# profess-dev/profess-ad

Hardware: AMD Instinct MI355X
Metric: energy+grad evals/sec (higher is better)
Workload: dtype f64; 1 GPU; 256^3 grid, f64, IonElectron+Hartree+WGC99(+TF+vW)+PBE closure chi->(E,dE/dchi); density=converged fcc-Al 32^3 fixture tiled 8^3 + 1e-3 low-|k| perturbation, parallelism=single GPU

## Files before the change

include/ofdft_hip.h:

```cpp
#ifndef OFDFT_HIP_H
#define OFDFT_HIP_H

#include <stdint.h>

#ifdef __cplusplus
extern "C" {
#endif

typedef struct ofdft_ctx ofdft_ctx;

#define OFDFT_OK            0
#define OFDFT_EINVAL       -1
#define OFDFT_EHIP         -2
#define OFDFT_ESTATE       -3
#define OFDFT_ENOMEM       -4

#define OFDFT_F64 0
#define OFDFT_F32 1

#define OFDFT_ION_ELECTRON  (1u << 0)
#define OFDFT_HARTREE       (1u << 1)
#define OFDFT_TF            (1u << 2)
#define OFDFT_VW            (1u << 3)
#define OFDFT_WT_NL         (1u << 4)
#define OFDFT_WGC99_NL      (1u << 5)
#define OFDFT_LDA_X         (1u << 6)
#define OFDFT_PZ_C          (1u << 7)
#define OFDFT_PW_C          (1u << 8)
#define OFDFT_CHACHIYO_C    (1u << 9)
#define OFDFT_PBE_X         (1u << 10)
#define OFDFT_PBE_C         (1u << 11)
#define OFDFT_GGA_K         (1u << 12)
#define OFDFT_VWGTF         (1u << 13)
#define OFDFT_NLK           (1u << 14)
#define OFDFT_NTERMS        15

#define OFDFT_P_WT_ALPHA    0
#define OFDFT_P_WT_BETA     1
#define OFDFT_P_WGC_ALPHA   2
#define OFDFT_P_WGC_BETA    3
#define OFDFT_P_WGC_GAMMA   4
#define OFDFT_P_WGC_KAPPA   5
#define OFDFT_P_GGAK_KIND   6
#define OFDFT_P_GGAK_MU     7
#define OFDFT_P_GGAK_BETA   8
#define OFDFT_P_GGAK_LAMBDA 9
#define OFDFT_P_GGAK_SIGMA  10
#define OFDFT_P_VWGTF_KIND  11
#define OFDFT_P_WTS_KIND    12
#define OFDFT_P_NLK_KIND    13
#define OFDFT_P_NLK_P0      14
#define OFDFT_P_NLK_P1      15
#define OFDFT_P_NLK_P2      16
#define OFDFT_NPARAMS       17

#define OFDFT_Q_FFT_COUNT        0
#define OFDFT_Q_WORKSPACE_BYTES  1
#define OFDFT_Q_FAST_PATH        2
#define OFDFT_Q_KERNEL_MS        3
#define OFDFT_Q_LAUNCH_COUNT     4
#define OFDFT_Q_YPASS_COUNT      5
#define OFDFT_Q_GRAPH_REPLAYS     6
#define OFDFT_Q_RESIDENT_EVALS    7
#define OFDFT_Q_XCHG_CHUNKS      9
#define OFDFT_Q_YFWD_FUSED      10
#define OFDFT_Q_RESIDENT_FALLBACKS 8
#define OFDFT_Q_XPASS_KINDS     11
#define OFDFT_XPASS_GROUP    (1u << 0)
#define OFDFT_XPASS_WAVE     (1u << 1)
#define OFDFT_XPASS_CROSS1   (1u << 2)
#define OFDFT_XPASS_CROSS2   (1u << 3)
#define OFDFT_XPASS_CHIRPZ   (1u << 4)

int  ofdft_create(ofdft_ctx** out, int n0, int n1, int n2, int dtype, int device_id);
void ofdft_destroy(ofdft_ctx* ctx);
const char* ofdft_last_error(const ofdft_ctx* ctx);

int  ofdft_set_cell(ofdft_ctx* ctx, const double box_vecs[9]);
int  ofdft_set_terms(ofdft_ctx* ctx, uint32_t term_mask, const double* params, int nparams);

int  ofdft_energy_potential(ofdft_ctx* ctx, const void* den_dev, const void* vext_dev,
                            double* E_terms_host, void* dEdn_dev, void* stream);

int  ofdft_energy_grad_chi(ofdft_ctx* ctx, const void* chi_dev, const void* vext_dev, double n_electrons,
                           double* E_terms_host, double* mu_host, void* grad_dev, void* stream);

int  ofdft_rfftn(ofdft_ctx* ctx, const void* real_dev, void* spec_dev, void* stream);
int  ofdft_irfftn(ofdft_ctx* ctx, const void* spec_dev, void* real_dev, void* stream);
int  ofdft_debug_math(ofdft_ctx* ctx, int kind, const void* in_dev, void* out_dev, long long n, void* stream);

int  ofdft_query(ofdft_ctx* ctx, int what, double* out);

int  ofdft_ipc_export(ofdft_ctx* ctx, void* handle64, unsigned long long* offsets5);
int  ofdft_ipc_attach(ofdft_ctx* ctx, int peer_rank, const void* handle64, const unsigned long long* offsets5);
int  ofdft_ipc_detach(ofdft_ctx* ctx);
int  ofdft_dist_closure(ofdft_ctx* ctx, const void* chi_local_dev, const void* vext_local_dev, double n_electrons_global,
                        double* E_terms_host, double* mu_host, void* grad_local_dev, void* v_work_local_dev, void* stream);

typedef int (*ofdft_all_to_all_fn)(void* user, void* send_dev, void* recv_dev, unsigned long long bytes_per_peer, void* stream);
typedef int (*ofdft_all_reduce_fn)(void* user, double* host_buf, int count);
int  ofdft_set_collectives(ofdft_ctx* ctx, ofdft_all_to_all_fn all_to_all, ofdft_all_reduce_fn all_reduce, void* user);

int  ofdft_create_dist(ofdft_ctx** out, int n0_global, int n1_global, int n2, int dtype, int device_id, int nranks, int rank);
int  ofdft_dist_sumsq(ofdft_ctx* ctx, const void* x_local_dev, int square, double* local_sum_host, void* stream);
int  ofdft_dist_begin(ofdft_ctx* ctx, const void* src_local_dev, int from_chi, double cscale, double n_electrons_global,
                      const void* vext_local_dev, void* v_out_local_dev, void* stream);
int  ofdft_dist_stage(ofdft_ctx* ctx, int stage, int chain, void* stream, unsigned long long* bytes_per_peer, void** sendbuf_dev,
                      void** recvbuf_dev);
int  ofdft_dist_step(ofdft_ctx* ctx, int step, int chain, int chunk, void* stream, unsigned long long* bytes_per_peer,
                     void** sendbuf_dev, void** recvbuf_dev);
int  ofdft_dist_finish(ofdft_ctx* ctx, double* local_sums_host , void* stream);
int  ofdft_dist_scalars(ofdft_ctx* ctx, void** scalars_dev );
int  ofdft_dist_energies(ofdft_ctx* ctx, const double* global_sums , double* E_terms_host, double* vn_integral);
int  ofdft_dist_chi_grad(ofdft_ctx* ctx, const void* chi_local_dev, const void* v_local_dev, void* grad_local_dev,
                         double cscale, double mu, void* stream);

int  ofdft_ionic_potential(ofdft_ctx* ctx, const double* frac_coords_host, int nions, const double* table_k_host,
                           const double* table_v_host, int ntable, double z_ion, int pme_order, void* vext_dev,
                           int accumulate, void* stream);

int  ofdft_ion_electron_forces(ofdft_ctx* ctx, const void* den_dev, const double* frac_coords_host, int nions,
                               const double* table_k_host, const double* table_v_host, int ntable, double z_ion,
                               int pme_order, double* forces_host, void* stream);

int  ofdft_stress(ofdft_ctx* ctx, const void* den_dev, double* sigma_terms_host, void* stream);
int  ofdft_ion_electron_stress(ofdft_ctx* ctx, const void* den_dev, const double* frac_coords_host, int nions,
                               const double* table_k_host, const double* table_v_host, int ntable, double z_ion,
                               int pme_order, double* sigma_host , void* stream);

int  ofdft_ion_ion(ofdft_ctx* ctx, const double* frac_coords_host, const double* charges_host, int nions, double Rc,
                   double* E_host, double* forces_host, double* stress_host, void* stream);

int  ofdft_ion_ion_cells(ofdft_ctx* ctx, const double* frac_coords_host, const double* charges_host, int nions, double Rc,
                         double Rd, int part, int nparts, double* E_host, double* forces_host ,
                         double* stress_host , void* stream);

typedef struct ofdft_lbfgs ofdft_lbfgs;
int  ofdft_lbfgs_create(ofdft_lbfgs** out, long long n_local, int history , int device_id);
void ofdft_lbfgs_destroy(ofdft_lbfgs* h);
const char* ofdft_lbfgs_last_error(const ofdft_lbfgs* h);
int  ofdft_lbfgs_reset(ofdft_lbfgs* h);
int  ofdft_lbfgs_direction(ofdft_lbfgs* h, const double* dots , int npairs, int first_iteration,
                           double* coef_s , double* coef_y , double* coef_g, double* g_dot_d,
                           int* npairs_out, int* pushed_out);
int  ofdft_lbfgs_abs_step(ofdft_lbfgs* h, double* abs_step_sum);
int  ofdft_lbfgs_dots(ofdft_lbfgs* h, const void* g_dev, double* dots_host , int* npairs, void* stream);
int  ofdft_lbfgs_commit(ofdft_lbfgs* h, int push);
int  ofdft_lbfgs_update(ofdft_lbfgs* h, const double* coef_s, const double* coef_y, double coef_g, double t, void* x_dev,
                        const void* g_dev, double* abs_step_sum_host, void* stream);

#define OFDFT_OPT_PIPELINE 0
#define OFDFT_OPT_XCHUNKS     2
#define OFDFT_OPT_XCHUNK_MASK 3
#define OFDFT_OPT_SPLIT_COMBINE 4
#define OFDFT_OPT_BLUESTEIN 5
#define OFDFT_OPT_GGA_SPLIT 6
#define OFDFT_OPT_GRAPH 7
#define OFDFT_OPT_SIDE_STREAM 1
#define OFDFT_OPT_MIXED_RADIX 9
#define OFDFT_OPT_RESIDENT 10
#define OFDFT_OPT_XCHG_CHUNKS 12
#define OFDFT_OPT_YBATCH 14
#define OFDFT_OPT_IPC_WAIT_MS 13
#define OFDFT_OPT_TEST_FAULT 11
#define OFDFT_OPT_BS_FUSED 15
#define OFDFT_OPT_POT_SPECTRUM 16
#define OFDFT_OPT_AXIS_PASSES 17
#define OFDFT_OPT_WGC_FOLD 28
#define OFDFT_OPT_XWAVE 8
int  ofdft_set_option(ofdft_ctx* ctx, int option, double value);

int  ofdft_set_profiling(ofdft_ctx* ctx, int on);
int  ofdft_profile_count(ofdft_ctx* ctx);
int  ofdft_profile_get(ofdft_ctx* ctx, int idx, char* name_buf, int buflen, double* total_ms, long long* launches);

#ifdef __cplusplus
}
#endif
#endif
```

professad_amd/_build.py:

```python
import contextlib
import fcntl
import os
import subprocess
import sys

PKG = os.path.dirname(os.path.abspath(__file__))
CSRC = os.path.join(PKG, 'csrc')
LIBDIR = os.path.join(PKG, 'lib')
LIB = os.path.join(LIBDIR, 'libofdft_hip.so')
LIB_F32 = os.path.join(LIBDIR, 'libofdft_hip_f32.so')
SOURCES = ['engine.hip', 'lines.hip', 'xpass_a.hip', 'xpass_b.hip', 'zfused.hip', 'resident.hip']
HEADERS = sorted(f for f in os.listdir(CSRC) if f.endswith('.h')) + [os.path.join('..', '..', 'include', 'ofdft_hip.h')]


def _stale(lib=None):
    lib = lib or LIB
    if not os.path.exists(lib):
        return True
    t = os.path.getmtime(lib)
    for f in SOURCES + HEADERS:
        p = os.path.join(CSRC, f)
        if os.path.exists(p) and os.path.getmtime(p) > t:
            return True
    return False


def _flags(extra_flags):
    return ['-O3', '-std=c++17', '--offload-arch=gfx950', '-fPIC', '-ffp-contract=on', '-Wall', '-Wno-unused-function',
            '-I', os.path.join(PKG, '..', 'include')] + list(extra_flags)


def _compile_and_link(extra_flags, out, verbose=False):
    hipcc = os.environ.get('HIPCC', '/opt/rocm/bin/hipcc')
    tag = '%s.%d' % (os.path.basename(out), os.getpid())
    objdir = os.path.join(LIBDIR, '.obj')
    os.makedirs(objdir, exist_ok=True)
    jobs, objs = [], []
    for src in SOURCES:
        obj = os.path.join(objdir, '%s.%s.o' % (tag, src))
        objs.append(obj)
        cmd = [hipcc] + _flags(extra_flags) + ['-c', os.path.join(CSRC, src), '-o', obj]
        if verbose:
            print(' '.join(cmd), flush=True)
        jobs.append((cmd, subprocess.Popen(cmd)))
    err = None
    for cmd, p in jobs:
        if p.wait() != 0:
            err = err or subprocess.CalledProcessError(p.returncode, cmd)
    try:
        if err:
            raise err
        link = [hipcc, '--offload-arch=gfx950', '-shared', '-fPIC'] + objs + ['-o', out]
        if verbose:
            print(' '.join(link), flush=True)
        subprocess.run(link, check=True)
    finally:
        for o in objs:
            with contextlib.suppress(OSError):
                os.remove(o)
    return out


@contextlib.contextmanager
def _build_lock():
    os.makedirs(LIBDIR, exist_ok=True)
    with open(os.path.join(LIBDIR, '.build.lock'), 'w') as fh:
        fcntl.flock(fh, fcntl.LOCK_EX)
        try:
            yield
        finally:
            fcntl.flock(fh, fcntl.LOCK_UN)


def build(force=False, verbose=True, extra_flags=(), out=None):
    os.makedirs(LIBDIR, exist_ok=True)
    if out is not None:
        tmp = '%s.tmp.%d' % (out, os.getpid())
        _compile_and_link(extra_flags, tmp, verbose)
        os.replace(tmp, out)
        return out
    import threading
    with _build_lock():
        todo = [(lib, flags) for lib, flags in ((LIB, []), (LIB_F32, ['-DOFDFT_REAL_F32', '-cl-single-precision-constant']))
                if force or _stale(lib)]
        errs = []

        def one(lib, flags):
            tmp = '%s.tmp.%d' % (lib, os.getpid())
            try:
                _compile_and_link(list(extra_flags) + flags, tmp, verbose)
                os.replace(tmp, lib)
            except Exception as e:
                errs.append(e)
                with contextlib.suppress(OSError):
                    os.remove(tmp)
        threads = [threading.Thread(target=one, args=t) for t in todo]
        for t in threads:
            t.start()
        for t in threads:
            t.join()
        if errs:
            raise errs[0]
    return LIB


if __name__ == '__main__':
    build(force='--force' in sys.argv)
```

professad_amd/_native.py:

```python
import ctypes as C
import os

import torch

from . import _build

_LIBS = {}

OK, EINVAL, EHIP, ESTATE, ENOMEM = 0, -1, -2, -3, -4
F64, F32 = 0, 1
TERM_BITS = {
    'ion_electron': 1 << 0, 'hartree': 1 << 1, 'tf': 1 << 2, 'vw': 1 << 3, 'wt_nl': 1 << 4, 'wgc99_nl': 1 << 5,
    'lda_x': 1 << 6, 'pz_c': 1 << 7, 'pw_c': 1 << 8, 'chachiyo_c': 1 << 9, 'pbe_x': 1 << 10, 'pbe_c': 1 << 11,
    'gga_k': 1 << 12, 'vwgtf': 1 << 13, 'nlk': 1 << 14,
}
TERM_ORDER = ['ion_electron', 'hartree', 'tf', 'vw', 'wt_nl', 'wgc99_nl', 'lda_x', 'pz_c', 'pw_c', 'chachiyo_c',
              'pbe_x', 'pbe_c', 'gga_k', 'vwgtf', 'nlk']
NTERMS = 15
NPARAMS = 17
NLK_KGAP, NLK_MGP, NLK_XWM = 1, 2, 3
NTERMS_ALWAYS = 14


def per_term(values, mask):
    return {nm: values[i] for i, nm in enumerate(TERM_ORDER) if i < NTERMS_ALWAYS or (mask & TERM_BITS[nm])}
Q_FFT_COUNT, Q_WORKSPACE_BYTES, Q_FAST_PATH, Q_KERNEL_MS, Q_LAUNCH_COUNT, Q_YPASS_COUNT, Q_GRAPH_REPLAYS, Q_RESIDENT_EVALS = 0, 1, 2, 3, 4, 5, 6, 7
Q_RESIDENT_FALLBACKS = 8
Q_XCHG_CHUNKS = 9
Q_YFWD_FUSED = 10
Q_XPASS_KINDS = 11
XPASS_GROUP, XPASS_WAVE, XPASS_CROSS1, XPASS_CROSS2, XPASS_CHIRPZ = 1 << 0, 1 << 1, 1 << 2, 1 << 3, 1 << 4
OPT_BLUESTEIN = 5
OPT_GGA_SPLIT = 6
OPT_GRAPH = 7
OPT_XWAVE = 8
OPT_MIXED_RADIX = 9
OPT_RESIDENT = 10
OPT_TEST_FAULT = 11
OPT_XCHG_CHUNKS = 12
OPT_IPC_WAIT_MS = 13
OPT_YBATCH = 14
OPT_BS_FUSED = 15
OPT_POT_SPECTRUM = 16
OPT_AXIS_PASSES = 17
OPT_WGC_FOLD = 28

EXPORTS = ['ofdft_create', 'ofdft_destroy', 'ofdft_last_error', 'ofdft_set_cell', 'ofdft_set_terms',
           'ofdft_energy_potential', 'ofdft_energy_grad_chi', 'ofdft_rfftn', 'ofdft_irfftn', 'ofdft_debug_math', 'ofdft_query',
           'ofdft_create_dist', 'ofdft_dist_sumsq', 'ofdft_dist_begin', 'ofdft_dist_stage', 'ofdft_dist_step', 'ofdft_dist_finish', 'ofdft_dist_scalars',
           'ofdft_dist_energies', 'ofdft_dist_chi_grad', 'ofdft_ipc_export', 'ofdft_ipc_attach', 'ofdft_ipc_detach', 'ofdft_dist_closure', 'ofdft_ionic_potential', 'ofdft_ion_electron_forces', 'ofdft_stress', 'ofdft_ion_electron_stress', 'ofdft_ion_ion', 'ofdft_ion_ion_cells', 'ofdft_lbfgs_create', 'ofdft_lbfgs_destroy', 'ofdft_lbfgs_last_error', 'ofdft_lbfgs_reset', 'ofdft_lbfgs_direction', 'ofdft_lbfgs_abs_step', 'ofdft_lbfgs_dots',
           'ofdft_lbfgs_commit', 'ofdft_lbfgs_update', 'ofdft_set_option', 'ofdft_set_collectives', 'ofdft_set_profiling', 'ofdft_profile_count', 'ofdft_profile_get']


A2A_FN = C.CFUNCTYPE(C.c_int, C.c_void_p, C.c_void_p, C.c_void_p, C.c_ulonglong, C.c_void_p)
ALLREDUCE_FN = C.CFUNCTYPE(C.c_int, C.c_void_p, C.POINTER(C.c_double), C.c_int)


class NativeLibraryError(RuntimeError):
    pass


def lib_path(dtype=F64):
    return _build.LIB_F32 if dtype == F32 else _build.LIB


def load(dtype=F64):
    if dtype in _LIBS:
        return _LIBS[dtype]
    env = 'OFDFT_LIB_F32' if dtype == F32 else 'OFDFT_LIB'
    path = os.environ.get(env) or lib_path(dtype)
    if os.environ.get(env):
        pass
    elif not os.path.exists(path) or (os.path.exists('/opt/rocm/bin/hipcc') and _build._stale(path)):
        try:
            _build.build(verbose=False)
        except Exception as e:
            raise NativeLibraryError('%s is missing and could not be built: %r' % (os.path.basename(path), e))
    try:
        lib = C.CDLL(path)
    except OSError as e:
        raise NativeLibraryError('cannot load %s: %s (the HIP engine is required; there is no CPU fallback)'
                                 % (path, e))
    vp, dp, ip = C.c_void_p, C.POINTER(C.c_double), C.c_int
    lib.ofdft_create.argtypes = [C.POINTER(vp), ip, ip, ip, ip, ip]
    lib.ofdft_create.restype = ip
    lib.ofdft_destroy.argtypes = [vp]
    lib.ofdft_destroy.restype = None
    lib.ofdft_last_error.argtypes = [vp]
    lib.ofdft_last_error.restype = C.c_char_p
    lib.ofdft_set_cell.argtypes = [vp, dp]
    lib.ofdft_set_cell.restype = ip
    lib.ofdft_set_terms.argtypes = [vp, C.c_uint32, dp, ip]
    lib.ofdft_set_terms.restype = ip
    lib.ofdft_energy_potential.argtypes = [vp, vp, vp, dp, vp, vp]
    lib.ofdft_energy_potential.restype = ip
    lib.ofdft_energy_grad_chi.argtypes = [vp, vp, vp, C.c_double, dp, dp, vp, vp]
    lib.ofdft_energy_grad_chi.restype = ip
    lib.ofdft_rfftn.argtypes = [vp, vp, vp, vp]
    lib.ofdft_rfftn.restype = ip
    lib.ofdft_irfftn.argtypes = [vp, vp, vp, vp]
    lib.ofdft_irfftn.restype = ip
    lib.ofdft_debug_math.argtypes = [vp, ip, vp, vp, C.c_longlong, vp]
    lib.ofdft_debug_math.restype = ip
    lib.ofdft_query.argtypes = [vp, ip, dp]
    lib.ofdft_query.restype = ip
    lib.ofdft_create_dist.argtypes = [C.POINTER(vp), ip, ip, ip, ip, ip, ip, ip]
    lib.ofdft_create_dist.restype = ip
    lib.ofdft_dist_sumsq.argtypes = [vp, vp, ip, dp, vp]
    lib.ofdft_dist_sumsq.restype = ip
    lib.ofdft_dist_begin.argtypes = [vp, vp, ip, C.c_double, C.c_double, vp, vp, vp]
    lib.ofdft_dist_begin.restype = ip
    lib.ofdft_dist_stage.argtypes = [vp, ip, ip, vp, C.POINTER(C.c_ulonglong), C.POINTER(vp), C.POINTER(vp)]
    lib.ofdft_dist_stage.restype = ip
    lib.ofdft_dist_step.argtypes = [vp, ip, ip, ip, vp, C.POINTER(C.c_ulonglong), C.POINTER(vp), C.POINTER(vp)]
    lib.ofdft_dist_step.restype = ip
    lib.ofdft_dist_scalars.argtypes = [vp, C.POINTER(vp)]
    lib.ofdft_dist_scalars.restype = ip
    lib.ofdft_dist_finish.argtypes = [vp, dp, vp]
    lib.ofdft_dist_finish.restype = ip
    lib.ofdft_dist_energies.argtypes = [vp, dp, dp, dp]
    lib.ofdft_dist_energies.restype = ip
    lib.ofdft_dist_chi_grad.argtypes = [vp, vp, vp, vp, C.c_double, C.c_double, vp]
    lib.ofdft_dist_chi_grad.restype = ip
    lib.ofdft_ipc_export.argtypes = [vp, vp, C.POINTER(C.c_ulonglong)]
    lib.ofdft_ipc_export.restype = ip
    lib.ofdft_ipc_attach.argtypes = [vp, ip, vp, C.POINTER(C.c_ulonglong)]
    lib.ofdft_ipc_attach.restype = ip
    lib.ofdft_ipc_detach.argtypes = [vp]
    lib.ofdft_ipc_detach.restype = ip
    lib.ofdft_dist_closure.argtypes = [vp, vp, vp, C.c_double, dp, dp, vp, vp, vp]
    lib.ofdft_dist_closure.restype = ip
    lib.ofdft_ionic_potential.argtypes = [vp, dp, ip, dp, dp, ip, C.c_double, ip, vp, ip, vp]
    lib.ofdft_ionic_potential.restype = ip
    lib.ofdft_ion_electron_forces.argtypes = [vp, vp, dp, ip, dp, dp, ip, C.c_double, ip, dp, vp]
    lib.ofdft_ion_electron_forces.restype = ip
    lib.ofdft_stress.argtypes = [vp, vp, dp, vp]
    lib.ofdft_stress.restype = ip
    lib.ofdft_ion_electron_stress.argtypes = [vp, vp, dp, ip, dp, dp, ip, C.c_double, ip, dp, vp]
    lib.ofdft_ion_electron_stress.restype = ip
    lib.ofdft_ion_ion.argtypes = [vp, dp, dp, ip, C.c_double, dp, dp, dp, vp]
    lib.ofdft_ion_ion.restype = ip
    lib.ofdft_ion_ion_cells.argtypes = [vp, dp, dp, ip, C.c_double, C.c_double, ip, ip, dp, dp, dp, vp]
    lib.ofdft_ion_ion_cells.restype = ip
    lib.ofdft_lbfgs_create.argtypes = [C.POINTER(vp), C.c_longlong, ip, ip]
    lib.ofdft_lbfgs_create.restype = ip
    lib.ofdft_lbfgs_destroy.argtypes = [vp]
    lib.ofdft_lbfgs_destroy.restype = None
    lib.ofdft_lbfgs_last_error.argtypes = [vp]
    lib.ofdft_lbfgs_last_error.restype = C.c_char_p
    lib.ofdft_lbfgs_reset.argtypes = [vp]
    lib.ofdft_lbfgs_reset.restype = ip
    lib.ofdft_lbfgs_dots.argtypes = [vp, vp, dp, C.POINTER(ip), vp]
    lib.ofdft_lbfgs_dots.restype = ip
    lib.ofdft_lbfgs_commit.argtypes = [vp, ip]
    lib.ofdft_lbfgs_commit.restype = ip
    lib.ofdft_lbfgs_update.argtypes = [vp, dp, dp, C.c_double, C.c_double, vp, vp, dp, vp]
    lib.ofdft_lbfgs_update.restype = ip
    lib.ofdft_lbfgs_direction.argtypes = [vp, dp, ip, ip, dp, dp, dp, dp, C.POINTER(ip), C.POINTER(ip)]
    lib.ofdft_lbfgs_direction.restype = ip
    lib.ofdft_lbfgs_abs_step.argtypes = [vp, dp]
    lib.ofdft_lbfgs_abs_step.restype = ip
    lib.ofdft_set_collectives.argtypes = [vp, A2A_FN, ALLREDUCE_FN, vp]
    lib.ofdft_set_collectives.restype = ip
    lib.ofdft_set_option.argtypes = [vp, ip, C.c_double]
    lib.ofdft_set_option.restype = ip
    lib.ofdft_set_profiling.argtypes = [vp, ip]
    lib.ofdft_set_profiling.restype = ip
    lib.ofdft_profile_count.argtypes = [vp]
    lib.ofdft_profile_count.restype = ip
    lib.ofdft_profile_get.argtypes = [vp, ip, C.c_char_p, ip, dp, C.POINTER(C.c_longlong)]
    lib.ofdft_profile_get.restype = ip
    _LIBS[dtype] = lib
    return lib
```

professad_amd/csrc/engine.hip:

```cpp
#include "engine_ctx.h"
#include <atomic>
#include <chrono>
#ifndef OFDFT_REAL_F32
#include "ion_kernels.h"
#include "ion_cells.h"
#include "stress_kernels.h"
#endif

namespace {
thread_local char g_create_error[512] = "";
}

namespace eng {

int fail(ofdft_ctx* c, int code, const char* fmt, ...) {
    va_list ap;
    va_start(ap, fmt);
    vsnprintf(c ? c->err : g_create_error, 512, fmt, ap);
    va_end(ap);
    return code;
}

int get_twiddle(ofdft_ctx* c, int n, cplx** out) {
    auto it = c->tw.find(n);
// ... 1309 lines not shown
    HIP_TRY(c, hipGetLastError());
    if (c->profiling) prof_collect(c);
    return OFDFT_OK;
}

int ofdft_irfftn(ofdft_ctx* c, const void* spec_dev, void* real_dev, void* stream) {
    hipStream_t st = (hipStream_t)stream;
    if (!c || !real_dev || !spec_dev) return OFDFT_EINVAL;
    OFDFT_ON_DEVICE(c, c->device);
    cplx* s;
    if (int rc = spec_ws(c, "io", &s)) return rc;
    OFDFT_LAUNCH(c, st, "spec_to_internal", spec_to_internal_kernel, dim3((unsigned)((c->g.total + 255) / 256)), dim3(256), 0,
                 (const cplx*)spec_dev, s, c->g);
    if (int rc = irfftn_internal(c, s, (real*)real_dev, 1.0 / (double)c->npts, st)) return rc;
    HIP_TRY(c, hipStreamSynchronize(st));
    HIP_TRY(c, hipGetLastError());
    if (c->profiling) prof_collect(c);
    return OFDFT_OK;
}

}
namespace {
__global__ void debug_math_kernel(int kind, const real* __restrict__ in, real* __restrict__ out, long long n) {
    for (long long i = (long long)blockIdx.x * blockDim.x + threadIdx.x; i < n; i += (long long)gridDim.x * blockDim.x) {
        const real x = in[i];
        real y;
        switch (kind) {
            case 0: y = fm::rcp(x); break;
            case 1: y = fm::log(x); break;
            case 2: y = fm::exp(x); break;
            case 3: y = fm::roots(x).y; break;
            case 4: y = fm::roots(x).n13; break;
            default: y = fm::roots(x).inv_n; break;
        }
        out[i] = y;
    }
}
}
extern "C" {

int ofdft_debug_math(ofdft_ctx* c, int kind, const void* in_dev, void* out_dev, long long n, void* stream) {
    hipStream_t st = (hipStream_t)stream;
    if (!c || !in_dev || !out_dev || n < 1 || kind < 0 || kind > 5) return OFDFT_EINVAL;
    OFDFT_ON_DEVICE(c, c->device);
    OFDFT_LAUNCH(c, st, "debug_math", debug_math_kernel, dim3(grid_for(n)), dim3(256), 0, kind, (const real*)in_dev, (real*)out_dev, n);
    HIP_TRY(c, hipStreamSynchronize(st));
    HIP_TRY(c, hipGetLastError());
    return OFDFT_OK;
}

#include "ipc_exchange.inc.h"

int ofdft_dist_sumsq(ofdft_ctx* c, const void* x_local, int square, double* local_sum, void* stream) {
    hipStream_t st = (hipStream_t)stream;
    if (!c || !x_local) return OFDFT_EINVAL;
    OFDFT_ON_DEVICE(c, c->device);
    if (local_sum) return device_sum(c, (const real*)x_local, square != 0, local_sum, st);
    const int blocks = grid_for(c->npts / 2 + 1, kRedThreads, kRedBlocks);
    if (square)
        OFDFT_LAUNCH(c, st, "sum", (sum_kernel<true>), dim3(blocks), dim3(kRedThreads), 0, (const real*)x_local, c->npts,
                     c->d_partial);
    else
        OFDFT_LAUNCH(c, st, "sum", (sum_kernel<false>), dim3(blocks), dim3(kRedThreads), 0, (const real*)x_local, c->npts,
                     c->d_partial);
    OFDFT_REDUCE(c, st, c->d_partial, blocks, 1, c->d_reduced + kSumsqSlot);
    HIP_TRY(c, hipGetLastError());
    return OFDFT_OK;
}

int ofdft_dist_scalars(ofdft_ctx* c, void** scalars_dev) {
    if (!c || !scalars_dev) return OFDFT_EINVAL;
    *scalars_dev = c->d_reduced;
    return OFDFT_OK;
}

int ofdft_dist_begin(ofdft_ctx* c, const void* src_local, int from_chi, double cscale, double nel_global,
                     const void* vext_local, void* v_out_local, void* stream) {
    hipStream_t st = (hipStream_t)stream;
    if (!c) return OFDFT_EINVAL;
    OFDFT_ON_DEVICE(c, c->device);
    if (int rc = begin_call(c, st)) return rc;
    if (!src_local) return fail(c, OFDFT_EINVAL, "null argument");
    if (!c->mask) return fail(c, OFDFT_ESTATE, "ofdft_set_terms has not been called");
    if ((c->mask & OFDFT_ION_ELECTRON) && !vext_local) return fail(c, OFDFT_EINVAL, "IonElectron term needs vext");
    if (!(c->fast && c->n2 / 2 <= 512)) return fail(c, OFDFT_EINVAL, "staged path needs the power-of-two fast path");
    if (gga_needs_laplacian(c) && !c->gga_split)
        return fail(c, OFDFT_EINVAL, "Laplacian-dependent Pauli-Gaussian members need the split-derivative GGA chain (OFDFT_OPT_GGA_SPLIT = 1)");
    if (wts_active(c) && c->nranks > 1)
        return fail(c, OFDFT_EINVAL, "the stabilised Wang-Teter style functional (OFDFT_P_WTS_KIND) is served by single-GPU contexts");
    ZRun& r = zrun(c);
    if (from_chi == 2) {
        OFDFT_LAUNCH(c, st, "reduce", closure_scale_kernel, dim3(1), dim3(64), 0, c->d_reduced + kSumsqSlot, c->d_scal, nel_global,
                     c->vol / (double)c->npts_g);
        r.ds = DenSrc{(const real*)src_local, 0.0, 1, c->d_scal};
    } else {
        r.ds = DenSrc{(const real*)src_local, (real)cscale, from_chi, nullptr};
    }
    r.nel = nel_global;
    r.vext = (const real*)vext_local;
    r.v_out = (real*)v_out_local;
    r.setup_done = false;
    r.stage[0] = r.stage[1] = 0;
    c->recv_parity[0] = c->recv_parity[1] = 0;
    r.step[0] = r.step[1] = 0;
    r.step_chunk[0] = r.step_chunk[1] = 0;
    r.deferred.clear();
    r.forked = false;
    r.closure = false;
    r.vpart_deferred = false;
    r.za.v_part_deferred = 0;
    r.xlist[0].clear();
    r.xlist[1].clear();
    return OFDFT_OK;
}

int ofdft_dist_stage(ofdft_ctx* c, int stage, int chain, void* stream, unsigned long long* bytes_per_peer, void** sendbuf,
                     void** recvbuf) {
    hipStream_t st = (hipStream_t)stream;
    if (!c || !bytes_per_peer || !sendbuf || !recvbuf || chain < 0 || chain > 1) return OFDFT_EINVAL;
    OFDFT_ON_DEVICE(c, c->device);
    ZRun& r = zrun(c);
    if (stage != r.stage[chain] + 1 || stage < 1 || stage > 4 || (chain == 1 && r.stage[0] < 1))
        return fail(c, OFDFT_ESTATE, "stage %d of chain %d out of order", stage, chain);
    if (c->xc.n > 1)
        return fail(c, OFDFT_ESTATE, "the exchange buffers are cut into %d kz chunks (OFDFT_OPT_XCHG_CHUNKS): sequence the evaluation with ofdft_dist_step", c->xc.n);
    int rc;
    switch (stage) {
        case 1: rc = zstage1(c, st, chain); break;
        case 2: rc = zstage2(c, st, chain); break;
        case 3: rc = zstage3(c, st, chain); break;
        default: rc = zstage4(c, st, chain); break;
    }
    if (rc) return rc;
    *bytes_per_peer = 0;
    *sendbuf = *recvbuf = nullptr;
    if (c->nranks > 1 && !r.xlist[chain].empty()) {
        cplx *send, *recv;
        if ((rc = dist_buffers(c, chain, &send, &recv))) return rc;
        if ((rc = dist_recv_next(c, chain, &recv))) return rc;
        *bytes_per_peer = (unsigned long long)(sizeof(cplx) * (size_t)c->xg.nxl * c->xg.arr_sz * r.xlist[chain].size());
        *sendbuf = send;
        *recvbuf = recv;
        c->recv_parity[chain] ^= 1;
    }
    HIP_TRY(c, hipGetLastError());
    return OFDFT_OK;
}

int ofdft_dist_step(ofdft_ctx* c, int step, int chain, int chunk, void* stream, unsigned long long* bytes_per_peer, void** sendbuf,
                    void** recvbuf) {
    hipStream_t st = (hipStream_t)stream;
    if (!c || !bytes_per_peer || !sendbuf || !recvbuf || chain < 0 || chain > 1) return OFDFT_EINVAL;
    OFDFT_ON_DEVICE(c, c->device);
    ZRun& r = zrun(c);
    const int K = c->xc.n;
    const bool next_chunk = step == r.step[chain] && chunk == r.step_chunk[chain] + 1 && chunk < K;
    const bool next_step = step == r.step[chain] + 1 && chunk == 0 && (r.step[chain] == 0 || r.step_chunk[chain] == K - 1);
    if (step < 1 || step > 6 || !(next_chunk || next_step) || (chain == 1 && r.step[0] < 1))
        return fail(c, OFDFT_ESTATE, "step %d chunk %d of chain %d out of order (last: step %d chunk %d of %d)", step, chunk, chain,
                    r.step[chain], r.step_chunk[chain], K);
    int rc;
    switch (step) {
        case 1: rc = zstage1(c, st, chain, chunk); break;
        case 2: rc = zstage2(c, st, chain, chunk); break;
        case 3: rc = zstage3(c, st, chain, 1, chunk); break;
        case 4: rc = zstage3(c, st, chain, 2, chunk); break;
        case 5: rc = zstage4(c, st, chain, chunk); break;
        default: rc = chain == 0 ? zstage5(c, nullptr, st, false, 1, chunk) : 0; break;
    }
    if (rc) return rc;
    r.step[chain] = step;
    r.step_chunk[chain] = chunk;
    *bytes_per_peer = 0;
    *sendbuf = *recvbuf = nullptr;
    const bool sends = step == 1 || step == 2 || step == 4 || step == 5;
    if (sends && c->nranks > 1 && !r.xlist[chain].empty()) {
        cplx *send, *recv;
        if ((rc = dist_buffers(c, chain, &send, &recv))) return rc;
        if ((rc = dist_recv_next(c, chain, &recv))) return rc;
        const XcView v = xc_view(c, chunk);
        const long long narr = (long long)r.xlist[chain].size();
        *bytes_per_peer = (unsigned long long)(sizeof(cplx) * (size_t)c->xg.nxl * v.arr_sz * narr);
        *sendbuf = send + narr * v.base1;
        *recvbuf = recv + narr * v.base1;
        if (chunk == K - 1) c->recv_parity[chain] ^= 1;
    }
    if (step == 5 && chunk == K - 1) r.stage[chain] = 4;
    HIP_TRY(c, hipGetLastError());
    return OFDFT_OK;
}

int ofdft_dist_finish(ofdft_ctx* c, double* local_sums, void* stream) {
    hipStream_t st = (hipStream_t)stream;
    if (!c) return OFDFT_EINVAL;
    OFDFT_ON_DEVICE(c, c->device);
    ZRun& r = zrun(c);
    if (r.stage[0] != 4 || r.stage[1] != 4) return fail(c, OFDFT_ESTATE, "ofdft_dist_finish called before stage 4 of both chains");
    const bool stepped = r.step[0] > 0;
    if (stepped && !(r.step[0] == 6 && r.step_chunk[0] == c->xc.n - 1 && r.step[1] == 6 && r.step_chunk[1] == c->xc.n - 1))
        return fail(c, OFDFT_ESTATE, "ofdft_dist_finish called before step 6 of both chains");
    int rc;
    if ((rc = zstage5(c, local_sums, st, false, stepped ? 2 : 0))) return rc;
    if (!local_sums) {
        HIP_TRY(c, hipEventRecord(c->ev1, st));
        c->ms_pending = true;
        HIP_TRY(c, hipGetLastError());
        if (c->profiling) {
            HIP_TRY(c, hipStreamSynchronize(st));
            prof_collect(c);
        }
        return OFDFT_OK;
    }
    return end_call(c, st);
}

int ofdft_dist_energies(ofdft_ctx* c, const double* global_sums, double* E_terms, double* vn_int) {
    if (!c || !global_sums || !E_terms || !vn_int) return OFDFT_EINVAL;
    for (int i = 0; i < OFDFT_NTERMS; ++i) E_terms[i] = 0.0;
    energies_from_sums(c, global_sums, global_sums + kCombineScalars, E_terms, vn_int);
    return OFDFT_OK;
}

int ofdft_dist_chi_grad(ofdft_ctx* c, const void* chi_local, const void* v_local, void* grad_local, double cscale,
                        double mu, void* stream) {
    hipStream_t st = (hipStream_t)stream;
    if (!c || !chi_local || !v_local || !grad_local) return OFDFT_EINVAL;
    OFDFT_ON_DEVICE(c, c->device);
    OFDFT_LAUNCH(c, st, "chi_grad", chi_grad_kernel, dim3(grid_for(c->npts / 2 + 1)), dim3(256), 0, (const real*)chi_local,
                 (const real*)v_local, (real*)grad_local, c->npts, cscale * 2.0 * c->dV,
                 cscale > 0.0 ? (const acc_t*)nullptr : (const acc_t*)c->d_scal, 2.0 * c->dV, mu);
    HIP_TRY(c, hipGetLastError());
    return OFDFT_OK;
}

#ifndef OFDFT_REAL_F32
#include "engine_ions_stress.inc.h"
#include "engine_ion_cells.inc.h"
#else
#define OFDFT_F64_ONLY(c) fail(c, OFDFT_EINVAL, "%s is served by the fp64 library (libofdft_hip.so) only", __func__)
extern "C" {
int ofdft_ionic_potential(ofdft_ctx* c, const double*, int, const double*, const double*, int, double, int, void*, int, void*) {
    return OFDFT_F64_ONLY(c);
}
int ofdft_ion_electron_forces(ofdft_ctx* c, const void*, const double*, int, const double*, const double*, int, double, int,
                              double*, void*) {
    return OFDFT_F64_ONLY(c);
}
int ofdft_stress(ofdft_ctx* c, const void*, double*, void*) { return OFDFT_F64_ONLY(c); }
int ofdft_ion_electron_stress(ofdft_ctx* c, const void*, const double*, int, const double*, const double*, int, double, int,
                              double*, void*) {
    return OFDFT_F64_ONLY(c);
}
int ofdft_ion_ion(ofdft_ctx* c, const double*, const double*, int, double, double*, double*, double*, void*) {
    return OFDFT_F64_ONLY(c);
}
int ofdft_ion_ion_cells(ofdft_ctx* c, const double*, const double*, int, double, double, int, int, double*, double*, double*, void*) {
    return OFDFT_F64_ONLY(c);
}
}
#endif

int ofdft_set_collectives(ofdft_ctx* c, ofdft_all_to_all_fn all_to_all, ofdft_all_reduce_fn all_reduce, void* user) {
    if (!c) return OFDFT_EINVAL;
    c->a2a = all_to_all;
    c->allreduce = all_reduce;
    c->coll_user = user;
    return OFDFT_OK;
}

int ofdft_set_option(ofdft_ctx* c, int option, double value) {
    if (!c) return OFDFT_EINVAL;
    c->version++;
    switch (option) {
        case OFDFT_OPT_GRAPH:
            c->use_graph = value != 0.0;
            return OFDFT_OK;
        case OFDFT_OPT_PIPELINE:
            c->force_unfused = value == 1.0;
            c->pipeline = (int)value;
            return OFDFT_OK;
        case OFDFT_OPT_SIDE_STREAM:
            c->use_side_stream = value != 0.0;
            return OFDFT_OK;
        case OFDFT_OPT_XCHUNKS:
            if (value < 0.0 || value > 64.0) return fail(c, OFDFT_EINVAL, "x chunks must be 0 (automatic) or 1..64");
            c->xchunks = (int)value;
            return OFDFT_OK;
        case OFDFT_OPT_BLUESTEIN:
            c->use_bluestein = value != 0.0;
            return OFDFT_OK;
        case OFDFT_OPT_BS_FUSED:
            c->bs_fused = value != 0.0;
            return OFDFT_OK;
        case OFDFT_OPT_GGA_SPLIT:
            c->gga_split = value != 0.0;
            return OFDFT_OK;
        case OFDFT_OPT_POT_SPECTRUM:
            c->pot_spectrum = value != 0.0;
            return OFDFT_OK;
        case OFDFT_OPT_AXIS_PASSES:
            if (value != 0.0 && value != 1.0 && value != 2.0 && value != 3.0) return fail(c, OFDFT_EINVAL, "OFDFT_OPT_AXIS_PASSES takes 0..3");
            c->axis_passes = (int)value;
            return OFDFT_OK;
        case OFDFT_OPT_SPLIT_COMBINE:
            c->split_combine = value != 0.0;
            c->defer_vpart = value != 1.0;
            return OFDFT_OK;
        case OFDFT_OPT_XCHUNK_MASK:
            c->xchunk_mask = (int)value & 31;
            return OFDFT_OK;
        case OFDFT_OPT_MIXED_RADIX:
            if (c->nranks > 1 && value == 0.0 && !all_pow2(c))
                return fail(c, OFDFT_EINVAL, "a slab-decomposed context on extents with factors 3 / 5 has no other path than the mixed-radix plans");
            c->fast = line_extent_ok(c->n0g) && line_extent_ok(c->n1g) && row_extent_ok(c->n2) && is_pow2(c->nranks) &&
                      (value != 0.0 || all_pow2(c));
            return OFDFT_OK;
        case OFDFT_OPT_XWAVE:
            c->use_xwave = (int)value;
            return OFDFT_OK;
        case OFDFT_OPT_RESIDENT:
            if (value != 0.0 && value != 1.0 && value != 2.0) return fail(c, OFDFT_EINVAL, "OFDFT_OPT_RESIDENT takes 0, 1 or 2");
            c->resident = (int)value;
            return OFDFT_OK;
        case OFDFT_OPT_XCHG_CHUNKS:
            if (value < 0.0 || value > 16.0) return fail(c, OFDFT_EINVAL, "OFDFT_OPT_XCHG_CHUNKS takes 0 (automatic) or 1..16");
            xchg_chunks_set(c, (int)value);
            c->wgc_valid = false;
            return OFDFT_OK;
        case OFDFT_OPT_YBATCH:
            c->ybatch = (int)value;
            return OFDFT_OK;
        case OFDFT_OPT_WGC_FOLD:
            c->wgc_fold = value != 0.0;
            return OFDFT_OK;
        case OFDFT_OPT_IPC_WAIT_MS:
            if (!(value >= 1.0 && value <= 3.6e6)) return fail(c, OFDFT_EINVAL, "OFDFT_OPT_IPC_WAIT_MS takes 1 .. 3 600 000 ms");
            c->ipc_wait_ms = value;
            return OFDFT_OK;
        case OFDFT_OPT_TEST_FAULT:
            c->test_fault = (int)value;
            if (c->test_fault == 2) c->res_fits = 0;
            return OFDFT_OK;
    }
    return fail(c, OFDFT_EINVAL, "unknown option %d", option);
}

int ofdft_set_profiling(ofdft_ctx* c, int on) {
    if (!c) return OFDFT_EINVAL;
    c->profiling = on != 0;
    c->prof.clear();
    c->pending.clear();
    c->ev_used = 0;
    return OFDFT_OK;
}

int ofdft_profile_count(ofdft_ctx* c) { return c ? (int)c->prof.size() : OFDFT_EINVAL; }

int ofdft_profile_get(ofdft_ctx* c, int idx, char* name_buf, int buflen, double* total_ms, long long* launches) {
    if (!c || idx < 0 || idx >= (int)c->prof.size() || !name_buf || buflen < 2) return OFDFT_EINVAL;
    auto it = c->prof.begin();
    std::advance(it, idx);
    std::snprintf(name_buf, (size_t)buflen, "%s", it->first.c_str());
    if (total_ms) *total_ms = it->second.ms;
    if (launches) *launches = it->second.launches;
    return OFDFT_OK;
}

int ofdft_query(ofdft_ctx* c, int what, double* out) {
    if (!c || !out) return OFDFT_EINVAL;
    switch (what) {
        case OFDFT_Q_FFT_COUNT: *out = c->fft_count; return OFDFT_OK;
        case OFDFT_Q_WORKSPACE_BYTES: *out = (double)c->ws_bytes; return OFDFT_OK;
        case OFDFT_Q_FAST_PATH: *out = c->fast ? 1.0 : 0.0; return OFDFT_OK;
        case OFDFT_Q_KERNEL_MS:
            if (c->ms_pending) {
                OFDFT_ON_DEVICE(c, c->device);
                HIP_TRY(c, hipEventSynchronize(c->ev1));
                HIP_TRY(c, hipEventElapsedTime(&c->last_ms, c->ev0, c->ev1));
                c->ms_pending = false;
            }
            *out = c->last_ms;
            return OFDFT_OK;
        case OFDFT_Q_LAUNCH_COUNT: *out = c->launch_count; return OFDFT_OK;
        case OFDFT_Q_YPASS_COUNT: *out = c->ypass_count; return OFDFT_OK;
        case OFDFT_Q_GRAPH_REPLAYS: *out = (double)c->graph_replays; return OFDFT_OK;
        case OFDFT_Q_RESIDENT_EVALS: *out = (double)c->resident_evals; return OFDFT_OK;
        case OFDFT_Q_RESIDENT_FALLBACKS: *out = (double)c->resident_fallbacks; return OFDFT_OK;
        case OFDFT_Q_XCHG_CHUNKS: *out = (double)c->xc.n; return OFDFT_OK;
        case OFDFT_Q_YFWD_FUSED: *out = (double)c->yfwd_fused; return OFDFT_OK;
        case OFDFT_Q_XPASS_KINDS: *out = (double)c->xpass_kinds; return OFDFT_OK;
        case 16: case 17: case 18: case 19: case 20: case 21: case 22: case 23: case 24: case 25: case 26: case 27:
            *out = c->h_partial[what] * 0.01;
            return OFDFT_OK;
    }
    return fail(c, OFDFT_EINVAL, "unknown query %d", what);
}

}

#include "lbfgs_abi.h"
```

professad_amd/csrc/engine_ctx.h:

```cpp
#pragma once
#include <hip/hip_runtime.h>

#include <algorithm>
#include <cmath>
#include <cstdarg>
#include <cstdio>
#include <cstring>
#include <map>
#include <string>
#include <vector>

#include "../../include/ofdft_hip.h"
#include "bluestein.h"
#include "zpass.h"
#include "xwave.h"

using namespace ofdft;

struct DevBuf {
    void* p = nullptr;
    size_t bytes = 0;
    bool borrowed = false;
};

struct XchgChunks {
    int n = 1;
    int kb[17] = {0};
};

struct ofdft_ctx {
    int n0 = 0, n1 = 0, n2 = 0, device = 0;
    int n0g = 0, n1g = 0, nranks = 1, rank = 0;
    SpecGeom g{};
    SpecGeom gx{};
    KGeom kg{};
    XchgGeom xg{};
    XchgChunks xc{};
    int xchg_chunks_req = 0;
    long long npts = 0;
    long long npts_g = 0;
    bool fast = false, cell_set = false, force_unfused = false;
    int pipeline = 0;
    double box[9] = {0}, vol = 0.0, dV = 0.0;
    unsigned mask = 0;
    double params[OFDFT_NPARAMS];
    std::map<int, cplx*> tw;
    std::map<std::string, DevBuf> ws;
    size_t ws_bytes = 0;
    double* d_partial = nullptr;
    double* d_reduced = nullptr;
    double* d_scal = nullptr;
    double* h_partial = nullptr;
    long long partial_rows = 0;
    double* d_wgc_coef = nullptr;
    long long wgc_key_nel = -1;
    int fft_passes_fused = 0;
    int yfwd_fused = 0;
    bool wgc_valid = false;
    double wgc_ck = 0.0;
    bool nlk_valid = false;
    long long nlk_key_nel = -1;
    double nlk_key_nel_exact = 0.0;
    double* d_nlk_w = nullptr;
    bool wgc_fold = true;
    int fft_count = 0, launch_count = 0;
    int xpass_blocks = 0;
    unsigned xpass_kinds = 0;
    double ypass_count = 0.0;
    float last_ms = 0.f;
    bool ms_pending = false;
    hipEvent_t ev0 = nullptr, ev1 = nullptr, ev_fork = nullptr, ev_join = nullptr, ev_join2 = nullptr, ev_a = nullptr, ev_b = nullptr, ev_c = nullptr;
    hipStream_t side_stream = nullptr, side_stream2 = nullptr;
    bool use_side_stream = true;
    bool bs_fused = true;
    bool use_bluestein = true;
    bool gga_split = true;
    bool pot_spectrum = true;
    int axis_passes = 3;
    bool split_combine = true;
    bool defer_vpart = true;
    int ybatch = 1;
    int xchunk_mask = 2;
    int use_xwave = 1;
    int xchunks = 1;
    bool profiling = false;
    std::vector<hipEvent_t> ev_pool;
    size_t ev_used = 0;
    struct Pending { const char* name; size_t a, b; };
    std::vector<Pending> pending;
    struct Acc { double ms = 0.0; long long launches = 0; };
    std::map<std::string, Acc> prof;
    struct ofdft_zrun_holder* zr = nullptr;
    struct GraphEntry {
        const void *chi = nullptr, *vext = nullptr, *grad = nullptr;
        double nel = 0.0;
        unsigned long long version = 0;
        int seen = 0;
        hipGraphExec_t exec = nullptr;
        int collect = 0;
        int fft_count = 0, launch_count = 0, yfwd_fused = 0;
        unsigned xpass_kinds = 0;
        double ypass_count = 0.0;
    };
    std::vector<GraphEntry> graphs;
    unsigned long long version = 1;
    bool use_graph = true;
    int resident = 2;
    unsigned* res_sync = nullptr;
    unsigned res_epoch = 0;
    long long resident_evals = 0;
    int test_fault = 0;
    int res_fits = -1;
    long long resident_fallbacks = 0;
    unsigned* res_done = nullptr;
    unsigned res_done_target = 0;
    long long graph_replays = 0;
    hipStream_t cap_stream = nullptr;
    struct ofdft_ipc_state* ipc = nullptr;
    int recv_parity[2] = {0, 0};
    double ipc_wait_ms = 30000.0;
    ofdft_all_to_all_fn a2a = nullptr;
    ofdft_all_reduce_fn allreduce = nullptr;
    void* coll_user = nullptr;
    char err[512] = "";
};


namespace eng {

constexpr unsigned kGgaAny = OFDFT_PBE_X | OFDFT_PBE_C | OFDFT_GGA_K;
constexpr int kNSums = kCombineScalars + kPbeScalars;
constexpr int kSumsqSlot = 15;

inline GgaSel gga_sel(const ofdft_ctx* c) {
    return GgaSel{(c->mask & OFDFT_PBE_X) ? 1 : 0, (c->mask & OFDFT_PBE_C) ? 1 : 0, (c->mask & OFDFT_GGA_K) ? 1 : 0,
                  (int)c->params[OFDFT_P_GGAK_KIND], (real)c->params[OFDFT_P_GGAK_MU], (real)c->params[OFDFT_P_GGAK_BETA],
                  (real)c->params[OFDFT_P_GGAK_LAMBDA], (real)c->params[OFDFT_P_GGAK_SIGMA]};
}

inline bool gga_needs_laplacian(const ofdft_ctx* c) {
    return (c->mask & OFDFT_GGA_K) && (int)c->params[OFDFT_P_GGAK_KIND] == 1 &&
           (c->params[OFDFT_P_GGAK_BETA] != 0.0 || c->params[OFDFT_P_GGAK_LAMBDA] != 0.0 || c->params[OFDFT_P_GGAK_SIGMA] != 0.0);
}
inline bool wts_active(const ofdft_ctx* c) {
    return (int)c->params[OFDFT_P_WTS_KIND] == 1 && (c->mask & OFDFT_TF) && (c->mask & (OFDFT_WT_NL | OFDFT_NLK));
}
struct NlPow {
    bool on = false, nlk = false, two = false;
    int kind = 0, sym = 0;
    double al = 0.0, be = 0.0;
    double e_b = 0.0, e_a = 0.0;
};
inline NlPow nl_pow(const ofdft_ctx* c) {
    NlPow p;
    if (c->mask & OFDFT_WT_NL) {
        p.on = true;
        p.al = c->params[OFDFT_P_WT_ALPHA];
        p.be = c->params[OFDFT_P_WT_BETA];
        p.e_b = p.be;
        p.e_a = p.al;
    } else if (c->mask & OFDFT_NLK) {
        p.on = p.nlk = true;
        p.kind = (int)c->params[OFDFT_P_NLK_KIND];
        const double x = c->params[OFDFT_P_NLK_P0];
        if (p.kind == NLK_KGAP) {
            const double fr = x * x / (5.0 + x * x), s5 = std::sqrt(5.0);
            p.al = 0.5 + ((5.0 + s5) / 6.0 - 0.5) * fr;
            p.be = 0.5 + ((5.0 - s5) / 6.0 - 0.5) * fr;
            p.e_b = p.be;
            p.e_a = p.al;
        } else if (p.kind == NLK_MGP) {
            p.al = p.be = p.e_b = p.e_a = kFiveSixths;
        } else {
            p.al = p.e_b = x + kFiveSixths;
            p.be = p.e_a = x + (double)11 / 6;
            p.sym = 1;
        }
    }
    p.two = p.on && p.al != p.be;
    return p;
}
inline unsigned combine_mask(const ofdft_ctx* c) {
    return (c->mask & OFDFT_NLK) ? ((c->mask & ~OFDFT_NLK) | OFDFT_WT_NL) : c->mask;
}
struct TermScalars {
    double nel = 0.0;
    long long nel_r = 0;
    double nbar = 0.0;
    double n0_r = 0.0;
    NlPow nlp;
    double wt_kf = 0.0;
    double wt_inv2kf = 0.0;
    double wt_pref = 0.0;
    TermConsts tc{};
};
inline TermScalars term_scalars(const ofdft_ctx* c, double nel) {
    TermScalars t;
    t.nel = nel;
    t.nel_r = std::llround(nel);
    t.nbar = nel / c->vol;
    t.n0_r = (double)t.nel_r / c->vol;
    t.nlp = nl_pow(c);
    t.wt_kf = std::cbrt(3.0 * kPi * kPi * t.nbar);
    t.wt_inv2kf = 1.0 / (2.0 * t.wt_kf);
    t.tc.gtf_kind = (int)c->params[OFDFT_P_VWGTF_KIND];
    t.tc.gtf_inv_n0 = (c->mask & OFDFT_VWGTF) ? c->vol / (double)std::llround(nel) : 0.0;
    if (t.nlp.on) {
        const double al = t.nlp.al, be = t.nlp.be;
        if (!t.nlp.nlk) t.wt_pref = 5.0 / (9.0 * al * be * std::pow(t.nbar, al + be - kFiveThirds));
        t.tc.wt_alpha = al;
        t.tc.wt_beta = be;
        t.tc.wt_nbar_pa = t.nlp.nlk ? 0.0 : std::pow(t.nbar, al);
        t.tc.wt_is_56 = (al == kFiveSixths && be == kFiveSixths) ? 1 : 0;
        t.tc.wt_sym = t.nlp.sym;
    }
    if (c->mask & OFDFT_WGC99_NL) {
        const double al = c->params[OFDFT_P_WGC_ALPHA], be = c->params[OFDFT_P_WGC_BETA];
        t.tc.wgc_alpha = al;
        t.tc.wgc_beta = be;
        t.tc.wgc_sum_53 = (std::fabs(al + be - kFiveThirds) < 4e-16) ? 1 : 0;
    }
    return t;
}
inline bool zfused_serves(const ofdft_ctx* c) {
    return c->fast && c->pipeline == 0 && c->n2 / 2 <= 512 && (!gga_needs_laplacian(c) || c->gga_split);
}

int fail(ofdft_ctx* c, int code, const char* fmt, ...);

#define HIP_TRY(ctx, call)                                                                         \
    do {                                                                                           \
        hipError_t e_ = (call);                                                                    \
        if (e_ != hipSuccess)                                                                      \
            return fail(ctx, OFDFT_EHIP, "%s failed: %s (%s:%d)", #call, hipGetErrorString(e_), __FILE__, __LINE__); \
    } while (0)


#define OFDFT_ON_DEVICE(ctx, dev)                                                                   \
    DeviceScope device_scope_(dev);                                                                 \
    if (device_scope_.err != hipSuccess)                                                            \
        return fail(ctx, OFDFT_EHIP, "cannot select device %d: %s", (dev), hipGetErrorString(device_scope_.err))

inline bool graph_eligible(const ofdft_ctx* c) { return c->use_graph && c->nranks == 1 && c->npts <= (1LL << 19); }
void prof_begin(ofdft_ctx* c, hipStream_t st, const char* name);
void prof_end(ofdft_ctx* c, hipStream_t st);
void prof_collect(ofdft_ctx* c);

#define OFDFT_LAUNCH(c, st, name, kern, grid, block, lds, ...)            \
    do {                                                                  \
        prof_begin(c, st, name);                                          \
        hipLaunchKernelGGL(kern, grid, block, lds, st, __VA_ARGS__);      \
        prof_end(c, st);                                                  \
        (c)->launch_count++;                                              \
    } while (0)

inline bool is_pow2(int n) { return n > 0 && (n & (n - 1)) == 0; }

#if !defined(OFDFT_REAL_F32) || !defined(OFDFT_NO_MIXED_F32)
#define OFDFT_MIXED_LINES(X) X(48) X(96) X(120) X(144) X(160) X(192) X(240) X(250) X(270) X(288) X(320) X(384) X(480)
#define OFDFT_MIXED_ROWS(X) X(24) X(48) X(60) X(72) X(80) X(96) X(120) X(125) X(135) X(144) X(160) X(192) X(240)
#else
#define OFDFT_MIXED_LINES(X)
#define OFDFT_MIXED_ROWS(X)
#endif
inline bool mixed_line(int n) {
#define X(L) if (n == L) return true;
    OFDFT_MIXED_LINES(X)
#undef X
    return false;
}
inline bool line_extent_ok(int n) { return (is_pow2(n) && n >= 8 && n <= 1024) || mixed_line(n); }
inline bool row_extent_ok(int n2) { return (is_pow2(n2) && n2 >= 16 && n2 <= 2048) || mixed_line(n2); }
inline bool all_pow2(const ofdft_ctx* c) { return is_pow2(c->n0g) && is_pow2(c->n1g) && is_pow2(c->n2); }

inline int grid_for(long long n, int tpb = 256, int cap = 2048) {
    long long b = (n + tpb - 1) / tpb;
    if (b > cap) b = cap;
    if (b < 1) b = 1;
    return (int)b;
}

#define OFDFT_REDUCE(c, st, partial, rows, ns, ...)                                                                          \
    do {                                                                                                                     \
        const acc_t* part_ = (partial);                                                                                      \
        const int rows_ = (rows), ns_ = (ns);                                                                                \
        if (rows_ > kRedTwoLevelRows) {                                                                                      \
            acc_t* mid_ = const_cast<acc_t*>(part_) + (size_t)rows_ * ns_;                                                   \
            int g_ = rows_ / 512;                                                                                            \
            g_ = g_ < 1 ? 1 : (g_ > kRedMidRows ? kRedMidRows : g_);                                                         \
            const int per_ = (rows_ + g_ - 1) / g_;                                                                          \
            g_ = (rows_ + per_ - 1) / per_;                                                                                  \
            OFDFT_LAUNCH(c, st, "reduce", reduce_rows_kernel, dim3(g_), dim3(kRedThreads), 0, part_, rows_, ns_, per_, mid_); \
            OFDFT_LAUNCH(c, st, "reduce", reduce_partials_kernel, dim3(ns_), dim3(kRedThreads), 0, (const acc_t*)mid_, g_, ns_, \
                         __VA_ARGS__);                                                                                       \
        } else {                                                                                                             \
            OFDFT_LAUNCH(c, st, "reduce", reduce_partials_kernel, dim3(ns_), dim3(kRedThreads), 0, part_, rows_, ns_, __VA_ARGS__); \
        }                                                                                                                    \
    } while (0)


constexpr int kWholeXchg = -2;
struct XcView {
    int kb0, kb1, nb, nrem;
    long long arr_sz;
    long long base1;
};
inline XcView xc_view(const ofdft_ctx* c, int k) {
    XcView v{};
    const bool whole = k == kWholeXchg || c->xc.n <= 1;
    v.kb0 = whole ? 0 : c->xc.kb[k];
    v.kb1 = whole ? c->xg.nb : c->xc.kb[k + 1];
    v.nb = v.kb1 - v.kb0;
    v.nrem = (whole || k == c->xc.n - 1) ? c->xg.nrem : 0;
    v.arr_sz = ((long long)v.nb * 8 + v.nrem) * c->xg.nyl;
    v.base1 = (long long)c->n0g * c->xg.nyl * 8 * v.kb0;
    return v;
}
inline int xchg_chunks_for(const ofdft_ctx* c, int req) {
    if (c->nranks < 2 || c->xg.nb < 2 || c->xg.nxl % 32 || c->xg.nyl % 32) return 1;
    int k = req;
    if (k <= 0) {
        k = c->npts >= (8LL << 20) ? 4 : (c->npts >= (1LL << 20) ? 2 : 1);
        k = std::min(k, c->xg.nb / 4);
    }
    k = std::max(1, std::min(k, std::min(16, c->xg.nb)));
    return k;
}
inline void xchg_chunks_set(ofdft_ctx* c, int req) {
    c->xchg_chunks_req = req;
    c->xc = XchgChunks{};
    c->xc.n = xchg_chunks_for(c, req);
    for (int k = 0; k <= c->xc.n; ++k) c->xc.kb[k] = (int)((long long)c->xg.nb * k / c->xc.n);
}

inline bool cell_axes_orthogonal(const ofdft_ctx* c) {
    const real* bb = c->kg.b;
    return bb[1] == 0.0 && bb[2] == 0.0 && bb[3] == 0.0 && bb[5] == 0.0 && bb[6] == 0.0 && bb[7] == 0.0;
}

int get_twiddle(ofdft_ctx* c, int n, cplx** out);
int get_ws(ofdft_ctx* c, const std::string& name, size_t bytes, void** out);
int real_ws(ofdft_ctx* c, const char* name, real** out);
int spec_ws(ofdft_ctx* c, const char* name, cplx** out);
size_t dist_buffer_bytes(ofdft_ctx* c, int chain);
int dist_buffers(ofdft_ctx* c, int chain, cplx** send, cplx** recv);
int dist_recv_next(ofdft_ctx* c, int chain, cplx** recv);
int dist_exchange(ofdft_ctx* c, cplx* send, cplx* recv, hipStream_t st);
int global_sums(ofdft_ctx* c, double* v, int n);

void pass_maps(const ofdft_ctx* c, int axis, LineMap& main, LineMap& rem);
template <bool INV>
int fast_axis_pass_multi(ofdft_ctx* c, int axis, cplx* const* specs, int narr, hipStream_t st, int x0 = 0, int cx = 0,
                         int kb0 = 0, int kb1 = 0);
template <bool INV> int fast_axis_pass(ofdft_ctx* c, int axis, cplx* spec, hipStream_t st);
template <bool INV> int ypass_xchg(ofdft_ctx* c, const std::vector<cplx*>& list, cplx* buf, hipStream_t st, int xk = -1);
int yderiv(ofdft_ctx* c, const cplx* in, cplx* out, double scale, hipStream_t st, cplx* fwd = nullptr);
int yderiv_add(ofdft_ctx* c, const cplx* in, const cplx* add, cplx* out, double scale, hipStream_t st);
int ylap(ofdft_ctx* c, const cplx* in, const cplx* add, cplx* out, double scale, hipStream_t st);
int rfftn_internal(ofdft_ctx* c, const real* in, cplx* spec, hipStream_t st);
int rfftn_internal_multi(ofdft_ctx* c, const real* const* in, cplx* const* spec, int n, hipStream_t st);
bool bluestein_xmix_ok(const ofdft_ctx* c);
template <int NIN, int NOUT, class Mix>
int bluestein_xmix(ofdft_ctx* c, const cplx* const* in, cplx* const* out, const Mix& mix, hipStream_t st);
struct BsPrep { int kind[kBsBatch] = {0, 0, 0, 0}; double e[kBsBatch] = {0, 0, 0, 0}; double nref = 0.0; };
int bluestein_fwd_zy_multi(ofdft_ctx* c, const real* const* in, cplx* const* spec, int n, hipStream_t st, const BsPrep* prep = nullptr);
int bluestein_inv_yz_multi(ofdft_ctx* c, cplx* const* spec, real* const* out, int n, double scale, hipStream_t st);
int irfftn_internal_multi(ofdft_ctx* c, cplx* const* spec, real* const* out, int n, double scale, hipStream_t st);
int irfftn_internal(ofdft_ctx* c, cplx* spec, real* out, double scale, hipStream_t st);
int fwd_zy(ofdft_ctx* c, const real* in, cplx* spec, hipStream_t st);
int inv_yz(ofdft_ctx* c, cplx* spec, real* out, double scale, hipStream_t st);

struct XfLayout {
    long long se_in = 0, se_out = 0, tse = 0;
    int kb0 = 0, kb1 = 0;
    int xnb = -1, xnrem = 0;
    int kz0 = 0;
};
template <int NIN, int NOUT, class Mix>
int xfused(ofdft_ctx* c, const XfIo& io, const Mix& mix, hipStream_t st, const char* nm, const XfLayout& lay = XfLayout{});
int xfused_wgc(ofdft_ctx* c, const XfIo& io, const MixWgc& mix, hipStream_t st, const char* nm, const XfLayout& lay = XfLayout{});
template <int NIN, class Mix>
int xfused_energy(ofdft_ctx* c, const XfIo& io, const Mix& mix, hipStream_t st, const char* nm);
bool xfused_energy_serves(const ofdft_ctx* c, int nin);

int launch_zf_density(ofdft_ctx* c, const DenSrc& ds, cplx* out_n, cplx* out_s, hipStream_t st, int chunk = 0, int nchunks = 1,
                      real* dzn = nullptr);
int ensure_wgc_tables(ofdft_ctx* c, long long nel_rounded, hipStream_t st, double* nref_out);
inline MixWgc wgc_tab(ofdft_ctx* c, long long off = 0) {
    const cplx* t01 = (const cplx*)c->ws["t:wgc"].p;
    return MixWgc{t01 + off, reinterpret_cast<const real*>(t01 + c->g.total) + off, (real)c->wgc_ck};
}
int ensure_nlk_table(ofdft_ctx* c, const TermScalars& ts, hipStream_t st);
inline int ensure_term_tables(ofdft_ctx* c, TermScalars& ts, hipStream_t st) {
    if (ts.nlp.nlk)
        if (int rc = ensure_nlk_table(c, ts, st)) return rc;
    if (c->mask & OFDFT_WGC99_NL) {
        double nref;
        if (int rc = ensure_wgc_tables(c, ts.nel_r, st, &nref)) return rc;
        ts.tc.nref = nref;
    }
    return 0;
}
inline const real* nlk_col(ofdft_ctx* c, int col) { return (const real*)c->ws["t:nlk"].p + (size_t)col * c->g.total; }
bool resident_serves(const ofdft_ctx* c);
constexpr int kResidentDeclined = 1;
int resident_closure(ofdft_ctx* c, const real* chi, const real* vext, double nel, real* v, real* grad, hipStream_t st, bool from_den = false);
int launch_zf_powers(ofdft_ctx* c, const DenSrc& ds, const PowersArgs& pa, hipStream_t st, int chunk = 0, int nchunks = 1);
int launch_zpbe(ofdft_ctx* c, const DenSrc& ds, cplx* gx, cplx* gy, cplx* gz, real* dfdn, double inv_n, int* blocks_out,
                hipStream_t st, int chunk = 0, int nchunks = 1);
int launch_zpbe2(ofdft_ctx* c, const DenSrc& ds, cplx* A, cplx* B, const real* dzn, real* dfdn, double inv_n, int* blocks_out,
                 hipStream_t st, cplx* L = nullptr);
int launch_zi_combine(ofdft_ctx* c, const ZCombineArgs& a, int* blocks_out, hipStream_t st, int chunk = 0, int nchunks = 1);
int launch_zi_wgc(ofdft_ctx* c, const ZCombineArgs& a, real* v_part, double* partial, int* blocks_out, hipStream_t st);

}
```

professad_amd/csrc/fft_kernels.h:

```cpp
#pragma once
#include "fft_radix.h"

namespace ofdft {

struct SpecGeom {
    int n0, n1, n2, nzc, nzm;
    int blk0 = 0;
    long long nrows;
    long long main_count;
    long long total;
};

__host__ __device__ inline long long spec_index(const SpecGeom& g, int x, int y, int kz) {
    const long long row = (long long)x * g.n1 + y;
    if (kz < g.nzm) return (((long long)(kz >> 3)) * g.nrows + row) * 8 + (kz & 7);
    return g.main_count + (long long)(kz - g.nzm) * g.nrows + row;
}

__device__ inline void spec_decode(const SpecGeom& g, long long i, int& x, int& y, int& kz) {
    if (i < g.main_count) {
        const int kin = (int)(i & 7);
        const long long r = i >> 3;
        const long long row = r % g.nrows;
        kz = (int)(r / g.nrows) * 8 + kin;
        x = (int)(row / g.n1);
        y = (int)(row % g.n1);
    } else {
        const long long r = i - g.main_count;
        const long long row = r % g.nrows;
        kz = g.nzm + (int)(r / g.nrows);
        x = (int)(row / g.n1);
        y = (int)(row % g.n1);
    }
}

struct LineMap {
    long long sb;
    long long se;
    int d;
    int sl;
    int nlines;
    int lf;
    int gc = 0, gn = 0, g0 = 0;
    int blk0 = 0;
    int kz0 = 0;
};

#ifndef OFDFT_CPASS_TPB
#define OFDFT_CPASS_TPB 256
#endif
template <int LEN> struct PassCfg {
    static constexpr int P = Plan<LEN>::P;
    static constexpr int E = Plan<LEN>::E;
    static constexpr int TPB = (8 * P > OFDFT_CPASS_TPB) ? 8 * P : OFDFT_CPASS_TPB;
    static constexpr int LPW = TPB / P;
    static constexpr int LSTR = kCXMul * LineBuf<LEN>::STRIDE;
    static constexpr size_t LDS = (Plan<LEN>::NST > 1) ? sizeof(real) * LPW * LSTR : 0;
};

__device__ __forceinline__ long long line_base(const LineMap& m, long long L) {
    long long grp = L / m.d;
    if (m.gc) grp = (grp / m.gc) * m.gn + m.g0 + grp % m.gc;
    return grp * m.sb + (L % m.d) * (long long)m.sl;
}

struct ArrList { cplx* p[16]; };

#ifndef OFDFT_CPASS_LD_AUX
#define OFDFT_CPASS_LD_AUX 2
#endif
#ifndef OFDFT_CPASS_ST_AUX
#define OFDFT_CPASS_ST_AUX 2
#endif
#ifndef OFDFT_XF_LD_AUX
#define OFDFT_XF_LD_AUX 0
#endif
#ifndef OFDFT_XF_BATCH_TABLES
#define OFDFT_XF_BATCH_TABLES 1
#endif
#ifndef OFDFT_XF_ST_AUX
#define OFDFT_XF_ST_AUX 2
#endif
#ifndef OFDFT_ZS_LD_AUX
#define OFDFT_ZS_LD_AUX 0
#endif
#ifndef OFDFT_ZS_ST_AUX
#define OFDFT_ZS_ST_AUX 0
#endif
#ifndef OFDFT_ZR_LD_AUX
#define OFDFT_ZR_LD_AUX 0
#endif
#ifndef OFDFT_ZR_ST_AUX
#define OFDFT_ZR_ST_AUX 0
#endif

#ifndef OFDFT_CPASS_TILES
#define OFDFT_CPASS_TILES 1
#endif
template <int LEN, bool INV>
__global__ __launch_bounds__(PassCfg<LEN>::TPB) void cpass_kernel(ArrList arrs, LineMap m_main, LineMap m_rem,
                                                                   int main_blocks, long long rem_offset,
                                                                   const cplx* __restrict__ tw) {
    cplx* data0 = arrs.p[blockIdx.y];
    constexpr int P = PassCfg<LEN>::P, E = PassCfg<LEN>::E, LPW = PassCfg<LEN>::LPW, T = OFDFT_CPASS_TILES;
    extern __shared__ __attribute__((aligned(16))) real lds[];
    const int tid = threadIdx.x;
    using PL = Plan<LEN>;
    cplx v[T][E];
    cplx* ubs[T];
    unsigned voffs[T];
    bool valids[T];
    long long se_us[T];
    int js[T], ls[T];
#pragma unroll
    for (int t = 0; t < T; ++t) {
        const int blk = (int)blockIdx.x * T + t;
        const bool in_rem = blk >= main_blocks;
        const LineMap m = in_rem ? m_rem : m_main;
        cplx* data = in_rem ? data0 + rem_offset : data0;
        const int bid = in_rem ? blk - main_blocks : blk + m.blk0;
        const int l_lo = tid % m.lf;
        const int j = (tid / m.lf) % P;
        const int l = (tid / (m.lf * P)) * m.lf + l_lo;
        const long long L0 = (long long)bid * LPW;
        const long long L = L0 + l;
        const bool valid = L < m.nlines;
        const long long b0 = uniform64(line_base(m, L0));
        ubs[t] = data + b0;
        voffs[t] = valid ? (unsigned)((line_base(m, L) - b0 + (long long)j * m.se) * kCB) : 0u;
        se_us[t] = uniform64(m.se);
        valids[t] = valid;
        js[t] = j;
        ls[t] = l;
#pragma unroll
        for (int q = 0; q < E; ++q)
            v[t][q] = (PL::slot_in(q) && valid && PL::lane_in(j, q)) ? buf_load_c_aux<OFDFT_CPASS_LD_AUX>(ubs[t] + PL::cin(q) * se_us[t], voffs[t])
                                                                       : mkc(0.0, 0.0);
    }
#pragma unroll
    for (int t = 0; t < T; ++t) {
        if (t > 0) __syncthreads();
        line_fft<LEN, INV, kCX>(v[t], js[t], lds + ls[t] * PassCfg<LEN>::LSTR, tw);
        if (valids[t]) {
#pragma unroll
            for (int q = 0; q < E; ++q)
                if (PL::slot_out(q) && PL::lane_out(js[t], q)) buf_store_c_aux<OFDFT_CPASS_ST_AUX>(ubs[t] + PL::cout(q) * se_us[t], voffs[t], v[t][q]);
        }
    }
}

template <class PL, bool WAVE>
__device__ __forceinline__ void repattern_out_to_in(cplx (&v)[PL::E], int j, real* line) {
    if constexpr (!PL::EXACT) {
        constexpr int E = PL::E;
        real re[E];
        exchange_sync<WAVE>();
#pragma unroll
        for (int q = 0; q < E; ++q)
            if (PL::slot_out(q) && PL::lane_out(j, q)) line[lpos<PL>(j + PL::cout(q))] = v[q].x;
        exchange_sync<WAVE>();
#pragma unroll
        for (int q = 0; q < E; ++q) re[q] = (PL::slot_in(q) && PL::lane_in(j, q)) ? line[lpos<PL>(j + PL::cin(q))] : (real)0.0;
        exchange_sync<WAVE>();
#pragma unroll
        for (int q = 0; q < E; ++q)
            if (PL::slot_out(q) && PL::lane_out(j, q)) line[lpos<PL>(j + PL::cout(q))] = v[q].y;
        exchange_sync<WAVE>();
#pragma unroll
        for (int q = 0; q < E; ++q)
            v[q] = (PL::slot_in(q) && PL::lane_in(j, q)) ? mkc(re[q], line[lpos<PL>(j + PL::cin(q))]) : mkc(0.0, 0.0);
        exchange_sync<WAVE>();
    }
}

template <int LEN, bool ADD = false, bool LAP = false>
__global__ __launch_bounds__(PassCfg<LEN>::TPB) void yderiv_kernel(const cplx* in, cplx* out,
                                                                   LineMap m_main, LineMap m_rem, int main_blocks,
                                                                   long long rem_offset, const cplx* __restrict__ tw,
                                                                   real scale, cplx* fwd, const cplx* add = nullptr) {
    constexpr int P = PassCfg<LEN>::P, E = PassCfg<LEN>::E, LPW = PassCfg<LEN>::LPW;
    extern __shared__ __attribute__((aligned(16))) real lds[];
    const int tid = threadIdx.x;
    const bool in_rem = (int)blockIdx.x >= main_blocks;
    const LineMap m = in_rem ? m_rem : m_main;
    const long long roff = in_rem ? rem_offset : 0;
    const int bid = in_rem ? (int)blockIdx.x - main_blocks : (int)blockIdx.x + m.blk0;
    const int l_lo = tid % m.lf;
    const int j = (tid / m.lf) % P;
    const int l = (tid / (m.lf * P)) * m.lf + l_lo;
    const long long L0 = (long long)bid * LPW;
    const long long L = L0 + l;
    const bool valid = L < m.nlines;
    const long long b0 = uniform64(line_base(m, L0));
    const unsigned voff = valid ? (unsigned)((line_base(m, L) - b0 + (long long)j * m.se) * kCB) : 0u;
    const long long se_u = uniform64(m.se);
    using PL = Plan<LEN>;
    cplx v[E];
#pragma unroll
    for (int q = 0; q < E; ++q)
        v[q] = (PL::slot_in(q) && valid && PL::lane_in(j, q)) ? buf_load_c(in + roff + b0 + PL::cin(q) * se_u, voff) : mkc(0.0, 0.0);
    cplx x[(ADD || LAP) ? E : 1];
    if constexpr (ADD || LAP) {
#pragma unroll
        for (int q = 0; q < E; ++q)
            x[q] = (PL::slot_out(q) && valid && PL::lane_out(j, q)) ? buf_load_c(add + roff + b0 + PL::cout(q) * se_u, voff) : mkc(0.0, 0.0);
    }
    real* mine = lds + l * PassCfg<LEN>::LSTR;
    line_fft<LEN, false, kCX>(v, j, mine, tw);
    if (fwd && valid) {
#pragma unroll
        for (int q = 0; q < E; ++q)
            if (PL::slot_out(q) && PL::lane_out(j, q)) buf_store_c_aux<OFDFT_CPASS_ST_AUX>(fwd + roff + b0 + PL::cout(q) * se_u, voff, v[q]);
    }
#pragma unroll
    for (int q = 0; q < E; ++q) {
        const int e = j + PL::cout(q);
        const real fe = (real)(e <= LEN / 2 ? e : e - LEN);
        if constexpr (LAP) {
            const real f = scale * fe * fe;
            v[q] = mkc(f * v[q].x, f * v[q].y);
        } else {
            const real f = scale * fe;
            v[q] = mkc(-f * v[q].y, f * v[q].x);
        }
        if constexpr (ADD) v[q] = cadd(v[q], x[q]);
    }
    __syncthreads();
    repattern_out_to_in<PL, false>(v, j, mine);
    line_fft<LEN, true, kCX>(v, j, mine, tw);
    if (valid) {
#pragma unroll
        for (int q = 0; q < E; ++q)
            if (PL::slot_out(q) && PL::lane_out(j, q)) {
                if constexpr (LAP) v[q] = cadd(v[q], x[q]);
                buf_store_c_aux<OFDFT_CPASS_ST_AUX>(out + roff + b0 + PL::cout(q) * se_u, voff, v[q]);
            }
    }
}

struct XchgGeom {
    int nxl, nyl, log_nyl, nb, nrem;
    long long arr_sz;
    long long rec;
    long long chunk;
    int kb0 = 0;
};
template <int LEN, bool INV>
__global__ __launch_bounds__(PassCfg<LEN>::TPB) void ypass_xchg_kernel(ArrList arrs, cplx* __restrict__ buf, XchgGeom xg,
                                                                       LineMap m_main, LineMap m_rem, int main_blocks,
                                                                       long long rem_offset,
                                                                       const cplx* __restrict__ tw) {
    constexpr int P = PassCfg<LEN>::P, E = PassCfg<LEN>::E, LPW = PassCfg<LEN>::LPW;
    extern __shared__ __attribute__((aligned(16))) real lds[];
    const int tid = threadIdx.x;
    const int a = blockIdx.y;
    const bool in_rem = (int)blockIdx.x >= main_blocks;
    const LineMap m = in_rem ? m_rem : m_main;
    cplx* data = arrs.p[a] + (in_rem ? rem_offset : 0);
    const int bid = in_rem ? (int)blockIdx.x - main_blocks : (int)blockIdx.x + m.blk0;
    const int l_lo = tid % m.lf;
    const int j = (tid / m.lf) % P;
    const int l = (tid / (m.lf * P)) * m.lf + l_lo;
    const long long L0 = (long long)bid * LPW;
    const long long L = L0 + l;
    const bool valid = L < m.nlines;
    const long long b0 = uniform64(line_base(m, L0));
    cplx* ub = data + b0;
    const unsigned voff = valid ? (unsigned)((line_base(m, L) - b0 + (long long)j * m.se) * kCB) : 0u;
    using PL = Plan<LEN>;
    long long lb;
    int es;
    if (!in_rem) {
        const long long r = L >> 3;
        const int kin = (int)(L & 7), xl = (int)(r % xg.nxl);
        const long long b = r / xg.nxl - xg.kb0;
        lb = xl * xg.rec + a * xg.arr_sz + b * xg.nyl * 8 + kin;
        es = 8;
    } else {
        const int xl = (int)(L % xg.nxl);
        const long long plane = L / xg.nxl;
        lb = xl * xg.rec + a * xg.arr_sz + (long long)xg.nb * xg.nyl * 8 + plane * xg.nyl;
        es = 1;
    }
    auto bpos = [&](int e) -> long long {
        int peer, yl;
        if constexpr (PL::EXACT) {
            peer = e >> xg.log_nyl;
            yl = e & (xg.nyl - 1);
        } else {
            peer = e / xg.nyl;
            yl = e - peer * xg.nyl;
        }
        return lb + (long long)peer * xg.chunk + (long long)yl * es;
    };
    const long long se_u = uniform64(m.se);
    cplx v[E];
#pragma unroll
    for (int q = 0; q < E; ++q) {
        const bool on = valid && PL::slot_in(q) && PL::lane_in(j, q);
        if (INV) v[q] = on ? nt_load_c(buf + bpos(j + PL::cin(q))) : mkc(0.0, 0.0);
        else v[q] = on ? buf_load_c_aux<OFDFT_CPASS_LD_AUX>(ub + PL::cin(q) * se_u, voff) : mkc(0.0, 0.0);
    }
    line_fft<LEN, INV, kCX>(v, j, lds + l * PassCfg<LEN>::LSTR, tw);
    if (valid) {
#pragma unroll
        for (int q = 0; q < E; ++q) {
            if (!(PL::slot_out(q) && PL::lane_out(j, q))) continue;
            if (INV) buf_store_c_aux<OFDFT_CPASS_ST_AUX>(ub + PL::cout(q) * se_u, voff, v[q]);
            else nt_store_c(buf + bpos(j + PL::cout(q)), v[q]);
        }
// ... 479 lines not shown
```

professad_amd/csrc/zfused.hip:

```cpp
#if defined(OFDFT_REAL_F32) && !defined(OFDFT_F32_PK)
#define OFDFT_F32_PK 1
#endif
#include "engine_ctx.h"

namespace eng {

#define OFDFT_ZCASES(X) X(8) X(16) X(32) X(64) X(128) X(256) X(512) OFDFT_MIXED_ROWS(X)
#ifndef OFDFT_EZ
#define OFDFT_EZ 4
#endif
constexpr int EZ = OFDFT_EZ;
#ifndef OFDFT_EZ_POWERS
#define OFDFT_EZ_POWERS OFDFT_EZ
#endif
constexpr int EZP = OFDFT_EZ_POWERS;

int z_tables(ofdft_ctx* c, cplx** twM, cplx** twN) {
    if (int rc = get_twiddle(c, c->n2 / 2, twM)) return rc;
    return get_twiddle(c, c->n2, twN);
}
template <int M, int E> int z_blocks(const ofdft_ctx* c) { return (int)((c->g.nrows + ZW<M, E>::RPB - 1) / ZW<M, E>::RPB); }

int launch_zf_density(ofdft_ctx* c, const DenSrc& ds, cplx* out_n, cplx* out_s, hipStream_t st, int chunk,
                      int nchunks, real* dzn) {
    cplx *twM, *twN;
    if (int rc = z_tables(c, &twM, &twN)) return rc;
    if (chunk == 0) c->fft_count += (out_n ? 1 : 0) + (out_s ? 1 : 0);
    SpecGeom gz = c->g;
#define X(M_)                                                                                                       \
    case M_: {                                                                                                      \
        const int nb = z_blocks<M_, ZPick<M_, 8>::E>(c) / nchunks;                                                  \
        gz.blk0 = chunk * nb;                                                                                       \
        OFDFT_LAUNCH(c, st, "zf_density", (zf_density_kernel<M_, ZPick<M_, 8>::E>), dim3(nb), dim3(256),            \
                     (ZW<M_, ZPick<M_, 8>::E>::LDS), ds, out_n, out_s, gz, twM, twN, dzn);                          \
        return 0;                                                                                                   \
    }
    switch (c->n2 / 2) { OFDFT_ZCASES(X) }
#undef X
    return fail(c, OFDFT_EINVAL, "bad n2");
}

int launch_zf_powers(ofdft_ctx* c, const DenSrc& ds, const PowersArgs& pa, hipStream_t st, int chunk, int nchunks) {
    cplx *twM, *twN;
    if (int rc = z_tables(c, &twM, &twN)) return rc;
    if (chunk == 0)
        for (int i = 0; i < 6; ++i) c->fft_count += pa.out[i] ? 1 : 0;
    SpecGeom gz = c->g;
#define X(M_)                                                                                                      \
    case M_: {                                                                                                     \
        const int nb = z_blocks<M_, ZPick<M_, EZP>::E>(c) / nchunks;                                                \
        gz.blk0 = chunk * nb;                                                                                      \
        if (pa.out[0] && !pa.out[1] && !pa.out[2] && !pa.out[3] && !pa.out[4] && !pa.out[5])                       \
            OFDFT_LAUNCH(c, st, "zf_powers", (zf_powers_kernel<M_, ZPick<M_, EZP>::E, true>), dim3(nb), dim3(256), \
                         (ZW<M_, ZPick<M_, EZP>::E>::LDS), ds, pa, gz, twM, twN);                                   \
        else                                                                                                       \
            OFDFT_LAUNCH(c, st, "zf_powers", (zf_powers_kernel<M_, ZPick<M_, EZP>::E>), dim3(nb), dim3(256),       \
                         (ZW<M_, ZPick<M_, EZP>::E>::LDS), ds, pa, gz, twM, twN);                                   \
        return 0;                                                                                                  \
    }
    switch (c->n2 / 2) { OFDFT_ZCASES(X) }
#undef X
    return fail(c, OFDFT_EINVAL, "bad n2");
}

int launch_zpbe(ofdft_ctx* c, const DenSrc& ds, cplx* gx, cplx* gy, cplx* gz, real* dfdn, double inv_n,
                int* blocks_out, hipStream_t st, int chunk, int nchunks) {
    cplx *twM, *twN;
    if (int rc = z_tables(c, &twM, &twN)) return rc;
    if (chunk == 0) c->fft_count += 6;
    SpecGeom gq = c->g;
#define X(M_)                                                                                                   \
    case M_: {                                                                                                  \
        *blocks_out = z_blocks<M_, ZPick<M_, EZ>::E>(c);                                                        \
        const int nb = *blocks_out / nchunks;                                                                   \
        gq.blk0 = chunk * nb;                                                                                   \
        OFDFT_LAUNCH(c, st, "zpbe", (zpbe_kernel<M_, ZPick<M_, EZ>::E>), dim3(nb), dim3(256),                   \
                     (ZW<M_, ZPick<M_, EZ>::E>::LDS), ds, gx, gy, gz, dfdn, inv_n, gga_sel(c), gq, twM, twN,   \
                     c->d_partial);                                                                             \
        return 0;                                                                                               \
    }
    switch (c->n2 / 2) { OFDFT_ZCASES(X) }
#undef X
    return fail(c, OFDFT_EINVAL, "bad n2");
}

int launch_zpbe2(ofdft_ctx* c, const DenSrc& ds, cplx* A, cplx* B, const real* dzn, real* dfdn, double inv_n,
                 int* blocks_out, hipStream_t st, cplx* L) {
    cplx *twM, *twN;
    if (int rc = z_tables(c, &twM, &twN)) return rc;
    c->fft_count += L ? 8 : 6;
    Bmat bm{};
    std::memcpy(bm.b, c->kg.b, sizeof(bm.b));
#define X(M_)                                                                                                   \
    case M_: {                                                                                                  \
        *blocks_out = z_blocks<M_, ZPick<M_, EZ>::E>(c);                                                        \
        if (L)                                                                                                  \
            OFDFT_LAUNCH(c, st, "zpbe", (zpbe2_kernel<M_, ZPick<M_, EZ>::E, true>), dim3(*blocks_out), dim3(256), \
                         (ZW<M_, ZPick<M_, EZ>::E>::LDS), ds, A, B, dzn, dfdn, inv_n, 1.0 / (double)c->n2, gga_sel(c), bm, \
                         c->g, twM, twN, c->d_partial, L);                                                      \
        else                                                                                                    \
            OFDFT_LAUNCH(c, st, "zpbe", (zpbe2_kernel<M_, ZPick<M_, EZ>::E, false>), dim3(*blocks_out), dim3(256), \
                         (ZW<M_, ZPick<M_, EZ>::E>::LDS), ds, A, B, dzn, dfdn, inv_n, 1.0 / (double)c->n2, gga_sel(c), bm, \
                         c->g, twM, twN, c->d_partial, L);                                                      \
        return 0;                                                                                               \
    }
    switch (c->n2 / 2) { OFDFT_ZCASES(X) }
#undef X
    return fail(c, OFDFT_EINVAL, "bad n2");
}

int launch_zi_combine(ofdft_ctx* c, const ZCombineArgs& a, int* blocks_out, hipStream_t st, int chunk, int nchunks) {
    cplx *twM, *twN;
    if (int rc = z_tables(c, &twM, &twN)) return rc;
    SpecGeom gq = c->g;
    const size_t park = sizeof(real) * 256 * kParkSlots;
#define X(M_)                                                                                                     \
    case M_: {                                                                                                    \
        using W = ZW<M_, ZPick<M_, EZ>::E>;                                                                       \
        *blocks_out = z_blocks<M_, W::E>(c);                                                                      \
        const int nb = *blocks_out / nchunks;                                                                     \
        gq.blk0 = chunk * nb;                                                                                     \
        if (a.v_part || !(a.mask & OFDFT_WGC99_NL))     \
            OFDFT_LAUNCH(c, st, "zi_combine", (zi_combine_kernel<M_, W::E, false>), dim3(nb), dim3(256),          \
                         (W::LDS + park), a, gq, twM, twN, c->d_partial);                                         \
        else                                                                                                      \
            OFDFT_LAUNCH(c, st, "zi_combine", (zi_combine_kernel<M_, W::E, true>), dim3(nb), dim3(256),           \
                         (W::LDS + park), a, gq, twM, twN, c->d_partial);                                         \
        return 0;                                                                                                 \
    }
    switch (c->n2 / 2) { OFDFT_ZCASES(X) }
#undef X
    return fail(c, OFDFT_EINVAL, "bad n2");
}

int launch_zi_wgc(ofdft_ctx* c, const ZCombineArgs& a, real* v_part, double* partial, int* blocks_out, hipStream_t st) {
    cplx *twM, *twN;
    if (int rc = z_tables(c, &twM, &twN)) return rc;
#define X(M_)                                                                                                     \
    case M_: {                                                                                                    \
        using W = ZW<M_, ZPick<M_, EZ>::E>;                                                                       \
        *blocks_out = z_blocks<M_, W::E>(c);                                                                      \
        OFDFT_LAUNCH(c, st, "zi_wgc", (zi_wgc_kernel<M_, W::E>), dim3(*blocks_out), dim3(256), (W::LDS), a, v_part, \
                     c->g, twM, twN, partial);                                                                    \
        return 0;                                                                                                 \
    }
    switch (c->n2 / 2) { OFDFT_ZCASES(X) }
#undef X
    return fail(c, OFDFT_EINVAL, "bad n2");
}


}
```

professad_amd/csrc/zpass.h:

```cpp
#pragma once
#include "pointwise_kernels.h"

namespace ofdft {

#ifndef OFDFT_ZPBE_WAVES
#define OFDFT_ZPBE_WAVES 2
#endif
#ifndef OFDFT_ZIWGC_WAVES
#define OFDFT_ZIWGC_WAVES 2
#endif
#ifndef OFDFT_Z_PREFETCH
#define OFDFT_Z_PREFETCH 1
#endif
#ifndef OFDFT_Z_PIPE_BIG_F32
#define OFDFT_Z_PIPE_BIG_F32 0
#endif
#ifndef OFDFT_ZI_ROOTS_ONCE
#define OFDFT_ZI_ROOTS_ONCE 0
#endif
#ifndef OFDFT_Z_LDS_TWIDDLES
#define OFDFT_Z_LDS_TWIDDLES 1
#endif

#ifndef OFDFT_Z_CX
#define OFDFT_Z_CX 0
#endif

template <int E> constexpr bool z_cx() { return kCX && (OFDFT_Z_CX == 1 || (OFDFT_Z_CX == 2 && E == 8)); }
template <int M, int E_> struct ZW {
    using PL = ZPlan<M, E_>;
    static constexpr int E = E_;
    static constexpr int P = PL::P;
    static constexpr int RPWV = 64 / P;
    static constexpr int TPB = 256;
    static constexpr int RPB = RPWV * (TPB / 64);
    static constexpr int RS = (z_cx<E_>() ? kCXMul : 1) * line_stride<PL>();
    static constexpr int ROWS = RPB * RS;
#if OFDFT_Z_LDS_TWIDDLES
    static constexpr size_t LDS = sizeof(real) * ROWS + sizeof(cplx) * 2 * M;
#else
    static constexpr size_t LDS = sizeof(real) * ROWS;
#endif
    static constexpr int N2 = 2 * M;
};

#ifndef OFDFT_Z_EMAX
#define OFDFT_Z_EMAX 6
#endif
#ifndef OFDFT_Z_EMAX_PBE
#define OFDFT_Z_EMAX_PBE 9
#endif
#ifndef OFDFT_Z_F32_BIG_WAVES
#define OFDFT_Z_F32_BIG_WAVES 1
#endif
template <int M, int E, int EMAX = OFDFT_Z_EMAX> constexpr int z_waves(int want) {
    if (sizeof(real) == 4 && OFDFT_Z_F32_BIG_WAVES && M >= 512 && E <= 8) return want > 2 ? 2 : want;
    return (M >= 512 || E > EMAX) ? (want > 2 ? 2 : 1) : want;
}

template <int M, int E, bool ONE> constexpr int z_powers_waves() {
    if (!ONE) return z_waves<M, E>(3);
    if (M >= 512 || E > OFDFT_Z_EMAX) return (sizeof(real) == 4 && E <= 8) ? 4 : z_waves<M, E>(3);
    return 4;
}

template <int M, int E> struct ZLane {
    int j;
    int rw;
    long long row_u;
    long long row;
    bool valid;
    real* mine;
    __device__ __forceinline__ ZLane(const SpecGeom& g, real* lds) {
        using W = ZW<M, E>;
        const int lane = threadIdx.x & 63;
        const int wave = __builtin_amdgcn_readfirstlane((int)(threadIdx.x >> 6));
        j = lane % W::P;
        rw = lane / W::P;
        row_u = uniform64((long long)(blockIdx.x + g.blk0) * W::RPB + (long long)wave * W::RPWV);
        row = row_u + rw;
        valid = row < g.nrows;
        mine = lds + (wave * W::RPWV + rw) * W::RS;
    }
    __device__ __forceinline__ ZLane(int j_, int rw_, real* mine_, bool valid_) : j(j_), rw(rw_), row_u(0), row(rw_), valid(valid_), mine(mine_) {}
};

template <int M, int E> struct ZTwReq {
    static constexpr int CNT = (M + ZW<M, E>::TPB - 1) / ZW<M, E>::TPB;
    cplx m[CNT], n[CNT];
};
template <int M, int E>
__device__ __forceinline__ ZTwReq<M, E> z_tw_request(const cplx* __restrict__ twM_g, const cplx* __restrict__ twN_g) {
    ZTwReq<M, E> r;
#if OFDFT_Z_LDS_TWIDDLES
#pragma unroll
    for (int c = 0; c < ZTwReq<M, E>::CNT; ++c) {
        const int i = threadIdx.x + c * ZW<M, E>::TPB;
        r.m[c] = twM_g[i < M ? i : 0];
        r.n[c] = twN_g[i < M ? i : 0];
    }
#endif
    return r;
}
template <int M, int E>
__device__ __forceinline__ void z_tw_commit(real* lds, const ZTwReq<M, E>& r, const cplx* __restrict__ twM_g,
                                            const cplx* __restrict__ twN_g, const cplx*& twM, const cplx*& twN) {
#if OFDFT_Z_LDS_TWIDDLES
    cplx* t = reinterpret_cast<cplx*>(lds + ZW<M, E>::ROWS);
#pragma unroll
    for (int c = 0; c < ZTwReq<M, E>::CNT; ++c) {
        const int i = threadIdx.x + c * ZW<M, E>::TPB;
        if (i < M) {
            t[i] = r.m[c];
            t[M + i] = r.n[c];
        }
    }
    __syncthreads();
    twM = t;
    twN = t + M;
#else
    twM = twM_g;
    twN = twN_g;
#endif
}

template <int M, int E, bool OUT = false>
__device__ __forceinline__ void z_load_real(cplx (&v)[E], const ZLane<M, E>& z, const real* __restrict__ a) {
    using W = ZW<M, E>;
    using PL = typename W::PL;
    const cplx* ub = reinterpret_cast<const cplx*>(a + z.row_u * W::N2);
    const unsigned voff = (unsigned)((z.rw * M + z.j) * kCB);
#pragma unroll
    for (int q = 0; q < E; ++q) {
        const bool on = OUT ? (PL::slot_out(q) && PL::lane_out(z.j, q)) : (PL::slot_in(q) && PL::lane_in(z.j, q));
        v[q] = (z.valid && on) ? buf_load_c_aux<OFDFT_ZR_LD_AUX>(ub + (OUT ? PL::cout(q) : PL::cin(q)), voff) : mkc(0.0, 0.0);
    }
}
template <int M, int E>
__device__ __forceinline__ void z_store_real(const cplx (&v)[E], const ZLane<M, E>& z, real* __restrict__ a) {
    using W = ZW<M, E>;
    using PL = typename W::PL;
    cplx* ub = reinterpret_cast<cplx*>(a + z.row_u * W::N2);
    const unsigned voff = (unsigned)((z.rw * M + z.j) * kCB);
    if (z.valid) {
#pragma unroll
        for (int q = 0; q < E; ++q)
            if (PL::slot_out(q) && PL::lane_out(z.j, q)) buf_store_c_aux<OFDFT_ZR_ST_AUX>(ub + PL::cout(q), voff, v[q]);
    }
}

__device__ __forceinline__ long long z_spec_off(const SpecGeom& g, long long row, int kz) {
    return kz < g.nzm ? (((long long)(kz >> 3)) * g.nrows + row) * 8 + (kz & 7) : g.main_count + (long long)(kz - g.nzm) * g.nrows + row;
}
template <int M> __device__ __forceinline__ int z_mirror(int k) {
    if constexpr ((M & (M - 1)) == 0) return (M - k) & (M - 1);
    else return k == 0 ? 0 : M - k;
}

template <int M, int E> __device__ __forceinline__ unsigned z_spec_voff(const ZLane<M, E>& z, const SpecGeom& g) {
    return (unsigned)((((long long)(z.j >> 3) * g.nrows + z.rw) * 8 + (z.j & 7)) * kCB);
}
template <int M, int E, int Q> __device__ __forceinline__ long long z_spec_ubase(const ZLane<M, E>& z, const SpecGeom& g) {
    constexpr int bu = (ZW<M, E>::P * Q) >> 3;
    constexpr int kin_u = (ZW<M, E>::P * Q) & 7;
    return ((long long)bu * g.nrows + z.row_u) * 8 + kin_u;
}

template <int M, int E, bool TT = (OFDFT_Z_TWTAB != 0)>
__device__ __forceinline__ void z_forward_store(cplx (&v)[E], const ZLane<M, E>& z, cplx* __restrict__ spec,
                                                const SpecGeom& g, const cplx* __restrict__ twM,
                                                const cplx* __restrict__ twN) {
    using W = ZW<M, E>;
    using PL = typename W::PL;
    constexpr int P = W::P;
    wave_line_fft<M, E, false, TT, z_cx<E>()>(v, z.j, z.mine, twM);
    real cr_m[E], c0r;
    exchange_sync<true>();
    if constexpr (PL::EXACT) {
#pragma unroll
        for (int q = 0; q < E; ++q) z.mine[lpos<PL>(z.j + P * q)] = v[q].x;
        exchange_sync<true>();
#pragma unroll
        for (int q = 0; q < E; ++q) cr_m[q] = z.mine[lpos<PL>((M - (z.j + P * q)) & (M - 1))];
        c0r = z.mine[0];
        exchange_sync<true>();
#pragma unroll
        for (int q = 0; q < E; ++q) z.mine[lpos<PL>(z.j + P * q)] = v[q].y;
        exchange_sync<true>();
        const unsigned voff = z_spec_voff<M, E>(z, g);
        static_for<E>([&](auto qc) {
            constexpr int q = decltype(qc)::value;
            const int k = z.j + P * q;
            const real ci_m = z.mine[lpos<PL>((M - k) & (M - 1))];
            const cplx ev = mkc(0.5 * (v[q].x + cr_m[q]), 0.5 * (v[q].y - ci_m));
            const cplx od = mkc(0.5 * (v[q].y + ci_m), -0.5 * (v[q].x - cr_m[q]));
            const cplx X = cadd(ev, cmul(twN[k], od));
            if (z.valid) buf_store_c_aux<OFDFT_ZS_ST_AUX>(spec + z_spec_ubase<M, E, q>(z, g), voff, X);
        });
    } else {
#pragma unroll
        for (int q = 0; q < E; ++q)
            if (PL::slot_out(q) && PL::lane_out(z.j, q)) z.mine[lpos<PL>(z.j + PL::cout(q))] = v[q].x;
        exchange_sync<true>();
#pragma unroll
        for (int q = 0; q < E; ++q) cr_m[q] = (PL::slot_out(q) && PL::lane_out(z.j, q)) ? z.mine[lpos<PL>(z_mirror<M>(z.j + PL::cout(q)))] : (real)0.0;
        c0r = z.mine[0];
        exchange_sync<true>();
#pragma unroll
        for (int q = 0; q < E; ++q)
            if (PL::slot_out(q) && PL::lane_out(z.j, q)) z.mine[lpos<PL>(z.j + PL::cout(q))] = v[q].y;
        exchange_sync<true>();
#pragma unroll
        for (int q = 0; q < E; ++q) {
            if (!(PL::slot_out(q) && PL::lane_out(z.j, q))) continue;
            const int k = z.j + PL::cout(q);
            const real ci_m = z.mine[lpos<PL>(z_mirror<M>(k))];
            const cplx ev = mkc(0.5 * (v[q].x + cr_m[q]), 0.5 * (v[q].y - ci_m));
            const cplx od = mkc(0.5 * (v[q].y + ci_m), -0.5 * (v[q].x - cr_m[q]));
            const cplx X = cadd(ev, cmul(twN[k], od));
            if (z.valid) spec[z_spec_off(g, z.row, k)] = X;
        }
    }
    if (z.j == 0 && z.valid) {
        const real c0i = z.mine[0];
        spec[z_spec_off(g, z.row, M)] = mkc(c0r - c0i, 0.0);
    }
    exchange_sync<true>();
}

template <int M, int E>
__device__ __forceinline__ void z_issue_row(cplx (&v)[E], real& nyq, const ZLane<M, E>& z, const cplx* __restrict__ spec,
                                            const SpecGeom& g) {
    using PL = typename ZW<M, E>::PL;
    if constexpr (PL::EXACT) {
        const unsigned voff = z_spec_voff<M, E>(z, g);
        static_for<E>([&](auto qc) {
            constexpr int q = decltype(qc)::value;
            v[q] = z.valid ? buf_load_c_aux<OFDFT_ZS_LD_AUX>(spec + z_spec_ubase<M, E, q>(z, g), voff) : mkc(0.0, 0.0);
        });
    } else {
#pragma unroll
        for (int q = 0; q < E; ++q)
            v[q] = (z.valid && PL::slot_in(q) && PL::lane_in(z.j, q)) ? spec[z_spec_off(g, z.row, z.j + PL::cin(q))] : mkc(0.0, 0.0);
    }
    nyq = (z.valid && z.j == 0) ? spec[z_spec_off(g, z.row, M)].x : 0.0;
}

template <int M, int E, bool TT = (OFDFT_Z_TWTAB != 0)>
__device__ __forceinline__ void z_forward_regs(cplx (&v)[E], const ZLane<M, E>& z, const cplx* __restrict__ twM,
                                               const cplx* __restrict__ twN, real& nyq) {
    using W = ZW<M, E>;
    using PL = typename W::PL;
    wave_line_fft<M, E, false, TT, z_cx<E>()>(v, z.j, z.mine, twM);
    real cr_m[E], c0r;
    exchange_sync<true>();
#pragma unroll
    for (int q = 0; q < E; ++q)
        if (PL::slot_out(q) && PL::lane_out(z.j, q)) z.mine[lpos<PL>(z.j + PL::cout(q))] = v[q].x;
    exchange_sync<true>();
#pragma unroll
    for (int q = 0; q < E; ++q) cr_m[q] = (PL::slot_out(q) && PL::lane_out(z.j, q)) ? z.mine[lpos<PL>(z_mirror<M>(z.j + PL::cout(q)))] : (real)0.0;
    c0r = z.mine[0];
    exchange_sync<true>();
#pragma unroll
    for (int q = 0; q < E; ++q)
        if (PL::slot_out(q) && PL::lane_out(z.j, q)) z.mine[lpos<PL>(z.j + PL::cout(q))] = v[q].y;
    exchange_sync<true>();
#pragma unroll
    for (int q = 0; q < E; ++q) {
        if (!(PL::slot_out(q) && PL::lane_out(z.j, q))) continue;
        const int k = z.j + PL::cout(q);
        const real ci_m = z.mine[lpos<PL>(z_mirror<M>(k))];
        const cplx ev = mkc(0.5 * (v[q].x + cr_m[q]), 0.5 * (v[q].y - ci_m));
        const cplx od = mkc(0.5 * (v[q].y + ci_m), -0.5 * (v[q].x - cr_m[q]));
        v[q] = cadd(ev, cmul(twN[k], od));
    }
    nyq = c0r - z.mine[0];
    exchange_sync<true>();
}

template <int M, int E, bool TT = (OFDFT_Z_TWTAB != 0)>
__device__ __forceinline__ void z_inverse_regs(cplx (&v)[E], const ZLane<M, E>& z, const cplx* __restrict__ twM,
                                               const cplx* __restrict__ twN, real nyq) {
    using W = ZW<M, E>;
    using PL = typename W::PL;
    real xr_m[E];
    exchange_sync<true>();
#pragma unroll
    for (int q = 0; q < E; ++q)
        if (PL::slot_in(q) && PL::lane_in(z.j, q)) z.mine[lpos<PL>(z.j + PL::cin(q))] = v[q].x;
    exchange_sync<true>();
#pragma unroll
    for (int q = 0; q < E; ++q) xr_m[q] = (PL::slot_in(q) && PL::lane_in(z.j, q)) ? z.mine[lpos<PL>(z_mirror<M>(z.j + PL::cin(q)))] : (real)0.0;
    exchange_sync<true>();
#pragma unroll
    for (int q = 0; q < E; ++q)
        if (PL::slot_in(q) && PL::lane_in(z.j, q)) z.mine[lpos<PL>(z.j + PL::cin(q))] = v[q].y;
    exchange_sync<true>();
#pragma unroll
    for (int q = 0; q < E; ++q) {
        if (!(PL::slot_in(q) && PL::lane_in(z.j, q))) continue;
        const int k = z.j + PL::cin(q);
        const real xi_m = z.mine[lpos<PL>(z_mirror<M>(k))];
        const cplx x = v[q];
        if (k == 0) {
            v[q] = mkc(x.x + nyq, x.x - nyq);
        } else {
            const cplx ev = mkc(x.x + xr_m[q], x.y - xi_m);
            const cplx d = mkc(x.x - xr_m[q], x.y + xi_m);
            const cplx od = cmul(d, cconj(twN[k]));
            v[q] = mkc(ev.x - od.y, ev.y + od.x);
        }
    }
    exchange_sync<true>();
    wave_line_fft<M, E, true, TT, z_cx<E>()>(v, z.j, z.mine, twM);
    exchange_sync<true>();
    if constexpr (!PL::EXACT) {
#pragma unroll
        for (int q = 0; q < E; ++q)
            if (!(PL::slot_out(q) && PL::lane_out(z.j, q))) v[q] = mkc(0.0, 0.0);
    }
}

template <int M, int E, bool TT = (OFDFT_Z_TWTAB != 0)>
__device__ __forceinline__ void z_load_inverse(cplx (&v)[E], const ZLane<M, E>& z, const cplx* __restrict__ spec,
                                               const SpecGeom& g, const cplx* __restrict__ twM,
                                               const cplx* __restrict__ twN) {
    asm volatile("" ::: "memory");
    __builtin_amdgcn_sched_barrier(0);
    real nyq;
    z_issue_row<M, E>(v, nyq, z, spec, g);
    z_inverse_regs<M, E, TT>(v, z, twM, twN, nyq);
}

template <int M, int E, bool TT = (OFDFT_Z_TWTAB != 0)>
__device__ __forceinline__ void z_deriv_row(cplx (&v)[E], const ZLane<M, E>& z, const cplx* __restrict__ twM,
                                            const cplx* __restrict__ twN) {
    using PL = typename ZW<M, E>::PL;
    real nyq;
    z_forward_regs<M, E, TT>(v, z, twM, twN, nyq);
#pragma unroll
    for (int q = 0; q < E; ++q) {
        const real k = (real)(z.j + PL::cout(q));
        v[q] = mkc(-k * v[q].y, k * v[q].x);
    }
    repattern_out_to_in<PL, true>(v, z.j, z.mine);
    z_inverse_regs<M, E, TT>(v, z, twM, twN, 0.0);
}

__device__ __forceinline__ real pow_pos(real x, real y) { return fm::pow_pos(x, y); }

struct DenSrc {
    const real* src;
    real cscale;
    int from_chi;
    const acc_t* cscale_dev;
    __device__ __forceinline__ real operator()(real x) const {
        const real c = cscale_dev ? (real)*cscale_dev : cscale;
        return from_chi ? c * x * x : x;
    }
    __device__ __forceinline__ DenSrc resolved() const {
        DenSrc r = *this;
        if (cscale_dev) r.cscale = (real)*cscale_dev;
        r.cscale_dev = nullptr;
        return r;
    }
};

template <int M, int E>
__global__ __launch_bounds__(256) void zfwd_w_kernel(const real* __restrict__ in, cplx* __restrict__ spec, SpecGeom g,
                                                     const cplx* __restrict__ twM_g, const cplx* __restrict__ twN_g) {
    extern __shared__ __attribute__((aligned(16))) real lds[];
    const cplx *twM, *twN;
    const ZTwReq<M, E> twq = z_tw_request<M, E>(twM_g, twN_g);
    const ZLane<M, E> z(g, lds);
    cplx v[E];
    z_load_real<M, E>(v, z, in);
    z_tw_commit<M, E>(lds, twq, twM_g, twN_g, twM, twN);
    z_forward_store<M, E>(v, z, spec, g, twM, twN);
}
template <int M, int E>
__global__ __launch_bounds__(256) void zinv_w_kernel(const cplx* __restrict__ spec, real* __restrict__ out, SpecGeom g,
                                                     const cplx* __restrict__ twM_g, const cplx* __restrict__ twN_g, real scale) {
    extern __shared__ __attribute__((aligned(16))) real lds[];
    const cplx *twM, *twN;
    const ZTwReq<M, E> twq = z_tw_request<M, E>(twM_g, twN_g);
    const ZLane<M, E> z(g, lds);
    cplx v[E];
    z_tw_commit<M, E>(lds, twq, twM_g, twN_g, twM, twN);
    z_load_inverse<M, E>(v, z, spec, g, twM, twN);
#pragma unroll
    for (int q = 0; q < E; ++q) v[q] = mkc(v[q].x * scale, v[q].y * scale);
    z_store_real<M, E>(v, z, out);
}

template <int M, int E>
__global__ __launch_bounds__(256, (ZW<M, E>::PL::EXACT ? 3 : 2)) void zf_density_kernel(DenSrc ds, cplx* __restrict__ out_n, cplx* __restrict__ out_s,
                                                         SpecGeom g, const cplx* __restrict__ twM_g,
                                                         const cplx* __restrict__ twN_g, real* __restrict__ dzn = nullptr) {
    extern __shared__ __attribute__((aligned(16))) real lds[];
    const cplx *twM, *twN;
    const ZTwReq<M, E> twq = z_tw_request<M, E>(twM_g, twN_g);
    ds = ds.resolved();
    const ZLane<M, E> z(g, lds);
    cplx x[E], v[E];
    z_load_real<M, E>(x, z, ds.src);
    z_tw_commit<M, E>(lds, twq, twM_g, twN_g, twM, twN);
    if (out_n) {
#pragma unroll
        for (int q = 0; q < E; ++q) v[q] = mkc(ds(x[q].x), ds(x[q].y));
        z_forward_store<M, E>(v, z, out_n, g, twM, twN);
    }
    if (out_s) {
#pragma unroll
        for (int q = 0; q < E; ++q) {
            const real a = ds(x[q].x), b = ds(x[q].y);
            v[q] = mkc(a != 0.0 ? sqrt(a) : 0.0, b != 0.0 ? sqrt(b) : 0.0);
        }
        z_forward_store<M, E>(v, z, out_s, g, twM, twN);
    }
    if (dzn) {
        const real sc = 1.0 / (real)(2 * M);
#pragma unroll
        for (int q = 0; q < E; ++q) v[q] = mkc(ds(x[q].x), ds(x[q].y));
        z_deriv_row<M, E>(v, z, twM, twN);
#pragma unroll
        for (int q = 0; q < E; ++q) v[q] = mkc(v[q].x * sc, v[q].y * sc);
        z_store_real<M, E>(v, z, dzn);
    }
}

struct PowersArgs {
    cplx* out[6];
    real e0, e1, nref;
    int sum53;
};
template <int M, int E, bool ONE = false>
__global__ __launch_bounds__(256, (z_powers_waves<M, E, ONE>())) void zf_powers_kernel(DenSrc ds, PowersArgs pa, SpecGeom g,
                                                        const cplx* __restrict__ twM_g, const cplx* __restrict__ twN_g) {
    extern __shared__ __attribute__((aligned(16))) real lds[];
    const cplx *twM, *twN;
    const ZTwReq<M, E> twq = z_tw_request<M, E>(twM_g, twN_g);
    ds = ds.resolved();
    const ZLane<M, E> z(g, lds);
    cplx n[E], a[E], v[E];
    z_load_real<M, E>(n, z, ds.src);
    z_tw_commit<M, E>(lds, twq, twM_g, twN_g, twM, twN);
    cplx l[E];
#pragma unroll
    for (int q = 0; q < E; ++q) {
        __builtin_amdgcn_sched_barrier(0);
        n[q] = mkc(ds(n[q].x), ds(n[q].y));
        l[q] = mkc(fm::log(n[q].x), fm::log(n[q].y));
        a[q] = mkc(fm::exp(pa.e0 * l[q].x), fm::exp(pa.e0 * l[q].y));
    }
    if constexpr (ONE) {
        z_forward_store<M, E>(a, z, pa.out[0], g, twM, twN);
        return;
    }
    for (int half = 0; half < 2; ++half) {
        if (half == 1) {
            if (!pa.out[3] && !pa.out[4] && !pa.out[5]) break;
#pragma unroll
            for (int q = 0; q < E; ++q) a[q] = mkc(fm::exp(pa.e1 * l[q].x), fm::exp(pa.e1 * l[q].y));
        }
        cplx* const* o = pa.out + 3 * half;
        if (o[0]) {
#pragma unroll
            for (int q = 0; q < E; ++q) v[q] = a[q];
            z_forward_store<M, E>(v, z, o[0], g, twM, twN);
        }
        if (o[1]) {
#pragma unroll
            for (int q = 0; q < E; ++q) v[q] = mkc(a[q].x * (n[q].x - pa.nref), a[q].y * (n[q].y - pa.nref));
            z_forward_store<M, E>(v, z, o[1], g, twM, twN);
        }
        if (o[2]) {
#pragma unroll
            for (int q = 0; q < E; ++q) {
                const real tx = n[q].x - pa.nref, ty = n[q].y - pa.nref;
                v[q] = mkc(0.5 * a[q].x * tx * tx, 0.5 * a[q].y * ty * ty);
            }
            z_forward_store<M, E>(v, z, o[2], g, twM, twN);
        }
    }
}

template <int M, int E>
__global__ __launch_bounds__(256, (z_waves<M, E>(OFDFT_ZPBE_WAVES))) void zpbe_kernel(DenSrc ds, cplx* __restrict__ gx, cplx* __restrict__ gy,
                                                   cplx* __restrict__ gz, real* __restrict__ dfdn, real inv_n,
                                                   GgaSel sel, SpecGeom g, const cplx* __restrict__ twM_g,
                                                   const cplx* __restrict__ twN_g, acc_t* __restrict__ partial) {
    extern __shared__ __attribute__((aligned(16))) real lds[];
    const cplx *twM, *twN;
    const ZTwReq<M, E> twq = z_tw_request<M, E>(twM_g, twN_g);
    ds = ds.resolved();
    const ZLane<M, E> z(g, lds);
    cplx a[E], b[E], c[E], n[E];
    z_tw_commit<M, E>(lds, twq, twM_g, twN_g, twM, twN);
    z_load_inverse<M, E>(a, z, gx, g, twM, twN);
    z_load_inverse<M, E>(b, z, gy, g, twM, twN);
    z_load_inverse<M, E>(c, z, gz, g, twM, twN);
    z_load_real<M, E, true>(n, z, ds.src);
    acc_t acc[kPbeScalars] = {0.0, 0.0, 0.0};
    cplx d[E];
#pragma unroll
    for (int q = 0; q < E; ++q) {
        __builtin_amdgcn_sched_barrier(0);
        const real ax = a[q].x * inv_n, bx = b[q].x * inv_n, cx = c[q].x * inv_n;
        const real ay = a[q].y * inv_n, by = b[q].y * inv_n, cy = c[q].y * inv_n;
        PbePoint p0 = {0, 0, 0, 0, 0}, p1 = {0, 0, 0, 0, 0};
        if (z.valid && ZW<M, E>::PL::slot_out(q) && ZW<M, E>::PL::lane_out(z.j, q)) {
            p0 = pbe_point(ds(n[q].x), ax * ax + bx * bx + cx * cx, sel);
            p1 = pbe_point(ds(n[q].y), ay * ay + by * by + cy * cy, sel);
        }
        acc[0] += p0.fx + p1.fx;
        acc[1] += p0.fc + p1.fc;
        acc[2] += p0.fk + p1.fk;
        d[q] = mkc(p0.dfdn, p1.dfdn);
        a[q] = mkc(p0.dfdg * ax, p1.dfdg * ay);
        b[q] = mkc(p0.dfdg * bx, p1.dfdg * by);
        c[q] = mkc(p0.dfdg * cx, p1.dfdg * cy);
    }
    z_store_real<M, E>(d, z, dfdn);
    using PL = typename ZW<M, E>::PL;
    repattern_out_to_in<PL, true>(a, z.j, z.mine);
    z_forward_store<M, E>(a, z, gx, g, twM, twN);
    repattern_out_to_in<PL, true>(b, z.j, z.mine);
    z_forward_store<M, E>(b, z, gy, g, twM, twN);
    repattern_out_to_in<PL, true>(c, z.j, z.mine);
    z_forward_store<M, E>(c, z, gz, g, twM, twN);
    block_reduce_store<kPbeScalars>(acc, partial + (long long)g.blk0 * kPbeScalars);
}

struct Bmat { real b[9]; };
#ifndef OFDFT_ZPBE_TWTAB
#define OFDFT_ZPBE_TWTAB 1
#endif
constexpr bool kZpbeTT = OFDFT_ZPBE_TWTAB != 0;
template <int M, int E, bool LAPL>
__global__ __launch_bounds__(256, (z_waves<M, E, OFDFT_Z_EMAX_PBE>(2))) void zpbe2_kernel(DenSrc ds, cplx* __restrict__ A, cplx* __restrict__ B,
                                                                      const real* __restrict__ dzn,
                                                                      real* __restrict__ dfdn, real inv_n, real inv_nz,
                                                                      GgaSel sel, Bmat bm, SpecGeom g,
                                                                      const cplx* __restrict__ twM_g,
                                                                      const cplx* __restrict__ twN_g,
                                                                      acc_t* __restrict__ partial, cplx* __restrict__ Lsp) {
    extern __shared__ __attribute__((aligned(16))) real lds[];
    const cplx *twM, *twN;
    const ZTwReq<M, E> twq = z_tw_request<M, E>(twM_g, twN_g);
    ds = ds.resolved();
    const ZLane<M, E> z(g, lds);
    cplx a[E], b[E], c[E], n[E];
    cplx lp[LAPL ? E : 1];
#if OFDFT_Z_PREFETCH
    {
        real nyq_a, nyq_b;
        z_issue_row<M, E>(a, nyq_a, z, A, g);
        z_issue_row<M, E>(b, nyq_b, z, B, g);
        z_tw_commit<M, E>(lds, twq, twM_g, twN_g, twM, twN);
        z_inverse_regs<M, E, kZpbeTT>(a, z, twM, twN, nyq_a);
        if constexpr (LAPL) {
            real nyq_l;
            z_issue_row<M, E>(lp, nyq_l, z, Lsp, g);
            z_inverse_regs<M, E, kZpbeTT>(b, z, twM, twN, nyq_b);
            z_inverse_regs<M, E, kZpbeTT>(lp, z, twM, twN, nyq_l);
        } else {
            z_inverse_regs<M, E, kZpbeTT>(b, z, twM, twN, nyq_b);
        }
    }
#else
    z_tw_commit<M, E>(lds, twq, twM_g, twN_g, twM, twN);
    z_load_inverse<M, E, kZpbeTT>(a, z, A, g, twM, twN);
    z_load_inverse<M, E, kZpbeTT>(b, z, B, g, twM, twN);
    if constexpr (LAPL) z_load_inverse<M, E, kZpbeTT>(lp, z, Lsp, g, twM, twN);
#endif
    z_load_real<M, E, true>(c, z, dzn);
    z_load_real<M, E, true>(n, z, ds.src);
    acc_t acc[kPbeScalars] = {0.0, 0.0, 0.0};
    cplx d[E];
    const bool diag = bm.b[1] == 0.0 && bm.b[2] == 0.0 && bm.b[3] == 0.0 && bm.b[5] == 0.0 && bm.b[6] == 0.0 && bm.b[7] == 0.0;
#pragma unroll
    for (int q = 0; q < E; ++q) {
        __builtin_amdgcn_sched_barrier(0);
        const real da0 = a[q].x * inv_n, db0 = b[q].x * inv_n, dc0 = c[q].x;
        const real da1 = a[q].y * inv_n, db1 = b[q].y * inv_n, dc1 = c[q].y;
        real gx0, gx1, gy0, gy1, gz0, gz1;
        if (diag) {
            gx0 = bm.b[0] * da0; gx1 = bm.b[0] * da1;
            gy0 = bm.b[4] * db0; gy1 = bm.b[4] * db1;
            gz0 = bm.b[8] * dc0; gz1 = bm.b[8] * dc1;
        } else {
            gx0 = bm.b[0] * da0 + bm.b[3] * db0 + bm.b[6] * dc0; gx1 = bm.b[0] * da1 + bm.b[3] * db1 + bm.b[6] * dc1;
            gy0 = bm.b[1] * da0 + bm.b[4] * db0 + bm.b[7] * dc0; gy1 = bm.b[1] * da1 + bm.b[4] * db1 + bm.b[7] * dc1;
            gz0 = bm.b[2] * da0 + bm.b[5] * db0 + bm.b[8] * dc0; gz1 = bm.b[2] * da1 + bm.b[5] * db1 + bm.b[8] * dc1;
        }
        PbePoint p0 = {0, 0, 0, 0, 0}, p1 = {0, 0, 0, 0, 0};
        if constexpr (LAPL) {
            real dl0 = 0.0, dl1 = 0.0;
            if (z.valid && ZW<M, E>::PL::slot_out(q) && ZW<M, E>::PL::lane_out(z.j, q)) {
                GgaSel nk = sel;
                nk.k = 0;
                const real g20 = gx0 * gx0 + gy0 * gy0 + gz0 * gz0, g21 = gx1 * gx1 + gy1 * gy1 + gz1 * gz1;
                p0 = pbe_point(ds(n[q].x), g20, nk);
                p1 = pbe_point(ds(n[q].y), g21, nk);
                pg_laplacian_point(ds(n[q].x), g20, lp[q].x * inv_n, sel, p0, dl0);
                pg_laplacian_point(ds(n[q].y), g21, lp[q].y * inv_n, sel, p1, dl1);
            }
            lp[q] = mkc(dl0, dl1);
        } else if (z.valid && ZW<M, E>::PL::slot_out(q) && ZW<M, E>::PL::lane_out(z.j, q)) {
            p0 = pbe_point(ds(n[q].x), gx0 * gx0 + gy0 * gy0 + gz0 * gz0, sel);
            p1 = pbe_point(ds(n[q].y), gx1 * gx1 + gy1 * gy1 + gz1 * gz1, sel);
        }
        acc[0] += p0.fx + p1.fx;
        acc[1] += p0.fc + p1.fc;
        acc[2] += p0.fk + p1.fk;
        d[q] = mkc(p0.dfdn, p1.dfdn);
        if (diag) {
            a[q] = mkc(p0.dfdg * (bm.b[0] * gx0), p1.dfdg * (bm.b[0] * gx1));
            b[q] = mkc(p0.dfdg * (bm.b[4] * gy0), p1.dfdg * (bm.b[4] * gy1));
            c[q] = mkc(p0.dfdg * (bm.b[8] * gz0), p1.dfdg * (bm.b[8] * gz1));
        } else {
            a[q] = mkc(p0.dfdg * (bm.b[0] * gx0 + bm.b[1] * gy0 + bm.b[2] * gz0),
                       p1.dfdg * (bm.b[0] * gx1 + bm.b[1] * gy1 + bm.b[2] * gz1));
            b[q] = mkc(p0.dfdg * (bm.b[3] * gx0 + bm.b[4] * gy0 + bm.b[5] * gz0),
                       p1.dfdg * (bm.b[3] * gx1 + bm.b[4] * gy1 + bm.b[5] * gz1));
            c[q] = mkc(p0.dfdg * (bm.b[6] * gx0 + bm.b[7] * gy0 + bm.b[8] * gz0),
                       p1.dfdg * (bm.b[6] * gx1 + bm.b[7] * gy1 + bm.b[8] * gz1));
        }
    }
    using PL = typename ZW<M, E>::PL;
    repattern_out_to_in<PL, true>(a, z.j, z.mine);
    z_forward_store<M, E, kZpbeTT>(a, z, A, g, twM, twN);
    repattern_out_to_in<PL, true>(b, z.j, z.mine);
    z_forward_store<M, E, kZpbeTT>(b, z, B, g, twM, twN);
    if constexpr (LAPL) {
        repattern_out_to_in<PL, true>(lp, z.j, z.mine);
        z_forward_store<M, E, kZpbeTT>(lp, z, Lsp, g, twM, twN);
    }
    repattern_out_to_in<PL, true>(c, z.j, z.mine);
    z_deriv_row<M, E, kZpbeTT>(c, z, twM, twN);
#pragma unroll
    for (int q = 0; q < E; ++q) d[q] = mkc(d[q].x - 2.0 * inv_nz * c[q].x, d[q].y - 2.0 * inv_nz * c[q].y);
    z_store_real<M, E>(d, z, dfdn);
    block_reduce_store<kPbeScalars>(acc, partial + (long long)g.blk0 * kPbeScalars);
}

struct ZCombineArgs {
    DenSrc ds;
    const real* vext;
    const real* dfdn;
    const cplx* vh;
    const cplx* lap;
    const cplx* conv_b;
    const cplx* conv_a;
    const cplx* u[3];
    const cplx* gw[3];
    const cplx* div;
    const cplx* div2;
    const acc_t* eh_part;
    long long eh_rows;
    real* v_out;
    const real* v_part;
    int v_part_deferred;
    unsigned mask;
    real inv_n;
    TermConsts tc;
    const acc_t* wts_w;
};

template <int M, int E>
__device__ __forceinline__ real wgc_row_section(const cplx (&n)[E], cplx (&vacc)[E], cplx (&w)[E], const ZLane<M, E>& z,
                                                  const ZCombineArgs& a, const SpecGeom& g, const cplx* __restrict__ twM,
                                                  const cplx* __restrict__ twN, real sc, real ctf) {
    cplx t1[E], t2[E];
    real e = 0.0;
#if OFDFT_Z_PREFETCH
    cplx nx[E];
    real nyq_nx, nyq_w;
    z_issue_row<M, E>(nx, nyq_nx, z, a.u[0], g);
#define OFDFT_ZROW(cur, nxt)                                                          \
    {                                                                                 \
        _Pragma("unroll") for (int q = 0; q < E; ++q) w[q] = nx[q];                   \
        nyq_w = nyq_nx;                                                               \
        if ((nxt) != nullptr) z_issue_row<M, E>(nx, nyq_nx, z, (nxt), g);             \
        z_inverse_regs<M, E>(w, z, twM, twN, nyq_w);                                  \
    }
#else
#define OFDFT_ZROW(cur, nxt) z_load_inverse<M, E>(w, z, (cur), g, twM, twN);
#endif
    OFDFT_ZROW(a.u[0], a.u[1])
#pragma unroll
    for (int q = 0; q < E; ++q) t1[q] = mkc(w[q].x * sc, w[q].y * sc);
    OFDFT_ZROW(a.u[1], a.u[2])
#pragma unroll
    for (int q = 0; q < E; ++q) {
        const real x0 = w[q].x * sc, x1 = w[q].y * sc;
        t1[q].x += (n[q].x - a.tc.nref) * x0;
        t1[q].y += (n[q].y - a.tc.nref) * x1;
        t2[q] = mkc(x0, x1);
    }
    OFDFT_ZROW(a.u[2], a.gw[0])
#pragma unroll
    for (int q = 0; q < E; ++q) {
        __builtin_amdgcn_sched_barrier(0);
        const real x0 = w[q].x * sc, x1 = w[q].y * sc;
        const real h0 = n[q].x - a.tc.nref, h1 = n[q].y - a.tc.nref;
        t1[q].x += 0.5 * h0 * h0 * x0;
        t1[q].y += 0.5 * h1 * h1 * x1;
        t2[q].x += h0 * x0;
        t2[q].y += h1 * x1;
        const real l0 = fm::log(n[q].x), l1 = fm::log(n[q].y);
        const real pb0 = fm::exp((a.tc.wgc_beta - 1.0) * l0), pb1 = fm::exp((a.tc.wgc_beta - 1.0) * l1);
        const real pa0 = fm::exp((a.tc.wgc_alpha - 1.0) * l0), pa1 = fm::exp((a.tc.wgc_alpha - 1.0) * l1);
        e += ctf * (pa0 * n[q].x * t1[q].x + pa1 * n[q].y * t1[q].y);
        vacc[q].x += ctf * pa0 * (a.tc.wgc_alpha * t1[q].x + n[q].x * t2[q].x);
        vacc[q].y += ctf * pa1 * (a.tc.wgc_alpha * t1[q].y + n[q].y * t2[q].y);
        t2[q] = mkc(pb0, pb1);
    }
    OFDFT_ZROW(a.gw[0], a.gw[1])
#pragma unroll
    for (int q = 0; q < E; ++q) t1[q] = mkc(a.tc.wgc_beta * w[q].x * sc, a.tc.wgc_beta * w[q].y * sc);
    OFDFT_ZROW(a.gw[1], a.gw[2])
#pragma unroll
    for (int q = 0; q < E; ++q) {
        t1[q].x += (a.tc.wgc_beta * (n[q].x - a.tc.nref) + n[q].x) * w[q].x * sc;
        t1[q].y += (a.tc.wgc_beta * (n[q].y - a.tc.nref) + n[q].y) * w[q].y * sc;
    }
    OFDFT_ZROW(a.gw[2], nullptr)
#pragma unroll
    for (int q = 0; q < E; ++q) {
        const real h0 = n[q].x - a.tc.nref, h1 = n[q].y - a.tc.nref;
        t1[q].x += (0.5 * a.tc.wgc_beta * h0 * h0 + n[q].x * h0) * w[q].x * sc;
        t1[q].y += (0.5 * a.tc.wgc_beta * h1 * h1 + n[q].y * h1) * w[q].y * sc;
        vacc[q].x += ctf * t2[q].x * t1[q].x;
        vacc[q].y += ctf * t2[q].y * t1[q].y;
    }
#undef OFDFT_ZROW
    return e;
}

constexpr int kParkIe = 0, kParkH = 1, kParkVw = 2, kParkWt = 3, kParkWgc = 4, kParkSlots = 5;
#ifndef OFDFT_ZI_WAVES_BIG_F32
#define OFDFT_ZI_WAVES_BIG_F32 4
#endif
template <int M, int E, bool WGC_INLINE> constexpr int zi_combine_waves() {
    if (sizeof(real) == 4 && M >= 512 && E <= 8 && !WGC_INLINE) return OFDFT_ZI_WAVES_BIG_F32;
    return z_waves<M, E>(2);
}
template <int M, int E, bool WGC_INLINE>
__global__ __launch_bounds__(256, (zi_combine_waves<M, E, WGC_INLINE>())) void zi_combine_kernel(ZCombineArgs a, SpecGeom g, const cplx* __restrict__ twM_g,
                                                         const cplx* __restrict__ twN_g, acc_t* __restrict__ partial) {
    extern __shared__ __attribute__((aligned(16))) real lds[];
    const cplx *twM, *twN;
    const ZTwReq<M, E> twq = z_tw_request<M, E>(twM_g, twN_g);
    a.ds = a.ds.resolved();
    const ZLane<M, E> z(g, lds);
    const real ctf = kCtf;
    real* park = lds + ZW<M, E>::LDS / sizeof(real) + threadIdx.x;
#pragma unroll
    for (int s = 0; s < kParkSlots; ++s) park[s * 256] = 0.0;
    cplx n[E], vacc[E], w[E];
    z_load_real<M, E, true>(n, z, a.ds.src);
    z_tw_commit<M, E>(lds, twq, twM_g, twN_g, twM, twN);
    using PL = typename ZW<M, E>::PL;
#pragma unroll
    for (int q = 0; q < E; ++q) {
        n[q] = (z.valid && PL::slot_out(q) && PL::lane_out(z.j, q)) ? mkc(a.ds(n[q].x), a.ds(n[q].y)) : mkc(1.0, 1.0);
        vacc[q] = mkc(0.0, 0.0);
    }
    const real sc = a.inv_n;
    const real w_tf = a.wts_w ? (real)a.wts_w[0] : (real)1.0, w_nl = a.wts_w ? (real)a.wts_w[1] : (real)1.0;
    constexpr unsigned kRootTerms = 4u | 8u | 16u | (0xFu << 6) | (1u << 13);
    constexpr bool ROOTS_ONCE = OFDFT_ZI_ROOTS_ONCE != 0;
    cplx yv[ROOTS_ONCE ? E : 1];
    if constexpr (ROOTS_ONCE) {
        if (a.mask & kRootTerms) {
#pragma unroll
            for (int q = 0; q < E; ++q)
                yv[q] = mkc(n[q].x != 0.0 ? fm::rsixth(n[q].x) : (real)0.0, n[q].y != 0.0 ? fm::rsixth(n[q].y) : (real)0.0);
        }
    }
    auto root_y = [&](int q, int c) -> real {
        if constexpr (ROOTS_ONCE) return c ? yv[q].y : yv[q].x;
        else {
            const real nn = c ? n[q].y : n[q].x;
            return nn != 0.0 ? fm::rsixth(nn) : (real)0.0;
        }
    };
    constexpr bool PIPE = OFDFT_Z_PREFETCH && !WGC_INLINE && (M < 512 || (sizeof(real) == 4 && OFDFT_Z_PIPE_BIG_F32));
    const bool gga = (a.mask & (7u << 10)) != 0;
    const cplx* chain[6] = {(a.mask & 2u) ? a.vh : nullptr,  (a.mask & 8u) ? a.lap : nullptr, (a.mask & 16u) ? a.conv_b : nullptr,
                            (a.mask & 16u) ? a.conv_a : nullptr, gga ? a.div : nullptr, gga ? a.div2 : nullptr};
    cplx nx[PIPE ? E : 1];
    real nyq_nx = 0.0;
    auto request_after = [&](auto ic) {
        constexpr int I = decltype(ic)::value;
        const cplx* p = nullptr;
#pragma unroll
        for (int k = 5; k > I; --k)
            if (chain[k]) p = chain[k];
        if constexpr (PIPE)
            if (p) z_issue_row<M, E>(nx, nyq_nx, z, p, g);
    };
    auto take_row = [&](auto ic, const cplx* spec) {
        if constexpr (PIPE) {
#pragma unroll
            for (int q = 0; q < E; ++q) w[q] = nx[q];
            const real nyq_w = nyq_nx;
            request_after(ic);
            z_inverse_regs<M, E>(w, z, twM, twN, nyq_w);
        } else {
            z_load_inverse<M, E>(w, z, spec, g, twM, twN);
        }
    };
    request_after(std::integral_constant<int, -1>{});
    if ((a.mask & 2u) && a.vh) {
        take_row(std::integral_constant<int, 0>{}, a.vh);
        real e = 0.0;
#pragma unroll
        for (int q = 0; q < E; ++q) {
            const real x0 = w[q].x * sc, x1 = w[q].y * sc;
            e += 0.5 * (n[q].x * x0 + n[q].y * x1);
            vacc[q].x += x0;
            vacc[q].y += x1;
        }
        park[kParkH * 256] = e;
    }
    if (a.mask & 8u) {
        take_row(std::integral_constant<int, 1>{}, a.lap);
        real e = 0.0;
#pragma unroll
        for (int q = 0; q < E; ++q) {
            __builtin_amdgcn_sched_barrier(0);
            const real x0 = w[q].x * sc, x1 = w[q].y * sc;
            const real y0 = root_y(q, 0), y1 = root_y(q, 1);
            const real r0 = y0 * y0 * y0, r1 = y1 * y1 * y1;
            e += -0.5 * (n[q].x * r0 * x0 + n[q].y * r1 * x1);
            vacc[q].x += -0.5 * x0 * r0;
            vacc[q].y += -0.5 * x1 * r1;
        }
        park[kParkVw * 256] = e;
    }
    if (a.mask & 16u) {
        take_row(std::integral_constant<int, 2>{}, a.conv_b);
        cplx pa1[E];
        real e = 0.0;
#pragma unroll
        for (int q = 0; q < E; ++q) {
            __builtin_amdgcn_sched_barrier(0);
            const real x0 = w[q].x * sc, x1 = w[q].y * sc;
            pa1[q] = a.tc.wt_is_56 ? mkc(root_y(q, 0), root_y(q, 1)) : mkc(pow_pos(n[q].x, a.tc.wt_alpha - 1.0), pow_pos(n[q].y, a.tc.wt_alpha - 1.0));
            e += ctf * ((pa1[q].x * n[q].x - a.tc.wt_nbar_pa) * x0 + (pa1[q].y * n[q].y - a.tc.wt_nbar_pa) * x1);
            const real f = w_nl * (a.conv_a ? a.tc.wt_alpha : 2.0 * a.tc.wt_alpha);
            vacc[q].x += ctf * f * pa1[q].x * x0;
            vacc[q].y += ctf * f * pa1[q].y * x1;
        }
        park[kParkWt * 256] = e;
        if (a.conv_a) {
            take_row(std::integral_constant<int, 3>{}, a.conv_a);
            if (a.tc.wt_sym) {
                real e2 = 0.0;
#pragma unroll
                for (int q = 0; q < E; ++q) {
                    const real p0 = ctf * pow_pos(n[q].x, a.tc.wt_beta - 1.0) * w[q].x * sc, p1 = ctf * pow_pos(n[q].y, a.tc.wt_beta - 1.0) * w[q].y * sc;
                    e2 += p0 * n[q].x + p1 * n[q].y;
                    vacc[q].x += w_nl * a.tc.wt_beta * p0;
                    vacc[q].y += w_nl * a.tc.wt_beta * p1;
                }
                park[kParkWt * 256] = (real)0.5 * (park[kParkWt * 256] + e2);
            } else {
#pragma unroll
                for (int q = 0; q < E; ++q) {
                    vacc[q].x += w_nl * ctf * a.tc.wt_beta * pow_pos(n[q].x, a.tc.wt_beta - 1.0) * w[q].x * sc;
                    vacc[q].y += w_nl * ctf * a.tc.wt_beta * pow_pos(n[q].y, a.tc.wt_beta - 1.0) * w[q].y * sc;
                }
            }
        }
    }
    if (a.mask & 32u) {
        if (WGC_INLINE) {
            park[kParkWgc * 256] = wgc_row_section<M, E>(n, vacc, w, z, a, g, twM, twN, sc, ctf);
        } else if (!a.v_part_deferred) {
            z_load_real<M, E, true>(w, z, a.v_part);
#pragma unroll
            for (int q = 0; q < E; ++q) {
                vacc[q].x += w[q].x;
                vacc[q].y += w[q].y;
            }
        }
    }
    if (a.mask & (7u << 10)) {
        take_row(std::integral_constant<int, 4>{}, a.div);
        cplx d[E];
        z_load_real<M, E, true>(d, z, a.dfdn);
#pragma unroll
        for (int q = 0; q < E; ++q) {
            vacc[q].x += d[q].x - 2.0 * w[q].x * sc;
            vacc[q].y += d[q].y - 2.0 * w[q].y * sc;
        }
        if (a.div2) {
            take_row(std::integral_constant<int, 5>{}, a.div2);
#pragma unroll
            for (int q = 0; q < E; ++q) {
                vacc[q].x -= 2.0 * w[q].x * sc;
                vacc[q].y -= 2.0 * w[q].y * sc;
            }
        }
    }
    if (a.mask & 1u) {
        cplx ve[E];
        z_load_real<M, E, true>(ve, z, a.vext);
        real e = 0.0;
#pragma unroll
        for (int q = 0; q < E; ++q) {
            e += n[q].x * ve[q].x + n[q].y * ve[q].y;
            vacc[q].x += ve[q].x;
            vacc[q].y += ve[q].y;
        }
        park[kParkIe * 256] = e;
    }
    acc_t acc[kCombineScalars];
#pragma unroll
    for (int s = 0; s < kCombineScalars; ++s) acc[s] = 0.0;
#pragma unroll
    for (int q = 0; q < E; ++q) {
        __builtin_amdgcn_sched_barrier(0);
        if (!(PL::slot_out(q) && PL::lane_out(z.j, q))) continue;
        const fm::Roots<real> rt0 = fm::roots_from_y(n[q].x, root_y(q, 0)), rt1 = fm::roots_from_y(n[q].y, root_y(q, 1));
        if (a.mask & 4u) {
            const real c0 = rt0.n13, c1 = rt1.n13;
            acc[2] += ctf * (c0 * c0 * n[q].x + c1 * c1 * n[q].y);
            vacc[q].x += w_tf * (5.0 / 3.0) * ctf * c0 * c0;
            vacc[q].y += w_tf * (5.0 / 3.0) * ctf * c1 * c1;
        }
        if (a.mask & (1u << 13)) {
            real e0, v0, e1, v1;
            vwgtf_point(n[q].x, rt0.n13, ctf, a.tc.gtf_inv_n0, a.tc.gtf_kind, e0, v0);
            vwgtf_point(n[q].y, rt1.n13, ctf, a.tc.gtf_inv_n0, a.tc.gtf_kind, e1, v1);
            acc[9] += e0 + e1;
            vacc[q].x += v0;
            vacc[q].y += v1;
        }
        if (a.mask & (0xFu << 6)) {
            const XcLocal x0 = lda_point(n[q].x, a.mask, rt0), x1 = lda_point(n[q].y, a.mask, rt1);
            acc[6] += x0.ex + x1.ex;
            acc[7] += x0.ec + x1.ec;
            vacc[q].x += x0.vx + x0.vc;
            vacc[q].y += x1.vx + x1.vc;
        }
        acc[8] += vacc[q].x * n[q].x + vacc[q].y * n[q].y;
    }
    acc[0] = park[kParkIe * 256];
    acc[1] = park[kParkH * 256];
    acc[3] = park[kParkVw * 256];
    acc[4] = park[kParkWt * 256];
    acc[5] = park[kParkWgc * 256];
    if (!z.valid) {
#pragma unroll
        for (int s = 0; s < kCombineScalars; ++s) acc[s] = 0.0;
    }
    if (a.eh_part && g.blk0 + blockIdx.x == 0) {
        for (long long i = threadIdx.x; i < a.eh_rows; i += blockDim.x) acc[1] += a.eh_part[i];
    }
    if (a.v_out) z_store_real<M, E>(vacc, z, a.v_out);
    block_reduce_store<kCombineScalars>(acc, partial + (long long)g.blk0 * kCombineScalars);
}

template <int M, int E>
__global__ __launch_bounds__(256, (z_waves<M, E>(OFDFT_ZIWGC_WAVES))) void zi_wgc_kernel(ZCombineArgs a, real* __restrict__ v_part, SpecGeom g,
                                                       const cplx* __restrict__ twM_g, const cplx* __restrict__ twN_g,
                                                       acc_t* __restrict__ partial) {
    extern __shared__ __attribute__((aligned(16))) real lds[];
    const cplx *twM, *twN;
    const ZTwReq<M, E> twq = z_tw_request<M, E>(twM_g, twN_g);
    a.ds = a.ds.resolved();
    const ZLane<M, E> z(g, lds);
    const real ctf = kCtf;
    cplx n[E], vacc[E], w[E];
    z_load_real<M, E, true>(n, z, a.ds.src);
    z_tw_commit<M, E>(lds, twq, twM_g, twN_g, twM, twN);
    using PL = typename ZW<M, E>::PL;
#pragma unroll
    for (int q = 0; q < E; ++q) {
        n[q] = (z.valid && PL::slot_out(q) && PL::lane_out(z.j, q)) ? mkc(a.ds(n[q].x), a.ds(n[q].y)) : mkc(1.0, 1.0);
        vacc[q] = mkc(0.0, 0.0);
    }
    acc_t acc[2];
    acc[0] = wgc_row_section<M, E>(n, vacc, w, z, a, g, twM, twN, a.inv_n, ctf);
    acc[1] = 0.0;
#pragma unroll
    for (int q = 0; q < E; ++q)
        if (PL::slot_out(q) && PL::lane_out(z.j, q)) acc[1] += vacc[q].x * n[q].x + vacc[q].y * n[q].y;
    if (!z.valid) acc[0] = acc[1] = 0.0;
    z_store_real<M, E>(vacc, z, v_part);
    block_reduce_store<2>(acc, partial + (long long)g.blk0 * 2);
}

}
```

Measured before the change: 423.3 evals/s.

## Process multiple z-row tiles per workgroup with next-tile prefetch in z kernels

Adds a tile plan so each z-pass workgroup loops over several row tiles (persistent-style), with an option to pick tiles per workgroup or a fixed grid size. Loads for the next tile are issued before the current tile's FFT and stores, to overlap memory latency with compute. The twiddle-table commit and block reduction are amortised over tiles. It also disables machine LICM for zfused.hip. With the default auto value of one tile per workgroup the launch shape is unchanged, but the loop structure and prefetch still change the code paths and register pressure.

```diff
diff --git a/include/ofdft_hip.h b/include/ofdft_hip.h
--- a/include/ofdft_hip.h
+++ b/include/ofdft_hip.h
@@ -166,6 +166,7 @@
 #define OFDFT_OPT_BS_FUSED 15
 #define OFDFT_OPT_POT_SPECTRUM 16
 #define OFDFT_OPT_AXIS_PASSES 17
+#define OFDFT_OPT_Z_TILES 18
 #define OFDFT_OPT_WGC_FOLD 28
 #define OFDFT_OPT_XWAVE 8
 int  ofdft_set_option(ofdft_ctx* ctx, int option, double value);
diff --git a/professad_amd/_build.py b/professad_amd/_build.py
--- a/professad_amd/_build.py
+++ b/professad_amd/_build.py
@@ -10,6 +10,7 @@
 LIB = os.path.join(LIBDIR, 'libofdft_hip.so')
 LIB_F32 = os.path.join(LIBDIR, 'libofdft_hip_f32.so')
 SOURCES = ['engine.hip', 'lines.hip', 'xpass_a.hip', 'xpass_b.hip', 'zfused.hip', 'resident.hip']
+SOURCE_FLAGS = {'zfused.hip': ['-mllvm', '-disable-machine-licm']}
 HEADERS = sorted(f for f in os.listdir(CSRC) if f.endswith('.h')) + [os.path.join('..', '..', 'include', 'ofdft_hip.h')]
 
 
@@ -39,7 +40,7 @@
     for src in SOURCES:
         obj = os.path.join(objdir, '%s.%s.o' % (tag, src))
         objs.append(obj)
-        cmd = [hipcc] + _flags(extra_flags) + ['-c', os.path.join(CSRC, src), '-o', obj]
+        cmd = [hipcc] + _flags(extra_flags) + SOURCE_FLAGS.get(src, []) + ['-c', os.path.join(CSRC, src), '-o', obj]
         if verbose:
             print(' '.join(cmd), flush=True)
         jobs.append((cmd, subprocess.Popen(cmd)))
diff --git a/professad_amd/_native.py b/professad_amd/_native.py
--- a/professad_amd/_native.py
+++ b/professad_amd/_native.py
@@ -43,6 +43,7 @@
 OPT_BS_FUSED = 15
 OPT_POT_SPECTRUM = 16
 OPT_AXIS_PASSES = 17
+OPT_Z_TILES = 18
 OPT_WGC_FOLD = 28
 
 EXPORTS = ['ofdft_create', 'ofdft_destroy', 'ofdft_last_error', 'ofdft_set_cell', 'ofdft_set_terms',
diff --git a/professad_amd/csrc/engine.hip b/professad_amd/csrc/engine.hip
--- a/professad_amd/csrc/engine.hip
+++ b/professad_amd/csrc/engine.hip
@@ -1635,6 +1635,10 @@
             if (value != 0.0 && value != 1.0 && value != 2.0 && value != 3.0) return fail(c, OFDFT_EINVAL, "OFDFT_OPT_AXIS_PASSES takes 0..3");
             c->axis_passes = (int)value;
             return OFDFT_OK;
+        case OFDFT_OPT_Z_TILES:
+            if (value != (double)(int)value || value > 64.0 || value < -65536.0) return fail(c, OFDFT_EINVAL, "OFDFT_OPT_Z_TILES takes 0 (automatic), 1..64 tiles per workgroup or -n for exactly n workgroups");
+            c->z_tiles = (int)value;
+            return OFDFT_OK;
         case OFDFT_OPT_SPLIT_COMBINE:
             c->split_combine = value != 0.0;
             c->defer_vpart = value != 1.0;
diff --git a/professad_amd/csrc/engine_ctx.h b/professad_amd/csrc/engine_ctx.h
--- a/professad_amd/csrc/engine_ctx.h
+++ b/professad_amd/csrc/engine_ctx.h
@@ -77,6 +77,7 @@
     bool gga_split = true;
     bool pot_spectrum = true;
     int axis_passes = 3;
+    int z_tiles = 0;
     bool split_combine = true;
     bool defer_vpart = true;
     int ybatch = 1;
@@ -333,6 +334,11 @@
     for (int k = 0; k <= c->xc.n; ++k) c->xc.kb[k] = (int)((long long)c->xg.nb * k / c->xc.n);
 }
 
+#ifndef OFDFT_Z_TILES_AUTO
+#define OFDFT_Z_TILES_AUTO 1
+#endif
+inline int z_tiles_auto() { return OFDFT_Z_TILES_AUTO; }
+
 inline bool cell_axes_orthogonal(const ofdft_ctx* c) {
     const real* bb = c->kg.b;
     return bb[1] == 0.0 && bb[2] == 0.0 && bb[3] == 0.0 && bb[5] == 0.0 && bb[6] == 0.0 && bb[7] == 0.0;
diff --git a/professad_amd/csrc/fft_kernels.h b/professad_amd/csrc/fft_kernels.h
--- a/professad_amd/csrc/fft_kernels.h
+++ b/professad_amd/csrc/fft_kernels.h
@@ -6,6 +6,7 @@
 struct SpecGeom {
     int n0, n1, n2, nzc, nzm;
     int blk0 = 0;
+    int tq = 1, trem = 0, tend = 0;
     long long nrows;
     long long main_count;
     long long total;
diff --git a/professad_amd/csrc/zfused.hip b/professad_amd/csrc/zfused.hip
--- a/professad_amd/csrc/zfused.hip
+++ b/professad_amd/csrc/zfused.hip
@@ -21,6 +21,25 @@
 }
 template <int M, int E> int z_blocks(const ofdft_ctx* c) { return (int)((c->g.nrows + ZW<M, E>::RPB - 1) / ZW<M, E>::RPB); }
 
+static int z_tile_plan(const ofdft_ctx* c, SpecGeom& g, int first, int tiles, int nchunks) {
+    int v = nchunks > 1 ? 1 : c->z_tiles;
+    if (v == 0) v = z_tiles_auto();
+    int grid;
+    if (v > 0) {
+        const int k = v < tiles ? v : tiles;
+        grid = (tiles + k - 1) / k;
+        g.tq = k;
+        g.trem = 0;
+    } else {
+        grid = -v < tiles ? -v : tiles;
+        g.tq = tiles / grid;
+        g.trem = tiles % grid;
+    }
+    g.blk0 = first;
+    g.tend = first + tiles;
+    return grid;
+}
+
 int launch_zf_density(ofdft_ctx* c, const DenSrc& ds, cplx* out_n, cplx* out_s, hipStream_t st, int chunk,
                       int nchunks, real* dzn) {
     cplx *twM, *twN;
@@ -29,8 +48,8 @@
     SpecGeom gz = c->g;
 #define X(M_)                                                                                                       \
     case M_: {                                                                                                      \
-        const int nb = z_blocks<M_, ZPick<M_, 8>::E>(c) / nchunks;                                                  \
-        gz.blk0 = chunk * nb;                                                                                       \
+        const int nt = z_blocks<M_, ZPick<M_, 8>::E>(c) / nchunks;                                                  \
+        const int nb = z_tile_plan(c, gz, chunk * nt, nt, nchunks);                                                 \
         OFDFT_LAUNCH(c, st, "zf_density", (zf_density_kernel<M_, ZPick<M_, 8>::E>), dim3(nb), dim3(256),            \
                      (ZW<M_, ZPick<M_, 8>::E>::LDS), ds, out_n, out_s, gz, twM, twN, dzn);                          \
         return 0;                                                                                                   \
@@ -48,8 +67,8 @@
     SpecGeom gz = c->g;
 #define X(M_)                                                                                                      \
     case M_: {                                                                                                     \
-        const int nb = z_blocks<M_, ZPick<M_, EZP>::E>(c) / nchunks;                                                \
-        gz.blk0 = chunk * nb;                                                                                      \
+        const int nt = z_blocks<M_, ZPick<M_, EZP>::E>(c) / nchunks;                                                \
+        const int nb = z_tile_plan(c, gz, chunk * nt, nt, nchunks);                                                \
         if (pa.out[0] && !pa.out[1] && !pa.out[2] && !pa.out[3] && !pa.out[4] && !pa.out[5])                       \
             OFDFT_LAUNCH(c, st, "zf_powers", (zf_powers_kernel<M_, ZPick<M_, EZP>::E, true>), dim3(nb), dim3(256), \
                          (ZW<M_, ZPick<M_, EZP>::E>::LDS), ds, pa, gz, twM, twN);                                   \
@@ -91,17 +110,18 @@
     c->fft_count += L ? 8 : 6;
     Bmat bm{};
     std::memcpy(bm.b, c->kg.b, sizeof(bm.b));
+    SpecGeom gq = c->g;
 #define X(M_)                                                                                                   \
     case M_: {                                                                                                  \
-        *blocks_out = z_blocks<M_, ZPick<M_, EZ>::E>(c);                                                        \
+        *blocks_out = z_tile_plan(c, gq, 0, z_blocks<M_, ZPick<M_, EZ>::E>(c), 1);    \
         if (L)                                                                                                  \
             OFDFT_LAUNCH(c, st, "zpbe", (zpbe2_kernel<M_, ZPick<M_, EZ>::E, true>), dim3(*blocks_out), dim3(256), \
                          (ZW<M_, ZPick<M_, EZ>::E>::LDS), ds, A, B, dzn, dfdn, inv_n, 1.0 / (double)c->n2, gga_sel(c), bm, \
-                         c->g, twM, twN, c->d_partial, L);                                                      \
+                         gq, twM, twN, c->d_partial, L);                                                        \
         else                                                                                                    \
             OFDFT_LAUNCH(c, st, "zpbe", (zpbe2_kernel<M_, ZPick<M_, EZ>::E, false>), dim3(*blocks_out), dim3(256), \
                          (ZW<M_, ZPick<M_, EZ>::E>::LDS), ds, A, B, dzn, dfdn, inv_n, 1.0 / (double)c->n2, gga_sel(c), bm, \
-                         c->g, twM, twN, c->d_partial, L);                                                      \
+                         gq, twM, twN, c->d_partial, L);                                                        \
         return 0;                                                                                               \
     }
     switch (c->n2 / 2) { OFDFT_ZCASES(X) }
@@ -117,15 +137,15 @@
 #define X(M_)                                                                                                     \
     case M_: {                                                                                                    \
         using W = ZW<M_, ZPick<M_, EZ>::E>;                                                                       \
-        *blocks_out = z_blocks<M_, W::E>(c);                                                                      \
-        const int nb = *blocks_out / nchunks;                                                                     \
-        gq.blk0 = chunk * nb;                                                                                     \
+        const int nt = z_blocks<M_, W::E>(c) / nchunks;                                                           \
+        const int nb = z_tile_plan(c, gq, chunk * nt, nt, nchunks);                                               \
+        *blocks_out = nb * nchunks;           \
         if (a.v_part || !(a.mask & OFDFT_WGC99_NL))     \
             OFDFT_LAUNCH(c, st, "zi_combine", (zi_combine_kernel<M_, W::E, false>), dim3(nb), dim3(256),          \
                          (W::LDS + park), a, gq, twM, twN, c->d_partial);                                         \
         else                                                                                                      \
             OFDFT_LAUNCH(c, st, "zi_combine", (zi_combine_kernel<M_, W::E, true>), dim3(nb), dim3(256),           \
-                         (W::LDS + park), a, gq, twM, twN, c->d_partial);                                         \
+                         (W::LDS + park + sizeof(acc_t) * 256 * 5), a, gq, twM, twN, c->d_partial);               \
         return 0;                                                                                                 \
     }
     switch (c->n2 / 2) { OFDFT_ZCASES(X) }
@@ -136,12 +156,13 @@
 int launch_zi_wgc(ofdft_ctx* c, const ZCombineArgs& a, real* v_part, double* partial, int* blocks_out, hipStream_t st) {
     cplx *twM, *twN;
     if (int rc = z_tables(c, &twM, &twN)) return rc;
+    SpecGeom gq = c->g;
 #define X(M_)                                                                                                     \
     case M_: {                                                                                                    \
         using W = ZW<M_, ZPick<M_, EZ>::E>;                                                                       \
-        *blocks_out = z_blocks<M_, W::E>(c);                                                                      \
+        *blocks_out = z_tile_plan(c, gq, 0, z_blocks<M_, W::E>(c), 1);                                            \
         OFDFT_LAUNCH(c, st, "zi_wgc", (zi_wgc_kernel<M_, W::E>), dim3(*blocks_out), dim3(256), (W::LDS), a, v_part, \
-                     c->g, twM, twN, partial);                                                                    \
+                     gq, twM, twN, partial);                                                                    \
         return 0;                                                                                                 \
     }
     switch (c->n2 / 2) { OFDFT_ZCASES(X) }
diff --git a/professad_amd/csrc/zpass.h b/professad_amd/csrc/zpass.h
--- a/professad_amd/csrc/zpass.h
+++ b/professad_amd/csrc/zpass.h
@@ -20,6 +20,9 @@
 #endif
 #ifndef OFDFT_Z_LDS_TWIDDLES
 #define OFDFT_Z_LDS_TWIDDLES 1
+#endif
+#ifndef OFDFT_ZT_PREFETCH
+#define OFDFT_ZT_PREFETCH 31
 #endif
 
 #ifndef OFDFT_Z_CX
@@ -64,6 +67,18 @@
     return 4;
 }
 
+struct ZTiles {
+    int first, count;
+    __device__ __forceinline__ explicit ZTiles(const SpecGeom& g) {
+        const int b = (int)blockIdx.x;
+        first = g.blk0 + b * g.tq + (b < g.trem ? b : g.trem);
+        const int want = g.tq + (b < g.trem ? 1 : 0), left = g.tend - first;
+        count = g.tend == 0 ? 1 : (want < left ? want : left);
+        first = __builtin_amdgcn_readfirstlane(first);
+        count = __builtin_amdgcn_readfirstlane(count);
+    }
+};
+
 template <int M, int E> struct ZLane {
     int j;
     int rw;
@@ -71,18 +86,31 @@
     long long row;
     bool valid;
     real* mine;
-    __device__ __forceinline__ ZLane(const SpecGeom& g, real* lds) {
+    real* base;
+    __device__ __forceinline__ ZLane(const SpecGeom& g, real* lds) : ZLane(g, lds, (int)blockIdx.x + g.blk0) {}
+    __device__ __forceinline__ ZLane(const SpecGeom& g, real* lds, int tile, bool on = true) {
         using W = ZW<M, E>;
         const int lane = threadIdx.x & 63;
         const int wave = __builtin_amdgcn_readfirstlane((int)(threadIdx.x >> 6));
         j = lane % W::P;
         rw = lane / W::P;
-        row_u = uniform64((long long)(blockIdx.x + g.blk0) * W::RPB + (long long)wave * W::RPWV);
+        base = lds;
+        mine = lds + (wave * W::RPWV + rw) * W::RS;
+        row_u = uniform64((long long)tile * W::RPB + (long long)wave * W::RPWV);
         row = row_u + rw;
-        valid = row < g.nrows;
-        mine = lds + (wave * W::RPWV + rw) * W::RS;
-    }
-    __device__ __forceinline__ ZLane(int j_, int rw_, real* mine_, bool valid_) : j(j_), rw(rw_), row_u(0), row(rw_), valid(valid_), mine(mine_) {}
+        valid = on && row < g.nrows;
+    }
+    __device__ __forceinline__ ZLane next(const SpecGeom& g, bool on) const {
+        using W = ZW<M, E>;
+        ZLane n = *this;
+        asm volatile("" : "+v"(n.j), "+v"(n.rw));
+        n.mine = base + (__builtin_amdgcn_readfirstlane((int)(threadIdx.x >> 6)) * W::RPWV + n.rw) * W::RS;
+        n.row_u = uniform64(row_u + W::RPB);
+        n.row = n.row_u + rw;
+        n.valid = on && n.row < g.nrows;
+        return n;
+    }
+    __device__ __forceinline__ ZLane(int j_, int rw_, real* mine_, bool valid_) : j(j_), rw(rw_), row_u(0), row(rw_), valid(valid_), mine(mine_), base(nullptr) {}
 };
 
 template <int M, int E> struct ZTwReq {
@@ -402,31 +430,42 @@
     const cplx *twM, *twN;
     const ZTwReq<M, E> twq = z_tw_request<M, E>(twM_g, twN_g);
     ds = ds.resolved();
-    const ZLane<M, E> z(g, lds);
+    constexpr bool XP = ZW<M, E>::PL::EXACT && (OFDFT_ZT_PREFETCH & 1) != 0;
+    const ZTiles tl(g);
+    ZLane<M, E> z(g, lds, tl.first);
     cplx x[E], v[E];
     z_load_real<M, E>(x, z, ds.src);
     z_tw_commit<M, E>(lds, twq, twM_g, twN_g, twM, twN);
-    if (out_n) {
-#pragma unroll
-        for (int q = 0; q < E; ++q) v[q] = mkc(ds(x[q].x), ds(x[q].y));
-        z_forward_store<M, E>(v, z, out_n, g, twM, twN);
-    }
-    if (out_s) {
-#pragma unroll
-        for (int q = 0; q < E; ++q) {
-            const real a = ds(x[q].x), b = ds(x[q].y);
-            v[q] = mkc(a != 0.0 ? sqrt(a) : 0.0, b != 0.0 ? sqrt(b) : 0.0);
-        }
-        z_forward_store<M, E>(v, z, out_s, g, twM, twN);
-    }
-    if (dzn) {
-        const real sc = 1.0 / (real)(2 * M);
-#pragma unroll
-        for (int q = 0; q < E; ++q) v[q] = mkc(ds(x[q].x), ds(x[q].y));
-        z_deriv_row<M, E>(v, z, twM, twN);
-#pragma unroll
-        for (int q = 0; q < E; ++q) v[q] = mkc(v[q].x * sc, v[q].y * sc);
-        z_store_real<M, E>(v, z, dzn);
+    const int last = dzn ? 2 : (out_s ? 1 : 0);
+    for (int t = 0; t < tl.count; ++t) {
+        const ZLane<M, E> zn = z.next(g, t + 1 < tl.count);
+        if (t > 0 && !XP) z_load_real<M, E>(x, z, ds.src);
+        if (out_n) {
+#pragma unroll
+            for (int q = 0; q < E; ++q) v[q] = mkc(ds(x[q].x), ds(x[q].y));
+            if (XP && last == 0) z_load_real<M, E>(x, zn, ds.src);
+            z_forward_store<M, E>(v, z, out_n, g, twM, twN);
+        }
+        if (out_s) {
+#pragma unroll
+            for (int q = 0; q < E; ++q) {
+                const real a = ds(x[q].x), b = ds(x[q].y);
+                v[q] = mkc(a != 0.0 ? sqrt(a) : 0.0, b != 0.0 ? sqrt(b) : 0.0);
+            }
+            if (XP && last == 1) z_load_real<M, E>(x, zn, ds.src);
+            z_forward_store<M, E>(v, z, out_s, g, twM, twN);
+        }
+        if (dzn) {
+            const real sc = 1.0 / (real)(2 * M);
+#pragma unroll
+            for (int q = 0; q < E; ++q) v[q] = mkc(ds(x[q].x), ds(x[q].y));
+            if (XP) z_load_real<M, E>(x, zn, ds.src);
+            z_deriv_row<M, E>(v, z, twM, twN);
+#pragma unroll
+            for (int q = 0; q < E; ++q) v[q] = mkc(v[q].x * sc, v[q].y * sc);
+            z_store_real<M, E>(v, z, dzn);
+        }
+        z = zn;
     }
 }
 
@@ -442,47 +481,62 @@
     const cplx *twM, *twN;
     const ZTwReq<M, E> twq = z_tw_request<M, E>(twM_g, twN_g);
     ds = ds.resolved();
-    const ZLane<M, E> z(g, lds);
+    constexpr bool XP = ZW<M, E>::PL::EXACT && (OFDFT_ZT_PREFETCH & 2) != 0;
+    const ZTiles tl(g);
+    ZLane<M, E> z(g, lds, tl.first);
     cplx n[E], a[E], v[E];
     z_load_real<M, E>(n, z, ds.src);
     z_tw_commit<M, E>(lds, twq, twM_g, twN_g, twM, twN);
-    cplx l[E];
-#pragma unroll
-    for (int q = 0; q < E; ++q) {
-        __builtin_amdgcn_sched_barrier(0);
-        n[q] = mkc(ds(n[q].x), ds(n[q].y));
-        l[q] = mkc(fm::log(n[q].x), fm::log(n[q].y));
-        a[q] = mkc(fm::exp(pa.e0 * l[q].x), fm::exp(pa.e0 * l[q].y));
-    }
-    if constexpr (ONE) {
-        z_forward_store<M, E>(a, z, pa.out[0], g, twM, twN);
-        return;
-    }
-    for (int half = 0; half < 2; ++half) {
-        if (half == 1) {
-            if (!pa.out[3] && !pa.out[4] && !pa.out[5]) break;
-#pragma unroll
-            for (int q = 0; q < E; ++q) a[q] = mkc(fm::exp(pa.e1 * l[q].x), fm::exp(pa.e1 * l[q].y));
-        }
-        cplx* const* o = pa.out + 3 * half;
-        if (o[0]) {
-#pragma unroll
-            for (int q = 0; q < E; ++q) v[q] = a[q];
-            z_forward_store<M, E>(v, z, o[0], g, twM, twN);
-        }
-        if (o[1]) {
-#pragma unroll
-            for (int q = 0; q < E; ++q) v[q] = mkc(a[q].x * (n[q].x - pa.nref), a[q].y * (n[q].y - pa.nref));
-            z_forward_store<M, E>(v, z, o[1], g, twM, twN);
-        }
-        if (o[2]) {
-#pragma unroll
-            for (int q = 0; q < E; ++q) {
-                const real tx = n[q].x - pa.nref, ty = n[q].y - pa.nref;
-                v[q] = mkc(0.5 * a[q].x * tx * tx, 0.5 * a[q].y * ty * ty);
-            }
-            z_forward_store<M, E>(v, z, o[2], g, twM, twN);
-        }
+    int last = 0;
+#pragma unroll
+    for (int i = 1; i < 6; ++i)
+        if (pa.out[i]) last = i;
+    for (int t = 0; t < tl.count; ++t) {
+        const ZLane<M, E> zn = z.next(g, t + 1 < tl.count);
+        if (t > 0 && !XP) z_load_real<M, E>(n, z, ds.src);
+        cplx l[E];
+#pragma unroll
+        for (int q = 0; q < E; ++q) {
+            __builtin_amdgcn_sched_barrier(0);
+            n[q] = mkc(ds(n[q].x), ds(n[q].y));
+            l[q] = mkc(fm::log(n[q].x), fm::log(n[q].y));
+            a[q] = mkc(fm::exp(pa.e0 * l[q].x), fm::exp(pa.e0 * l[q].y));
+        }
+        if constexpr (ONE) {
+            if (XP) z_load_real<M, E>(n, zn, ds.src);
+            z_forward_store<M, E>(a, z, pa.out[0], g, twM, twN);
+        } else {
+            for (int half = 0; half < 2; ++half) {
+                if (half == 1) {
+                    if (!pa.out[3] && !pa.out[4] && !pa.out[5]) break;
+#pragma unroll
+                    for (int q = 0; q < E; ++q) a[q] = mkc(fm::exp(pa.e1 * l[q].x), fm::exp(pa.e1 * l[q].y));
+                }
+                cplx* const* o = pa.out + 3 * half;
+                if (o[0]) {
+#pragma unroll
+                    for (int q = 0; q < E; ++q) v[q] = a[q];
+                    if (XP && last == 3 * half) z_load_real<M, E>(n, zn, ds.src);
+                    z_forward_store<M, E>(v, z, o[0], g, twM, twN);
+                }
+                if (o[1]) {
+#pragma unroll
+                    for (int q = 0; q < E; ++q) v[q] = mkc(a[q].x * (n[q].x - pa.nref), a[q].y * (n[q].y - pa.nref));
+                    if (XP && last == 3 * half + 1) z_load_real<M, E>(n, zn, ds.src);
+                    z_forward_store<M, E>(v, z, o[1], g, twM, twN);
+                }
+                if (o[2]) {
+#pragma unroll
+                    for (int q = 0; q < E; ++q) {
+                        const real tx = n[q].x - pa.nref, ty = n[q].y - pa.nref;
+                        v[q] = mkc(0.5 * a[q].x * tx * tx, 0.5 * a[q].y * ty * ty);
+                    }
+                    if (XP && last == 3 * half + 2) z_load_real<M, E>(n, zn, ds.src);
+                    z_forward_store<M, E>(v, z, o[2], g, twM, twN);
+                }
+            }
+        }
+        z = zn;
     }
 }
 
@@ -550,15 +604,30 @@
     const cplx *twM, *twN;
     const ZTwReq<M, E> twq = z_tw_request<M, E>(twM_g, twN_g);
     ds = ds.resolved();
-    const ZLane<M, E> z(g, lds);
+    constexpr bool XP = OFDFT_Z_PREFETCH && !LAPL && ZW<M, E>::PL::EXACT && (OFDFT_ZT_PREFETCH & 4) != 0;
+    const ZTiles tl(g);
+    ZLane<M, E> z(g, lds, tl.first);
     cplx a[E], b[E], c[E], n[E];
     cplx lp[LAPL ? E : 1];
+    real nyq_a, nyq_b;
 #if OFDFT_Z_PREFETCH
-    {
-        real nyq_a, nyq_b;
-        z_issue_row<M, E>(a, nyq_a, z, A, g);
-        z_issue_row<M, E>(b, nyq_b, z, B, g);
-        z_tw_commit<M, E>(lds, twq, twM_g, twN_g, twM, twN);
+    z_issue_row<M, E>(a, nyq_a, z, A, g);
+    z_issue_row<M, E>(b, nyq_b, z, B, g);
+#endif
+    z_tw_commit<M, E>(lds, twq, twM_g, twN_g, twM, twN);
+    if constexpr (XP) {
+        z_load_real<M, E, true>(c, z, dzn);
+        z_load_real<M, E, true>(n, z, ds.src);
+    }
+    acc_t acc[kPbeScalars] = {0.0, 0.0, 0.0};
+    const bool diag = bm.b[1] == 0.0 && bm.b[2] == 0.0 && bm.b[3] == 0.0 && bm.b[5] == 0.0 && bm.b[6] == 0.0 && bm.b[7] == 0.0;
+    for (int t = 0; t < tl.count; ++t) {
+        const ZLane<M, E> zn = z.next(g, t + 1 < tl.count);
+#if OFDFT_Z_PREFETCH
+        if (t > 0 && !XP) {
+            z_issue_row<M, E>(a, nyq_a, z, A, g);
+            z_issue_row<M, E>(b, nyq_b, z, B, g);
+        }
         z_inverse_regs<M, E, kZpbeTT>(a, z, twM, twN, nyq_a);
         if constexpr (LAPL) {
             real nyq_l;
@@ -568,81 +637,85 @@
         } else {
             z_inverse_regs<M, E, kZpbeTT>(b, z, twM, twN, nyq_b);
         }
-    }
 #else
-    z_tw_commit<M, E>(lds, twq, twM_g, twN_g, twM, twN);
-    z_load_inverse<M, E, kZpbeTT>(a, z, A, g, twM, twN);
-    z_load_inverse<M, E, kZpbeTT>(b, z, B, g, twM, twN);
-    if constexpr (LAPL) z_load_inverse<M, E, kZpbeTT>(lp, z, Lsp, g, twM, twN);
-#endif
-    z_load_real<M, E, true>(c, z, dzn);
-    z_load_real<M, E, true>(n, z, ds.src);
-    acc_t acc[kPbeScalars] = {0.0, 0.0, 0.0};
-    cplx d[E];
-    const bool diag = bm.b[1] == 0.0 && bm.b[2] == 0.0 && bm.b[3] == 0.0 && bm.b[5] == 0.0 && bm.b[6] == 0.0 && bm.b[7] == 0.0;
-#pragma unroll
-    for (int q = 0; q < E; ++q) {
-        __builtin_amdgcn_sched_barrier(0);
-        const real da0 = a[q].x * inv_n, db0 = b[q].x * inv_n, dc0 = c[q].x;
-        const real da1 = a[q].y * inv_n, db1 = b[q].y * inv_n, dc1 = c[q].y;
-        real gx0, gx1, gy0, gy1, gz0, gz1;
-        if (diag) {
-            gx0 = bm.b[0] * da0; gx1 = bm.b[0] * da1;
-            gy0 = bm.b[4] * db0; gy1 = bm.b[4] * db1;
-            gz0 = bm.b[8] * dc0; gz1 = bm.b[8] * dc1;
-        } else {
-            gx0 = bm.b[0] * da0 + bm.b[3] * db0 + bm.b[6] * dc0; gx1 = bm.b[0] * da1 + bm.b[3] * db1 + bm.b[6] * dc1;
-            gy0 = bm.b[1] * da0 + bm.b[4] * db0 + bm.b[7] * dc0; gy1 = bm.b[1] * da1 + bm.b[4] * db1 + bm.b[7] * dc1;
-            gz0 = bm.b[2] * da0 + bm.b[5] * db0 + bm.b[8] * dc0; gz1 = bm.b[2] * da1 + bm.b[5] * db1 + bm.b[8] * dc1;
-        }
-        PbePoint p0 = {0, 0, 0, 0, 0}, p1 = {0, 0, 0, 0, 0};
+        z_load_inverse<M, E, kZpbeTT>(a, z, A, g, twM, twN);
+        z_load_inverse<M, E, kZpbeTT>(b, z, B, g, twM, twN);
+        if constexpr (LAPL) z_load_inverse<M, E, kZpbeTT>(lp, z, Lsp, g, twM, twN);
+#endif
+        if constexpr (!XP) {
+            z_load_real<M, E, true>(c, z, dzn);
+            z_load_real<M, E, true>(n, z, ds.src);
+        }
+        cplx d[E];
+#pragma unroll
+        for (int q = 0; q < E; ++q) {
+            __builtin_amdgcn_sched_barrier(0);
+            const real da0 = a[q].x * inv_n, db0 = b[q].x * inv_n, dc0 = c[q].x;
+            const real da1 = a[q].y * inv_n, db1 = b[q].y * inv_n, dc1 = c[q].y;
+            real gx0, gx1, gy0, gy1, gz0, gz1;
+            if (diag) {
+                gx0 = bm.b[0] * da0; gx1 = bm.b[0] * da1;
+                gy0 = bm.b[4] * db0; gy1 = bm.b[4] * db1;
+                gz0 = bm.b[8] * dc0; gz1 = bm.b[8] * dc1;
+            } else {
+                gx0 = bm.b[0] * da0 + bm.b[3] * db0 + bm.b[6] * dc0; gx1 = bm.b[0] * da1 + bm.b[3] * db1 + bm.b[6] * dc1;
+                gy0 = bm.b[1] * da0 + bm.b[4] * db0 + bm.b[7] * dc0; gy1 = bm.b[1] * da1 + bm.b[4] * db1 + bm.b[7] * dc1;
+                gz0 = bm.b[2] * da0 + bm.b[5] * db0 + bm.b[8] * dc0; gz1 = bm.b[2] * da1 + bm.b[5] * db1 + bm.b[8] * dc1;
+            }
+            PbePoint p0 = {0, 0, 0, 0, 0}, p1 = {0, 0, 0, 0, 0};
+            if constexpr (LAPL) {
+                real dl0 = 0.0, dl1 = 0.0;
+                if (z.valid && ZW<M, E>::PL::slot_out(q) && ZW<M, E>::PL::lane_out(z.j, q)) {
+                    GgaSel nk = sel;
+                    nk.k = 0;
+                    const real g20 = gx0 * gx0 + gy0 * gy0 + gz0 * gz0, g21 = gx1 * gx1 + gy1 * gy1 + gz1 * gz1;
+                    p0 = pbe_point(ds(n[q].x), g20, nk);
+                    p1 = pbe_point(ds(n[q].y), g21, nk);
+                    pg_laplacian_point(ds(n[q].x), g20, lp[q].x * inv_n, sel, p0, dl0);
+                    pg_laplacian_point(ds(n[q].y), g21, lp[q].y * inv_n, sel, p1, dl1);
+                }
+                lp[q] = mkc(dl0, dl1);
+            } else if (z.valid && ZW<M, E>::PL::slot_out(q) && ZW<M, E>::PL::lane_out(z.j, q)) {
+                p0 = pbe_point(ds(n[q].x), gx0 * gx0 + gy0 * gy0 + gz0 * gz0, sel);
+                p1 = pbe_point(ds(n[q].y), gx1 * gx1 + gy1 * gy1 + gz1 * gz1, sel);
+            }
+            acc[0] += p0.fx + p1.fx;
+            acc[1] += p0.fc + p1.fc;
+            acc[2] += p0.fk + p1.fk;
+            d[q] = mkc(p0.dfdn, p1.dfdn);
+            if (diag) {
+                a[q] = mkc(p0.dfdg * (bm.b[0] * gx0), p1.dfdg * (bm.b[0] * gx1));
+                b[q] = mkc(p0.dfdg * (bm.b[4] * gy0), p1.dfdg * (bm.b[4] * gy1));
+                c[q] = mkc(p0.dfdg * (bm.b[8] * gz0), p1.dfdg * (bm.b[8] * gz1));
+            } else {
+                a[q] = mkc(p0.dfdg * (bm.b[0] * gx0 + bm.b[1] * gy0 + bm.b[2] * gz0),
+                           p1.dfdg * (bm.b[0] * gx1 + bm.b[1] * gy1 + bm.b[2] * gz1));
+                b[q] = mkc(p0.dfdg * (bm.b[3] * gx0 + bm.b[4] * gy0 + bm.b[5] * gz0),
+                           p1.dfdg * (bm.b[3] * gx1 + bm.b[4] * gy1 + bm.b[5] * gz1));
+                c[q] = mkc(p0.dfdg * (bm.b[6] * gx0 + bm.b[7] * gy0 + bm.b[8] * gz0),
+                           p1.dfdg * (bm.b[6] * gx1 + bm.b[7] * gy1 + bm.b[8] * gz1));
+            }
+        }
+        using PL = typename ZW<M, E>::PL;
+        repattern_out_to_in<PL, true>(a, z.j, z.mine);
+        z_forward_store<M, E, kZpbeTT>(a, z, A, g, twM, twN);
+        if constexpr (XP) z_issue_row<M, E>(a, nyq_a, zn, A, g);
+        repattern_out_to_in<PL, true>(b, z.j, z.mine);
+        z_forward_store<M, E, kZpbeTT>(b, z, B, g, twM, twN);
+        if constexpr (XP) z_issue_row<M, E>(b, nyq_b, zn, B, g);
         if constexpr (LAPL) {
-            real dl0 = 0.0, dl1 = 0.0;
-            if (z.valid && ZW<M, E>::PL::slot_out(q) && ZW<M, E>::PL::lane_out(z.j, q)) {
-                GgaSel nk = sel;
-                nk.k = 0;
-                const real g20 = gx0 * gx0 + gy0 * gy0 + gz0 * gz0, g21 = gx1 * gx1 + gy1 * gy1 + gz1 * gz1;
-                p0 = pbe_point(ds(n[q].x), g20, nk);
-                p1 = pbe_point(ds(n[q].y), g21, nk);
-                pg_laplacian_point(ds(n[q].x), g20, lp[q].x * inv_n, sel, p0, dl0);
-                pg_laplacian_point(ds(n[q].y), g21, lp[q].y * inv_n, sel, p1, dl1);
-            }
-            lp[q] = mkc(dl0, dl1);
-        } else if (z.valid && ZW<M, E>::PL::slot_out(q) && ZW<M, E>::PL::lane_out(z.j, q)) {
-            p0 = pbe_point(ds(n[q].x), gx0 * gx0 + gy0 * gy0 + gz0 * gz0, sel);
-            p1 = pbe_point(ds(n[q].y), gx1 * gx1 + gy1 * gy1 + gz1 * gz1, sel);
-        }
-        acc[0] += p0.fx + p1.fx;
-        acc[1] += p0.fc + p1.fc;
-        acc[2] += p0.fk + p1.fk;
-        d[q] = mkc(p0.dfdn, p1.dfdn);
-        if (diag) {
-            a[q] = mkc(p0.dfdg * (bm.b[0] * gx0), p1.dfdg * (bm.b[0] * gx1));
-            b[q] = mkc(p0.dfdg * (bm.b[4] * gy0), p1.dfdg * (bm.b[4] * gy1));
-            c[q] = mkc(p0.dfdg * (bm.b[8] * gz0), p1.dfdg * (bm.b[8] * gz1));
-        } else {
-            a[q] = mkc(p0.dfdg * (bm.b[0] * gx0 + bm.b[1] * gy0 + bm.b[2] * gz0),
-                       p1.dfdg * (bm.b[0] * gx1 + bm.b[1] * gy1 + bm.b[2] * gz1));
-            b[q] = mkc(p0.dfdg * (bm.b[3] * gx0 + bm.b[4] * gy0 + bm.b[5] * gz0),
-                       p1.dfdg * (bm.b[3] * gx1 + bm.b[4] * gy1 + bm.b[5] * gz1));
-            c[q] = mkc(p0.dfdg * (bm.b[6] * gx0 + bm.b[7] * gy0 + bm.b[8] * gz0),
-                       p1.dfdg * (bm.b[6] * gx1 + bm.b[7] * gy1 + bm.b[8] * gz1));
-        }
-    }
-    using PL = typename ZW<M, E>::PL;
-    repattern_out_to_in<PL, true>(a, z.j, z.mine);
-    z_forward_store<M, E, kZpbeTT>(a, z, A, g, twM, twN);
-    repattern_out_to_in<PL, true>(b, z.j, z.mine);
-    z_forward_store<M, E, kZpbeTT>(b, z, B, g, twM, twN);
-    if constexpr (LAPL) {
-        repattern_out_to_in<PL, true>(lp, z.j, z.mine);
-        z_forward_store<M, E, kZpbeTT>(lp, z, Lsp, g, twM, twN);
-    }
-    repattern_out_to_in<PL, true>(c, z.j, z.mine);
-    z_deriv_row<M, E, kZpbeTT>(c, z, twM, twN);
-#pragma unroll
-    for (int q = 0; q < E; ++q) d[q] = mkc(d[q].x - 2.0 * inv_nz * c[q].x, d[q].y - 2.0 * inv_nz * c[q].y);
-    z_store_real<M, E>(d, z, dfdn);
+            repattern_out_to_in<PL, true>(lp, z.j, z.mine);
+            z_forward_store<M, E, kZpbeTT>(lp, z, Lsp, g, twM, twN);
+        }
+        if constexpr (XP) z_load_real<M, E, true>(n, zn, ds.src);
+        repattern_out_to_in<PL, true>(c, z.j, z.mine);
+        z_deriv_row<M, E, kZpbeTT>(c, z, twM, twN);
+#pragma unroll
+        for (int q = 0; q < E; ++q) d[q] = mkc(d[q].x - 2.0 * inv_nz * c[q].x, d[q].y - 2.0 * inv_nz * c[q].y);
+        if constexpr (XP) z_load_real<M, E, true>(c, zn, dzn);
+        z_store_real<M, E>(d, z, dfdn);
+        z = zn;
+    }
     block_reduce_store<kPbeScalars>(acc, partial + (long long)g.blk0 * kPbeScalars);
 }
 
@@ -670,20 +743,26 @@
 };
 
 template <int M, int E>
+__device__ __forceinline__ void wgc_first_row(cplx (&nx)[E], real& nyq_nx, const ZLane<M, E>& z, const ZCombineArgs& a, const SpecGeom& g) {
+#if OFDFT_Z_PREFETCH
+    z_issue_row<M, E>(nx, nyq_nx, z, a.u[0], g);
+#endif
+}
+template <int M, int E, bool XP>
 __device__ __forceinline__ real wgc_row_section(const cplx (&n)[E], cplx (&vacc)[E], cplx (&w)[E], const ZLane<M, E>& z,
                                                   const ZCombineArgs& a, const SpecGeom& g, const cplx* __restrict__ twM,
-                                                  const cplx* __restrict__ twN, real sc, real ctf) {
+                                                  const cplx* __restrict__ twN, real sc, real ctf, cplx (&nx)[E], real& nyq_nx,
+                                                  const ZLane<M, E>& zn) {
     cplx t1[E], t2[E];
     real e = 0.0;
 #if OFDFT_Z_PREFETCH
-    cplx nx[E];
-    real nyq_nx, nyq_w;
-    z_issue_row<M, E>(nx, nyq_nx, z, a.u[0], g);
+    real nyq_w;
 #define OFDFT_ZROW(cur, nxt)                                                          \
     {                                                                                 \
         _Pragma("unroll") for (int q = 0; q < E; ++q) w[q] = nx[q];                   \
         nyq_w = nyq_nx;                                                               \
         if ((nxt) != nullptr) z_issue_row<M, E>(nx, nyq_nx, z, (nxt), g);             \
+        else if (XP) z_issue_row<M, E>(nx, nyq_nx, zn, a.u[0], g);                    \
         z_inverse_regs<M, E>(w, z, twM, twN, nyq_w);                                  \
     }
 #else
@@ -746,6 +825,7 @@
 #endif
 template <int M, int E, bool WGC_INLINE> constexpr int zi_combine_waves() {
     if (sizeof(real) == 4 && M >= 512 && E <= 8 && !WGC_INLINE) return OFDFT_ZI_WAVES_BIG_F32;
+    if (sizeof(real) == 8 && M < 512 && E <= 4 && !WGC_INLINE) return 3;
     return z_waves<M, E>(2);
 }
 template <int M, int E, bool WGC_INLINE>
@@ -755,7 +835,9 @@
     const cplx *twM, *twN;
     const ZTwReq<M, E> twq = z_tw_request<M, E>(twM_g, twN_g);
     a.ds = a.ds.resolved();
-    const ZLane<M, E> z(g, lds);
+    constexpr bool XP = !WGC_INLINE && ZW<M, E>::PL::EXACT && (OFDFT_ZT_PREFETCH & 8) != 0;
+    const ZTiles tl(g);
+    ZLane<M, E> z(g, lds, tl.first);
     const real ctf = kCtf;
     real* park = lds + ZW<M, E>::LDS / sizeof(real) + threadIdx.x;
 #pragma unroll
@@ -764,206 +846,239 @@
     z_load_real<M, E, true>(n, z, a.ds.src);
     z_tw_commit<M, E>(lds, twq, twM_g, twN_g, twM, twN);
     using PL = typename ZW<M, E>::PL;
-#pragma unroll
-    for (int q = 0; q < E; ++q) {
-        n[q] = (z.valid && PL::slot_out(q) && PL::lane_out(z.j, q)) ? mkc(a.ds(n[q].x), a.ds(n[q].y)) : mkc(1.0, 1.0);
-        vacc[q] = mkc(0.0, 0.0);
-    }
     const real sc = a.inv_n;
     const real w_tf = a.wts_w ? (real)a.wts_w[0] : (real)1.0, w_nl = a.wts_w ? (real)a.wts_w[1] : (real)1.0;
     constexpr unsigned kRootTerms = 4u | 8u | 16u | (0xFu << 6) | (1u << 13);
     constexpr bool ROOTS_ONCE = OFDFT_ZI_ROOTS_ONCE != 0;
     cplx yv[ROOTS_ONCE ? E : 1];
-    if constexpr (ROOTS_ONCE) {
-        if (a.mask & kRootTerms) {
-#pragma unroll
-            for (int q = 0; q < E; ++q)
-                yv[q] = mkc(n[q].x != 0.0 ? fm::rsixth(n[q].x) : (real)0.0, n[q].y != 0.0 ? fm::rsixth(n[q].y) : (real)0.0);
-        }
-    }
-    auto root_y = [&](int q, int c) -> real {
-        if constexpr (ROOTS_ONCE) return c ? yv[q].y : yv[q].x;
-        else {
-            const real nn = c ? n[q].y : n[q].x;
-            return nn != 0.0 ? fm::rsixth(nn) : (real)0.0;
-        }
-    };
     constexpr bool PIPE = OFDFT_Z_PREFETCH && !WGC_INLINE && (M < 512 || (sizeof(real) == 4 && OFDFT_Z_PIPE_BIG_F32));
     const bool gga = (a.mask & (7u << 10)) != 0;
     const cplx* chain[6] = {(a.mask & 2u) ? a.vh : nullptr,  (a.mask & 8u) ? a.lap : nullptr, (a.mask & 16u) ? a.conv_b : nullptr,
                             (a.mask & 16u) ? a.conv_a : nullptr, gga ? a.div : nullptr, gga ? a.div2 : nullptr};
     cplx nx[PIPE ? E : 1];
     real nyq_nx = 0.0;
-    auto request_after = [&](auto ic) {
-        constexpr int I = decltype(ic)::value;
-        const cplx* p = nullptr;
-#pragma unroll
-        for (int k = 5; k > I; --k)
-            if (chain[k]) p = chain[k];
-        if constexpr (PIPE)
-            if (p) z_issue_row<M, E>(nx, nyq_nx, z, p, g);
-    };
-    auto take_row = [&](auto ic, const cplx* spec) {
-        if constexpr (PIPE) {
-#pragma unroll
-            for (int q = 0; q < E; ++q) w[q] = nx[q];
-            const real nyq_w = nyq_nx;
-            request_after(ic);
-            z_inverse_regs<M, E>(w, z, twM, twN, nyq_w);
-        } else {
-            z_load_inverse<M, E>(w, z, spec, g, twM, twN);
-        }
-    };
-    request_after(std::integral_constant<int, -1>{});
-    if ((a.mask & 2u) && a.vh) {
-        take_row(std::integral_constant<int, 0>{}, a.vh);
-        real e = 0.0;
+    const cplx* first_spec = nullptr;
+#pragma unroll
+    for (int k = 5; k >= 0; --k)
+        if (chain[k]) first_spec = chain[k];
+    if constexpr (PIPE)
+        if (XP && first_spec) z_issue_row<M, E>(nx, nyq_nx, z, first_spec, g);
+    acc_t acc[kCombineScalars];
+#pragma unroll
+    for (int s = 0; s < kCombineScalars; ++s) acc[s] = 0.0;
+    constexpr int kLocalSlot[5] = {2, 6, 7, 8, 9};
+    acc_t* lpark = reinterpret_cast<acc_t*>(lds + ZW<M, E>::LDS / sizeof(real) + 256 * kParkSlots) + threadIdx.x;
+    if constexpr (WGC_INLINE) {
+#pragma unroll
+        for (int s = 0; s < 5; ++s) lpark[s * 256] = 0.0;
+    }
+    for (int t = 0; t < tl.count; ++t) {
+        const ZLane<M, E> zn = z.next(g, t + 1 < tl.count);
+        if (t > 0 && !XP) z_load_real<M, E, true>(n, z, a.ds.src);
 #pragma unroll
         for (int q = 0; q < E; ++q) {
-            const real x0 = w[q].x * sc, x1 = w[q].y * sc;
-            e += 0.5 * (n[q].x * x0 + n[q].y * x1);
-            vacc[q].x += x0;
-            vacc[q].y += x1;
-        }
-        park[kParkH * 256] = e;
-    }
-    if (a.mask & 8u) {
-        take_row(std::integral_constant<int, 1>{}, a.lap);
-        real e = 0.0;
+            n[q] = (z.valid && PL::slot_out(q) && PL::lane_out(z.j, q)) ? mkc(a.ds(n[q].x), a.ds(n[q].y)) : mkc(1.0, 1.0);
+            vacc[q] = mkc(0.0, 0.0);
+        }
+        if constexpr (ROOTS_ONCE) {
+            if (a.mask & kRootTerms) {
+#pragma unroll
+                for (int q = 0; q < E; ++q)
+                    yv[q] = mkc(n[q].x != 0.0 ? fm::rsixth(n[q].x) : (real)0.0, n[q].y != 0.0 ? fm::rsixth(n[q].y) : (real)0.0);
+            }
+        }
+        auto root_y = [&](int q, int c) -> real {
+            if constexpr (ROOTS_ONCE) return c ? yv[q].y : yv[q].x;
+            else {
+                const real nn = c ? n[q].y : n[q].x;
+                return nn != 0.0 ? fm::rsixth(nn) : (real)0.0;
+            }
+        };
+        auto request_after = [&](auto ic) {
+            constexpr int I = decltype(ic)::value;
+            const cplx* p = nullptr;
+#pragma unroll
+            for (int k = 5; k > I; --k)
+                if (chain[k]) p = chain[k];
+            if constexpr (PIPE) {
+                if (p) z_issue_row<M, E>(nx, nyq_nx, z, p, g);
+                else if (XP && I >= 0 && first_spec) z_issue_row<M, E>(nx, nyq_nx, zn, first_spec, g);
+            }
+        };
+        auto take_row = [&](auto ic, const cplx* spec) {
+            if constexpr (PIPE) {
+#pragma unroll
+                for (int q = 0; q < E; ++q) w[q] = nx[q];
+                const real nyq_w = nyq_nx;
+                request_after(ic);
+                z_inverse_regs<M, E>(w, z, twM, twN, nyq_w);
+            } else {
+                z_load_inverse<M, E>(w, z, spec, g, twM, twN);
+            }
+        };
+        if (!XP) request_after(std::integral_constant<int, -1>{});
+        if ((a.mask & 2u) && a.vh) {
+            take_row(std::integral_constant<int, 0>{}, a.vh);
+            real e = 0.0;
+#pragma unroll
+            for (int q = 0; q < E; ++q) {
+                const real x0 = w[q].x * sc, x1 = w[q].y * sc;
+                e += 0.5 * (n[q].x * x0 + n[q].y * x1);
+                vacc[q].x += x0;
+                vacc[q].y += x1;
+            }
+            if (z.valid) park[kParkH * 256] += e;
+        }
+        if (a.mask & 8u) {
+            take_row(std::integral_constant<int, 1>{}, a.lap);
+            real e = 0.0;
+#pragma unroll
+            for (int q = 0; q < E; ++q) {
+                __builtin_amdgcn_sched_barrier(0);
+                const real x0 = w[q].x * sc, x1 = w[q].y * sc;
+                const real y0 = root_y(q, 0), y1 = root_y(q, 1);
+                const real r0 = y0 * y0 * y0, r1 = y1 * y1 * y1;
+                e += -0.5 * (n[q].x * r0 * x0 + n[q].y * r1 * x1);
+                vacc[q].x += -0.5 * x0 * r0;
+                vacc[q].y += -0.5 * x1 * r1;
+            }
+            if (z.valid) park[kParkVw * 256] += e;
+        }
+        if (a.mask & 16u) {
+            take_row(std::integral_constant<int, 2>{}, a.conv_b);
+            cplx pa1[E];
+            real e = 0.0;
+#pragma unroll
+            for (int q = 0; q < E; ++q) {
+                __builtin_amdgcn_sched_barrier(0);
+                const real x0 = w[q].x * sc, x1 = w[q].y * sc;
+                pa1[q] = a.tc.wt_is_56 ? mkc(root_y(q, 0), root_y(q, 1)) : mkc(pow_pos(n[q].x, a.tc.wt_alpha - 1.0), pow_pos(n[q].y, a.tc.wt_alpha - 1.0));
+                e += ctf * ((pa1[q].x * n[q].x - a.tc.wt_nbar_pa) * x0 + (pa1[q].y * n[q].y - a.tc.wt_nbar_pa) * x1);
+                const real f = w_nl * (a.conv_a ? a.tc.wt_alpha : 2.0 * a.tc.wt_alpha);
+                vacc[q].x += ctf * f * pa1[q].x * x0;
+                vacc[q].y += ctf * f * pa1[q].y * x1;
+            }
+            if (a.conv_a) {
+                take_row(std::integral_constant<int, 3>{}, a.conv_a);
+                if (a.tc.wt_sym) {
+                    real e2 = 0.0;
+#pragma unroll
+                    for (int q = 0; q < E; ++q) {
+                        const real p0 = ctf * pow_pos(n[q].x, a.tc.wt_beta - 1.0) * w[q].x * sc, p1 = ctf * pow_pos(n[q].y, a.tc.wt_beta - 1.0) * w[q].y * sc;
+                        e2 += p0 * n[q].x + p1 * n[q].y;
+                        vacc[q].x += w_nl * a.tc.wt_beta * p0;
+                        vacc[q].y += w_nl * a.tc.wt_beta * p1;
+                    }
+                    e = (real)0.5 * (e + e2);
+                } else {
+#pragma unroll
+                    for (int q = 0; q < E; ++q) {
+                        vacc[q].x += w_nl * ctf * a.tc.wt_beta * pow_pos(n[q].x, a.tc.wt_beta - 1.0) * w[q].x * sc;
+                        vacc[q].y += w_nl * ctf * a.tc.wt_beta * pow_pos(n[q].y, a.tc.wt_beta - 1.0) * w[q].y * sc;
+                    }
+                }
+            }
+            if (z.valid) park[kParkWt * 256] += e;
+        }
+        if (a.mask & 32u) {
+            if (WGC_INLINE) {
+                cplx ux[OFDFT_Z_PREFETCH ? E : 1];
+                real nyq_ux = 0.0;
+                wgc_first_row<M, E>(ux, nyq_ux, z, a, g);
+                const real e = wgc_row_section<M, E, false>(n, vacc, w, z, a, g, twM, twN, sc, ctf, ux, nyq_ux, zn);
+                if (z.valid) park[kParkWgc * 256] += e;
+            } else if (!a.v_part_deferred) {
+                z_load_real<M, E, true>(w, z, a.v_part);
+#pragma unroll
+                for (int q = 0; q < E; ++q) {
+                    vacc[q].x += w[q].x;
+                    vacc[q].y += w[q].y;
+                }
+            }
+        }
+        if (a.mask & (7u << 10)) {
+            take_row(std::integral_constant<int, 4>{}, a.div);
+            cplx d[E];
+            z_load_real<M, E, true>(d, z, a.dfdn);
+#pragma unroll
+            for (int q = 0; q < E; ++q) {
+                vacc[q].x += d[q].x - 2.0 * w[q].x * sc;
+                vacc[q].y += d[q].y - 2.0 * w[q].y * sc;
+            }
+            if (a.div2) {
+                take_row(std::integral_constant<int, 5>{}, a.div2);
+#pragma unroll
+                for (int q = 0; q < E; ++q) {
+                    vacc[q].x -= 2.0 * w[q].x * sc;
+                    vacc[q].y -= 2.0 * w[q].y * sc;
+                }
+            }
+        }
+        if (a.mask & 1u) {
+            cplx ve[E];
+            z_load_real<M, E, true>(ve, z, a.vext);
+            real e = 0.0;
+#pragma unroll
+            for (int q = 0; q < E; ++q) {
+                e += n[q].x * ve[q].x + n[q].y * ve[q].y;
+                vacc[q].x += ve[q].x;
+                vacc[q].y += ve[q].y;
+            }
+            if (z.valid) park[kParkIe * 256] += e;
+        }
+        acc_t e_tf = 0.0, e_gtf = 0.0, e_x = 0.0, e_c = 0.0, e_vn = 0.0;
 #pragma unroll
         for (int q = 0; q < E; ++q) {
             __builtin_amdgcn_sched_barrier(0);
-            const real x0 = w[q].x * sc, x1 = w[q].y * sc;
-            const real y0 = root_y(q, 0), y1 = root_y(q, 1);
-            const real r0 = y0 * y0 * y0, r1 = y1 * y1 * y1;
-            e += -0.5 * (n[q].x * r0 * x0 + n[q].y * r1 * x1);
-            vacc[q].x += -0.5 * x0 * r0;
-            vacc[q].y += -0.5 * x1 * r1;
-        }
-        park[kParkVw * 256] = e;
-    }
-    if (a.mask & 16u) {
-        take_row(std::integral_constant<int, 2>{}, a.conv_b);
-        cplx pa1[E];
-        real e = 0.0;
-#pragma unroll
-        for (int q = 0; q < E; ++q) {
-            __builtin_amdgcn_sched_barrier(0);
-            const real x0 = w[q].x * sc, x1 = w[q].y * sc;
-            pa1[q] = a.tc.wt_is_56 ? mkc(root_y(q, 0), root_y(q, 1)) : mkc(pow_pos(n[q].x, a.tc.wt_alpha - 1.0), pow_pos(n[q].y, a.tc.wt_alpha - 1.0));
-            e += ctf * ((pa1[q].x * n[q].x - a.tc.wt_nbar_pa) * x0 + (pa1[q].y * n[q].y - a.tc.wt_nbar_pa) * x1);
-            const real f = w_nl * (a.conv_a ? a.tc.wt_alpha : 2.0 * a.tc.wt_alpha);
-            vacc[q].x += ctf * f * pa1[q].x * x0;
-            vacc[q].y += ctf * f * pa1[q].y * x1;
-        }
-        park[kParkWt * 256] = e;
-        if (a.conv_a) {
-            take_row(std::integral_constant<int, 3>{}, a.conv_a);
-            if (a.tc.wt_sym) {
-                real e2 = 0.0;
-#pragma unroll
-                for (int q = 0; q < E; ++q) {
-                    const real p0 = ctf * pow_pos(n[q].x, a.tc.wt_beta - 1.0) * w[q].x * sc, p1 = ctf * pow_pos(n[q].y, a.tc.wt_beta - 1.0) * w[q].y * sc;
-                    e2 += p0 * n[q].x + p1 * n[q].y;
-                    vacc[q].x += w_nl * a.tc.wt_beta * p0;
-                    vacc[q].y += w_nl * a.tc.wt_beta * p1;
-                }
-                park[kParkWt * 256] = (real)0.5 * (park[kParkWt * 256] + e2);
-            } else {
-#pragma unroll
-                for (int q = 0; q < E; ++q) {
-                    vacc[q].x += w_nl * ctf * a.tc.wt_beta * pow_pos(n[q].x, a.tc.wt_beta - 1.0) * w[q].x * sc;
-                    vacc[q].y += w_nl * ctf * a.tc.wt_beta * pow_pos(n[q].y, a.tc.wt_beta - 1.0) * w[q].y * sc;
-                }
-            }
-        }
-    }
-    if (a.mask & 32u) {
-        if (WGC_INLINE) {
-            park[kParkWgc * 256] = wgc_row_section<M, E>(n, vacc, w, z, a, g, twM, twN, sc, ctf);
-        } else if (!a.v_part_deferred) {
-            z_load_real<M, E, true>(w, z, a.v_part);
-#pragma unroll
-            for (int q = 0; q < E; ++q) {
-                vacc[q].x += w[q].x;
-                vacc[q].y += w[q].y;
-            }
-        }
-    }
-    if (a.mask & (7u << 10)) {
-        take_row(std::integral_constant<int, 4>{}, a.div);
-        cplx d[E];
-        z_load_real<M, E, true>(d, z, a.dfdn);
-#pragma unroll
-        for (int q = 0; q < E; ++q) {
-            vacc[q].x += d[q].x - 2.0 * w[q].x * sc;
-            vacc[q].y += d[q].y - 2.0 * w[q].y * sc;
-        }
-        if (a.div2) {
-            take_row(std::integral_constant<int, 5>{}, a.div2);
-#pragma unroll
-            for (int q = 0; q < E; ++q) {
-                vacc[q].x -= 2.0 * w[q].x * sc;
-                vacc[q].y -= 2.0 * w[q].y * sc;
-            }
-        }
-    }
-    if (a.mask & 1u) {
-        cplx ve[E];
-        z_load_real<M, E, true>(ve, z, a.vext);
-        real e = 0.0;
-#pragma unroll
-        for (int q = 0; q < E; ++q) {
-            e += n[q].x * ve[q].x + n[q].y * ve[q].y;
-            vacc[q].x += ve[q].x;
-            vacc[q].y += ve[q].y;
-        }
-        park[kParkIe * 256] = e;
-    }
-    acc_t acc[kCombineScalars];
-#pragma unroll
-    for (int s = 0; s < kCombineScalars; ++s) acc[s] = 0.0;
-#pragma unroll
-    for (int q = 0; q < E; ++q) {
-        __builtin_amdgcn_sched_barrier(0);
-        if (!(PL::slot_out(q) && PL::lane_out(z.j, q))) continue;
-        const fm::Roots<real> rt0 = fm::roots_from_y(n[q].x, root_y(q, 0)), rt1 = fm::roots_from_y(n[q].y, root_y(q, 1));
-        if (a.mask & 4u) {
-            const real c0 = rt0.n13, c1 = rt1.n13;
-            acc[2] += ctf * (c0 * c0 * n[q].x + c1 * c1 * n[q].y);
-            vacc[q].x += w_tf * (5.0 / 3.0) * ctf * c0 * c0;
-            vacc[q].y += w_tf * (5.0 / 3.0) * ctf * c1 * c1;
-        }
-        if (a.mask & (1u << 13)) {
-            real e0, v0, e1, v1;
-            vwgtf_point(n[q].x, rt0.n13, ctf, a.tc.gtf_inv_n0, a.tc.gtf_kind, e0, v0);
-            vwgtf_point(n[q].y, rt1.n13, ctf, a.tc.gtf_inv_n0, a.tc.gtf_kind, e1, v1);
-            acc[9] += e0 + e1;
-            vacc[q].x += v0;
-            vacc[q].y += v1;
-        }
-        if (a.mask & (0xFu << 6)) {
-            const XcLocal x0 = lda_point(n[q].x, a.mask, rt0), x1 = lda_point(n[q].y, a.mask, rt1);
-            acc[6] += x0.ex + x1.ex;
-            acc[7] += x0.ec + x1.ec;
-            vacc[q].x += x0.vx + x0.vc;
-            vacc[q].y += x1.vx + x1.vc;
-        }
-        acc[8] += vacc[q].x * n[q].x + vacc[q].y * n[q].y;
+            if (!(PL::slot_out(q) && PL::lane_out(z.j, q))) continue;
+            const fm::Roots<real> rt0 = fm::roots_from_y(n[q].x, root_y(q, 0)), rt1 = fm::roots_from_y(n[q].y, root_y(q, 1));
+            if (a.mask & 4u) {
+                const real c0 = rt0.n13, c1 = rt1.n13;
+                e_tf += ctf * (c0 * c0 * n[q].x + c1 * c1 * n[q].y);
+                vacc[q].x += w_tf * (5.0 / 3.0) * ctf * c0 * c0;
+                vacc[q].y += w_tf * (5.0 / 3.0) * ctf * c1 * c1;
+            }
+            if (a.mask & (1u << 13)) {
+                real e0, v0, e1, v1;
+                vwgtf_point(n[q].x, rt0.n13, ctf, a.tc.gtf_inv_n0, a.tc.gtf_kind, e0, v0);
+                vwgtf_point(n[q].y, rt1.n13, ctf, a.tc.gtf_inv_n0, a.tc.gtf_kind, e1, v1);
+                e_gtf += e0 + e1;
+                vacc[q].x += v0;
+                vacc[q].y += v1;
+            }
+            if (a.mask & (0xFu << 6)) {
+                const XcLocal x0 = lda_point(n[q].x, a.mask, rt0), x1 = lda_point(n[q].y, a.mask, rt1);
+                e_x += x0.ex + x1.ex;
+                e_c += x0.ec + x1.ec;
+                vacc[q].x += x0.vx + x0.vc;
+                vacc[q].y += x1.vx + x1.vc;
+            }
+            e_vn += vacc[q].x * n[q].x + vacc[q].y * n[q].y;
+        }
+        if (z.valid) {
+            const acc_t el[5] = {e_tf, e_x, e_c, e_vn, e_gtf};
+#pragma unroll
+            for (int s = 0; s < 5; ++s) {
+                if constexpr (WGC_INLINE) lpark[s * 256] += el[s];
+                else acc[kLocalSlot[s]] += el[s];
+            }
+        }
+        if constexpr (XP) z_load_real<M, E, true>(n, zn, a.ds.src);
+        if (a.v_out) z_store_real<M, E>(vacc, z, a.v_out);
+        z = zn;
     }
     acc[0] = park[kParkIe * 256];
     acc[1] = park[kParkH * 256];
     acc[3] = park[kParkVw * 256];
     acc[4] = park[kParkWt * 256];
     acc[5] = park[kParkWgc * 256];
-    if (!z.valid) {
-#pragma unroll
-        for (int s = 0; s < kCombineScalars; ++s) acc[s] = 0.0;
+    if constexpr (WGC_INLINE) {
+#pragma unroll
+        for (int s = 0; s < 5; ++s) acc[kLocalSlot[s]] = lpark[s * 256];
     }
     if (a.eh_part && g.blk0 + blockIdx.x == 0) {
         for (long long i = threadIdx.x; i < a.eh_rows; i += blockDim.x) acc[1] += a.eh_part[i];
     }
-    if (a.v_out) z_store_real<M, E>(vacc, z, a.v_out);
     block_reduce_store<kCombineScalars>(acc, partial + (long long)g.blk0 * kCombineScalars);
 }
 
@@ -975,25 +1090,39 @@
     const cplx *twM, *twN;
     const ZTwReq<M, E> twq = z_tw_request<M, E>(twM_g, twN_g);
     a.ds = a.ds.resolved();
-    const ZLane<M, E> z(g, lds);
+    constexpr bool XP = OFDFT_Z_PREFETCH && ZW<M, E>::PL::EXACT && (OFDFT_ZT_PREFETCH & 16) != 0;
+    const ZTiles tl(g);
+    ZLane<M, E> z(g, lds, tl.first);
     const real ctf = kCtf;
-    cplx n[E], vacc[E], w[E];
+    cplx n[E], vacc[E], w[E], nx[OFDFT_Z_PREFETCH ? E : 1];
+    real nyq_nx = 0.0;
     z_load_real<M, E, true>(n, z, a.ds.src);
+    if constexpr (XP) wgc_first_row<M, E>(nx, nyq_nx, z, a, g);
     z_tw_commit<M, E>(lds, twq, twM_g, twN_g, twM, twN);
     using PL = typename ZW<M, E>::PL;
-#pragma unroll
-    for (int q = 0; q < E; ++q) {
-        n[q] = (z.valid && PL::slot_out(q) && PL::lane_out(z.j, q)) ? mkc(a.ds(n[q].x), a.ds(n[q].y)) : mkc(1.0, 1.0);
-        vacc[q] = mkc(0.0, 0.0);
-    }
-    acc_t acc[2];
-    acc[0] = wgc_row_section<M, E>(n, vacc, w, z, a, g, twM, twN, a.inv_n, ctf);
-    acc[1] = 0.0;
-#pragma unroll
-    for (int q = 0; q < E; ++q)
-        if (PL::slot_out(q) && PL::lane_out(z.j, q)) acc[1] += vacc[q].x * n[q].x + vacc[q].y * n[q].y;
-    if (!z.valid) acc[0] = acc[1] = 0.0;
-    z_store_real<M, E>(vacc, z, v_part);
+    acc_t acc[2] = {0.0, 0.0};
+    for (int t = 0; t < tl.count; ++t) {
+        const ZLane<M, E> zn = z.next(g, t + 1 < tl.count);
+        if (t > 0 && !XP) z_load_real<M, E, true>(n, z, a.ds.src);
+        if constexpr (!XP) wgc_first_row<M, E>(nx, nyq_nx, z, a, g);
+#pragma unroll
+        for (int q = 0; q < E; ++q) {
+            n[q] = (z.valid && PL::slot_out(q) && PL::lane_out(z.j, q)) ? mkc(a.ds(n[q].x), a.ds(n[q].y)) : mkc(1.0, 1.0);
+            vacc[q] = mkc(0.0, 0.0);
+        }
+        const acc_t e = wgc_row_section<M, E, XP>(n, vacc, w, z, a, g, twM, twN, a.inv_n, ctf, nx, nyq_nx, zn);
+        acc_t vn = 0.0;
+#pragma unroll
+        for (int q = 0; q < E; ++q)
+            if (PL::slot_out(q) && PL::lane_out(z.j, q)) vn += vacc[q].x * n[q].x + vacc[q].y * n[q].y;
+        if (z.valid) {
+            acc[0] += e;
+            acc[1] += vn;
+        }
+        if constexpr (XP) z_load_real<M, E, true>(n, zn, a.ds.src);
+        z_store_real<M, E>(vacc, z, v_part);
+        z = zn;
+    }
     block_reduce_store<2>(acc, partial + (long long)g.blk0 * 2);
 }
 
```

Result: slower. 402.3 evals/s (-5.0%).
